# HPCForge/Bubbleformer

Measured on AMD Instinct MI355X. Metric: train samples/sec, FiLMAViT 16x192x192x4ch, bs=8 per GPU, higher is better.
Workload: dtype bf16; 1 GPU; FiLMAViT-small (E=384, 6 heads, 12 blocks, P=16, 9 fluid params) fwd + relative-L2 loss + bwd + AdamW, 4-field 16x192x192 clips, batch 8 per GPU (BASELINE.json configs[1]); global_batch=8, parallelism=dp1

## Files before the change

### bubbleformer_amd/_lib.py

```python
import ctypes as C
import os
import subprocess

_HERE = os.path.dirname(os.path.abspath(__file__))
LIB_PATH = os.path.join(_HERE, "libbubbleformer_hip.so")
CSRC = os.path.join(_HERE, "csrc")

BF_DTYPE_F32, BF_DTYPE_BF16 = 0, 1
BF_LAY_KC, BF_LAY_XC = 0, 1
BF_PRO_NONE, BF_PRO_AFFINE, BF_PRO_AFFINE_GELU, BF_PRO_GELU = 0, 1, 2, 3
BF_AUX_NONE, BF_AUX_ADD, BF_AUX_DGELU = 0, 1, 2
BF_OUT_STORE, BF_OUT_STORE_F32, BF_OUT_ATOMIC_F32 = 0, 1, 2
BF_MAX_STAGES = 5
BF_LOSS_LIMBS = 5

vp, fp, i32, i64, f32 = C.c_void_p, C.c_void_p, C.c_int32, C.c_int64, C.c_float


class Operand(C.Structure):
    _fields_ = [("p", vp), ("ld", i64), ("layout", i32), ("seglen", i32), ("segstride", i64), ("gw", i32), ("gh", i32),
                ("gc", i32), ("pro", i32), ("sc", fp), ("sh", fp), ("rows_per_frame", i32), ("nch", i32)]


class Epilogue(C.Structure):
    _fields_ = [("bias", fp), ("colscale", fp), ("colshift", fp), ("aux_mode", i32), ("aux", vp), ("ld_aux", i64),
                ("out_mode", i32), ("c", vp), ("ldc", i64), ("seglen", i32), ("segstride", i64), ("gw", i32), ("gh", i32),
                ("gc", i32), ("gelu_out", vp), ("colsum", fp), ("rowscale", fp), ("rows_per_group", i32)]


class Dims(C.Structure):
    _fields_ = [(n, i32) for n in ("dtype", "B", "T", "h", "w", "E", "heads", "attn_scale", "feat_scale", "patch", "cin",
                                   "cout", "nfluid")]


TEMPORAL_FIELDS = ("gamma", "attn_scale_factor", "norm1_w", "norm1_b", "norm2_w", "norm2_b", "input_head_w", "input_head_b",
                   "output_head_w", "output_head_b", "qnorm_w", "qnorm_b", "knorm_w", "knorm_b", "rel_pos_emb")
SPATIAL_FIELDS = ("gamma_att", "gamma_mlp", "attn_scale_factor_x", "attn_scale_factor_y", "low_freq_scalar",
                  "high_freq_scalar", "norm1_w", "norm1_b", "norm2_w", "norm2_b", "input_head_w", "input_head_b",
                  "output_head_w", "output_head_b", "qnorm_w", "qnorm_b", "knorm_w", "knorm_b", "rel_pos_emb", "fc1_w", "fc1_b",
                  "fc2_w", "fc2_b", "mlp_norm_w", "mlp_norm_b")


class TemporalParams(C.Structure):
    _fields_ = [(n, fp) for n in TEMPORAL_FIELDS]


class SpatialParams(C.Structure):
    _fields_ = [(n, fp) for n in SPATIAL_FIELDS]


class FrameNorm(C.Structure):
    _fields_ = [("w", fp), ("b", fp), ("g", fp), ("gdiv", i32), ("mean", fp), ("rstd", fp), ("sc", fp), ("sh", fp), ("resid", vp), ("out", vp)]


class EmbedParams(C.Structure):
    _fields_ = [("conv_w", fp * BF_MAX_STAGES), ("in_w", fp * BF_MAX_STAGES), ("in_b", fp * BF_MAX_STAGES), ("film_ln_w", fp),
                ("film_ln_b", fp), ("film_w", fp), ("film_b", fp)]


class DebedParams(C.Structure):
    _fields_ = [("conv_w", fp * BF_MAX_STAGES), ("in_w", fp * BF_MAX_STAGES), ("in_b", fp * BF_MAX_STAGES)]


class ConvSrc(C.Structure):
    _fields_ = [("p", vp), ("C", i32), ("nchw", i32), ("f32", i32)]


class ConvGeo(C.Structure):
    _fields_ = [(n, i32) for n in ("F", "Hi", "Wi", "Ho", "Wo", "kh", "kw", "stride", "pad")]


BF_CONV_PRO_NONE, BF_CONV_PRO_AFFINE_GELU, BF_CONV_PRO_GELU = 0, 1, 2

STAGE_DONE_FN = C.CFUNCTYPE(None, C.c_int, C.c_void_p)
P = C.POINTER
SIGNATURES = {
    "bf_last_error": (C.c_char_p, []),
    "bf_abi_version": (C.c_int, []),
    "bf_prof_enable": (None, [C.c_int]),
    "bf_debug_force_generic_attn": (None, [C.c_int]),
    "bf_debug_tokred_fold": (None, [C.c_int]),
    "bf_side_defer": (None, [C.c_int]),
    "bf_prep_stages": (C.c_int, [C.POINTER(Dims), C.c_int, C.POINTER(C.c_int32), C.POINTER(vp), C.POINTER(vp), C.POINTER(vp), vp]),
    "bf_stage_prepared": (None, [C.c_int]),
    "bf_trunk_train_fwd": (C.c_int, [C.POINTER(Dims), C.c_int, C.POINTER(C.c_int32), C.POINTER(vp), C.POINTER(vp), C.POINTER(vp), C.POINTER(vp), vp,
                                     C.POINTER(vp), vp, vp]),
    "bf_trunk_train_bwd": (C.c_int, [C.POINTER(Dims), C.c_int, C.POINTER(C.c_int32), C.POINTER(vp), C.POINTER(vp), C.POINTER(vp), C.POINTER(vp),
                                     C.POINTER(vp), vp, C.POINTER(vp), vp, C.POINTER(vp), vp, vp, vp, vp, vp]),
    "bf_field_stats_ws_doubles": (i64, [C.c_int]),
    "bf_field_stats": (C.c_int, [fp, vp, vp, C.c_int, vp, vp, vp]),
    "bf_stage_chain_next": (C.c_int, [C.POINTER(Dims), C.c_int, vp, vp]),
    "bf_stage_next_scale": (C.c_int, [fp, C.c_int]),
    "bf_gemm_fwd_frames": (C.c_int, [C.c_int, C.c_int, C.c_int, C.c_int, vp, i64, vp, i64, fp, fp, fp, fp, C.c_int, vp, vp, C.c_int,
                                     C.POINTER(FrameNorm), C.POINTER(FrameNorm), vp]),
    "bf_trunk_eval_weights_bytes": (i64, [C.POINTER(Dims), C.c_int, C.POINTER(C.c_int32)]),
    "bf_trunk_eval_prepare": (C.c_int, [C.POINTER(Dims), C.c_int, C.POINTER(C.c_int32), C.POINTER(vp), vp, vp]),
    "bf_trunk_eval_fwd": (C.c_int, [C.POINTER(Dims), C.c_int, C.POINTER(C.c_int32), C.POINTER(vp), vp, vp, vp, vp, vp]),
    "bf_frame_linear": (C.c_int, [C.c_int, C.c_int, C.c_int, C.c_int, C.c_int, vp, i64, vp, i64, fp, fp, fp, fp, fp, vp, i64, C.c_int, fp, fp, fp,
                                  vp, i64, fp, fp, vp, i64, vp]),
    "bf_side_join": (C.c_int, [vp]),
    "bf_prof_report": (C.c_int, [C.c_char_p, C.c_int]),
    "bf_gemm": (C.c_int, [C.c_int, C.c_int, C.c_int, C.c_int, P(Operand), P(Operand), P(Epilogue), C.c_int, vp]),
    "bf_gemm_tokred": (C.c_int, [C.c_int, C.c_int, C.c_int, i64, vp, i64, vp, i64, fp, C.c_int, fp, fp, i64, vp]),
    "bf_gemm_tokred_ws_floats": (i64, [C.c_int, C.c_int, i64]),
    "bf_gemm_inbwd_frames": (C.c_int, [C.c_int, C.c_int, C.c_int, C.c_int, vp, i64, vp, i64, vp, vp, vp, C.c_int, fp, fp, fp, fp, fp, C.c_int, vp]),
    "bf_gemm_inbwd_frames_chain": (C.c_int, [C.c_int, C.c_int, C.c_int, C.c_int, vp, i64, vp, i64, vp, vp, vp, C.c_int, fp, fp, fp, fp, fp, C.c_int,
                                             vp, vp, fp, fp, fp, fp, C.c_int, fp, vp]),
    "bf_in_stats": (C.c_int, [C.c_int, vp, C.c_int, C.c_int, C.c_int, fp, fp, fp, C.c_int, fp, fp, fp, fp, fp, fp, vp]),
    "bf_in_ws_floats": (i64, [C.c_int, C.c_int, C.c_int, C.c_int]),
    "bf_affine_apply": (C.c_int, [C.c_int, vp, vp, fp, fp, vp, i64, C.c_int, C.c_int, vp]),
    "bf_in_bwd": (C.c_int, [C.c_int, vp, vp, vp, vp, C.c_int, C.c_int, C.c_int, fp, fp, fp, fp, fp, C.c_int, C.c_int, fp, fp,
                            fp, fp, fp, vp]),
    "bf_colsum": (C.c_int, [C.c_int, vp, i64, C.c_int, fp, fp, vp]),
    "bf_attn_axial_fwd": (C.c_int, [C.c_int, vp, vp, i64, C.c_int, C.c_int, C.c_int, C.c_int, fp, fp, fp, fp, fp, fp, fp, vp]),
    "bf_attn_axial_norm_fwd": (C.c_int, [C.c_int, vp, vp, vp, i64, C.c_int, C.c_int, C.c_int, C.c_int, fp, fp, fp, fp, fp, fp, fp, fp, fp, fp, fp, fp,
                                         fp, vp]),
    "bf_attn_fwd": (C.c_int, [C.c_int, vp, vp, i64, C.c_int, i64, i64, i64, i64, C.c_int, C.c_int, fp, fp, fp, fp, fp, fp, f32,
                              C.c_int, vp]),
    "bf_attn_bwd": (C.c_int, [C.c_int, vp, vp, vp, i64, C.c_int, i64, i64, i64, i64, C.c_int, C.c_int, fp, fp, fp, fp, fp, fp,
                              fp, fp, fp, fp, fp, fp, f32, C.c_int, fp, i64, vp]),
    "bf_im2col_nchw": (C.c_int, [C.c_int, fp, vp, C.c_int, C.c_int, C.c_int, C.c_int, C.c_int, vp]),
    "bf_col2im_nchw": (C.c_int, [C.c_int, vp, fp, C.c_int, C.c_int, C.c_int, C.c_int, C.c_int, vp]),
    "bf_pm2nchw": (C.c_int, [fp, fp, fp, fp, C.c_int, C.c_int, C.c_int, C.c_int, C.c_int, vp]),
    "bf_debed_last_bwd": (C.c_int, [C.c_int, fp, fp, fp, fp, fp, vp, vp, vp, C.c_int, C.c_int, C.c_int, C.c_int, C.c_int, C.c_int, vp]),
    "bf_debed_last_bwd_norm": (C.c_int, [C.c_int, fp, fp, fp, fp, fp, vp, vp, vp, fp, fp, fp, fp, vp, fp, fp, C.c_int, C.c_int, C.c_int, C.c_int, C.c_int,
                                         C.c_int, fp, C.c_int64, vp]),
    "bf_gather_gemm": (C.c_int, [C.c_int, vp, vp, C.c_int, fp, fp, vp, C.c_int, C.c_int, C.c_int, C.c_int, C.c_int, vp]),
    "bf_scatter_gemm": (C.c_int, [C.c_int, vp, vp, C.c_int, fp, fp, vp, fp, C.c_int, C.c_int, C.c_int, C.c_int, C.c_int, vp]),
    "bf_gather_wgrad_ws_floats": (C.c_int64, [C.c_int, C.c_int, C.c_int]),
    "bf_gather_wgrad": (C.c_int, [C.c_int, vp, vp, fp, fp, fp, fp, fp, C.c_int, C.c_int, C.c_int, C.c_int, C.c_int, C.c_int, fp, C.c_int64, vp]),
    "bf_gather_gemm_rebuilt": (C.c_int, [C.c_int, vp, vp, vp, C.c_int, fp, fp, vp, C.c_int, C.c_int, C.c_int, C.c_int, C.c_int, vp]),
    "bf_gather_wgrad_rebuilt": (C.c_int, [C.c_int, vp, vp, vp, fp, fp, fp, C.c_int, C.c_int, C.c_int, C.c_int, C.c_int, C.c_int, fp, C.c_int64, vp]),
    "bf_stage_chain_head": (C.c_int, [vp, vp, vp]),
    "bf_stage_chain_tail": (C.c_int, [vp, vp, C.c_int]),
    "bf_embed_tail_ws_floats": (C.c_int64, [C.c_int, C.c_int, C.c_int, C.c_int, C.c_int]),
    "bf_embed_tail_bwd": (C.c_int, [C.c_int, vp, vp, vp, vp, vp, fp, fp, fp, fp, fp, fp, fp, fp, C.c_int, C.c_int, C.c_int, C.c_int, C.c_int, C.c_int,
                                    fp, C.c_int64, vp]),
    "bf_embed_first": (C.c_int, [C.c_int, fp, vp, vp, vp, C.c_int, C.c_int, C.c_int, C.c_int, C.c_int, C.c_int, fp, vp]),
    "bf_in_stats_merge_slices": (C.c_int, [C.c_int, C.c_int, C.c_int, C.c_int, C.c_int, fp, fp, fp, C.c_int, fp, fp, fp, fp, fp, fp, vp]),
    "bf_debed_last": (C.c_int, [C.c_int, vp, fp, fp, vp, fp, fp, fp, C.c_int, C.c_int, C.c_int, C.c_int, C.c_int, C.c_int, vp]),
    "bf_lploss_finalize": (C.c_int, [fp, C.c_int, C.c_int, fp, fp, vp]),
    "bf_nchw2pm": (C.c_int, [C.c_int, fp, fp, fp, fp, fp, vp, C.c_int, C.c_int, C.c_int, C.c_int, C.c_int, vp]),
    "bf_wprep": (C.c_int, [C.c_int, C.c_int, fp, vp, C.c_int, C.c_int, C.c_int, vp]),
    "bf_wgrad_unprep": (C.c_int, [C.c_int, fp, fp, C.c_int, C.c_int, C.c_int, C.c_int, vp]),
    "bf_film_net_fwd": (C.c_int, [fp, fp, fp, fp, fp, fp, fp, fp, C.c_int, C.c_int, C.c_int, vp]),
    "bf_film_net_bwd": (C.c_int, [fp, fp, fp, fp, fp, fp, fp, fp, fp, C.c_int, C.c_int, C.c_int, vp]),
    "bf_adamw": (C.c_int, [fp, fp, fp, fp, i64, C.c_int, f32, f32, f32, f32, f32, f32, vp]),
    "bf_adam": (C.c_int, [fp, fp, fp, fp, i64, C.c_int, f32, f32, f32, f32, f32, f32, vp]),
    "bf_lion": (C.c_int, [fp, fp, fp, i64, f32, f32, f32, f32, f32, vp]),
    "bf_grad_norm_ws_doubles": (i64, [i64]),
    "bf_grad_norm": (C.c_int, [fp, i64, f32, f32, fp, vp, i64, vp]),
    "bf_adamw_dev": (C.c_int, [fp, fp, fp, fp, i64, C.c_int, f32, f32, f32, f32, f32, f32, fp, f32, vp]),
    "bf_adam_dev": (C.c_int, [fp, fp, fp, fp, i64, C.c_int, f32, f32, f32, f32, f32, f32, fp, f32, vp]),
    "bf_lion_dev": (C.c_int, [fp, fp, fp, i64, f32, f32, f32, f32, f32, fp, f32, vp]),
    "bf_eikonal_sum": (C.c_int, [fp, i64, C.c_int, C.c_int, f32, vp, vp]),
    "bf_eikonal_l1_frames": (C.c_int, [fp, i64, C.c_int, C.c_int, f32, fp, vp]),
    "bf_heatflux_rows": (C.c_int, [fp, fp, i64, i64, C.c_int, f32, f32, f32, f32, fp, vp]),
    "bf_clip_gather": (C.c_int, [fp, i64, vp, vp, C.c_int, fp, fp, fp, C.c_int, C.c_int, C.c_int, C.c_int, C.c_int, C.c_int, C.c_int, vp]),
    "bf_clip_gather_batch": (C.c_int, [fp, i64, vp, i64, vp, vp, fp, fp, C.c_int, C.c_int, fp, vp, fp, fp, C.c_int, C.c_int, fp, fp, vp, C.c_int, fp,
                                       C.c_int, C.c_int, C.c_int, C.c_int, C.c_int, vp]),
    "bf_rollout_score_ws_doubles": (i64, [C.c_int, C.c_int, C.c_int, C.c_int, C.c_int]),
    "bf_rollout_score": (C.c_int, [fp, fp, i64, i64, C.c_int, vp, vp, vp, fp, fp, C.c_int, f32, fp, fp, fp, fp, fp, fp, vp, i64, C.c_int, C.c_int,
                                   C.c_int, C.c_int, C.c_int, C.c_int, C.c_int, C.c_int, vp]),
    "bf_rollout_heatflux": (C.c_int, [fp, fp, i64, i64, C.c_int, vp, vp, vp, fp, fp, C.c_int, C.c_int, fp, f32, f32, f32, f32, fp, fp, C.c_int, C.c_int,
# ... 88 lines not shown
```

### bubbleformer_amd/csrc/attn_mfma.hip

```cpp
#include "bf_common.h"
#include "param_reduce.h"
#include <stdlib.h>

namespace {

typedef __attribute__((ext_vector_type(8))) short s16x8;
typedef __attribute__((address_space(3))) s16x4* lds_s16x4;

__device__ __forceinline__ void drain_vm() { __builtin_amdgcn_s_waitcnt(0x0F70); }
__device__ __forceinline__ void wsync() {
    __builtin_amdgcn_fence(__ATOMIC_ACQ_REL, "wavefront");
    __builtin_amdgcn_wave_barrier();
}
__device__ __forceinline__ int t5b(int n) {
    const int a = n < 0 ? -n : n;
    int b;
    if (a < 8) b = a; else if (a < 10) b = 8; else if (a < 12) b = 9; else if (a < 14) b = 10; else if (a < 16) b = 11;
    else if (a < 20) b = 12; else if (a < 23) b = 13; else if (a < 27) b = 14; else b = 15;
    return b + (n < 0 ? 16 : 0);
}
typedef unsigned u32x2 __attribute__((ext_vector_type(2)));
__device__ __forceinline__ float quad_sum(float v) {
    u32x2 r = __builtin_amdgcn_permlane16_swap(__float_as_uint(v), __float_as_uint(v), false, false);
    v = __uint_as_float(r[0]) + __uint_as_float(r[1]);
// ... 812 lines not shown
        const int head = (int)(((long)blockIdx.x * wpb + wave) % heads);
#pragma unroll
        for (int jb = 0; jb < NB; ++jb)
#pragma unroll
            for (int ib = 0; ib < NB; ++ib)
#pragma unroll
                for (int r = 0; r < 4; ++r) {
                    const int i = 16 * ib + i16, j = 16 * jb + 4 * gq + r;
                    if (gr.demb && i < L && j < L) atomicAdd(&s_demb[t5b(i - j) * 16 + head], a_emb[jb][ib][r]);
                }
        if (p.hscale && gr.dhscale) {
            a_dhs = wave_sum(a_dhs);
            if (lane == 0) atomicAdd(&s_dhs[head], a_dhs);
        }
    }
#pragma unroll
    for (int k = 0; k < NACC; ++k) {
        const int v = 16 * k + i16, q = v / (8 * KS), ks = (v >> 3) % KS, j = v & 7;
        relay[q * D + 32 * ks + 8 * gq + j] = a_ln[k];
    }
    __syncthreads();
    const int nvals = 4 * D + 32 * heads + heads;
    for (int i = threadIdx.x; i < nvals; i += blockDim.x) {
        float val;
        float* dst;
        if (i < 4 * D) {
            val = 0.f;
            for (int w = 0; w < wpb; ++w) val += reinterpret_cast<const float*>(smem_bwd + w * PER_WAVE)[i];
            const int q = i / D, e = i % D; dst = (q == 0 ? gr.dqw : q == 1 ? gr.dqb : q == 2 ? gr.dkw : gr.dkb); if (dst) dst += e; }
        else if (i < 4 * D + 32 * heads) { const int t = i - 4 * D; val = s_demb[(t / heads) * 16 + (t % heads)]; dst = gr.demb ? gr.demb + t : nullptr; }
        else { const int t = i - 4 * D - 32 * heads; val = s_dhs[t]; dst = gr.dhscale ? gr.dhscale + t : nullptr; }
        if (ws) ws[(long)blockIdx.x * nvals + i] = val;
        else if (dst && val != 0.f) atomicAdd(dst, val);
    }
}

__global__ void __launch_bounds__(64 * BF_RED_FL) attn_ws_reduce(AttnReduceJob j) {
    __shared__ float red[1][BF_RED_FL][64];
    attn_reduce_block(j, blockIdx.x, blockIdx.y, gridDim.y, red);
}

template <typename K>
int set_lds(K kernel, size_t shm) {
    if (shm > 64 * 1024) {
        hipError_t e = hipFuncSetAttribute(reinterpret_cast<const void*>(kernel), hipFuncAttributeMaxDynamicSharedMemorySize, (int)shm);
        if (e != hipSuccess) return bf_fail(e, __FILE__, __LINE__);
    }
    return 0;
}

template <int NB, int KS>
int go_fwd(const bf16* qkv, bf16* out, Geo g, int heads, Par p, float out_scale, int accumulate, hipStream_t st) {
    constexpr int D = 32 * KS;
    const int wpb = 4;
    const size_t shm = (size_t)wpb * 16 * NB * (D + 16) * sizeof(bf16);
    const long nprob = g.nseq * heads;
    BF_REQUIRE(nprob < (1L << 31) && g.inner < (1L << 31), "attention: problem count must fit 31 bits");
    static const int bpc = bf_knob("BF_ATTN_FWD_BPC", 2);
    const int grid = (int)std::min<long>((nprob + wpb - 1) / wpb, 256L * bpc);
    hipLaunchKernelGGL((attn_fwd_mfma<NB, KS>), dim3(grid), dim3(wpb * 64), shm, st, qkv, out, g, heads, p, out_scale, accumulate);
    BF_CHECK_LAUNCH();
    return 0;
}
template <int NB, int KS, int ACC>
int go_bwd_mode(const bf16* qkv, const bf16* dout, bf16* dqkv, Geo g, int heads, Par p, Grd gr, float out_scale, int accumulate, float* ws,
                long ws_floats, int* rows_out, hipStream_t st) {
    constexpr int D = 32 * KS, R = 16 * NB;
    const int wpb = NB == 1 ? 4 : 2;
    const size_t shm = (size_t)wpb * (3 * R * (D + 16) + 2 * R * 40) * sizeof(bf16);
    if (int rc = set_lds(attn_bwd_mfma<NB, KS, ACC>, shm)) return rc;
    const long nprob = g.nseq * heads;
    BF_REQUIRE(nprob < (1L << 31) && g.inner < (1L << 31), "attention: problem count must fit 31 bits");
    const int nvals = 4 * D + 32 * heads + heads;
    static int resident = 0;
    if (!resident) {
        int dev = 0, cus = 256, per_cu = 1;
        (void)hipGetDevice(&dev);
        (void)hipDeviceGetAttribute(&cus, hipDeviceAttributeMultiprocessorCount, dev);
        if (hipOccupancyMaxActiveBlocksPerMultiprocessor(&per_cu, attn_bwd_mfma<NB, KS, ACC>, wpb * 64, shm) != hipSuccess || per_cu < 1) per_cu = 1;
        static const int bpc = bf_knob("BF_ATTN_BWD_BPC", 0);
        if (bpc > 0) per_cu = bpc;
        resident = cus * per_cu;
    }
    long grid = std::min<long>((nprob + wpb - 1) / wpb, (long)resident);
    {
        long a = wpb, b = heads;
        while (b) { const long t = a % b; a = b; b = t; }
        const long m = heads / a;
        if (grid >= 8 * m) grid -= grid % m;
    }
    if (ws && ws_floats < grid * nvals) { grid = ws_floats / nvals; if (grid < 1) ws = nullptr; }
    hipLaunchKernelGGL((attn_bwd_mfma<NB, KS, ACC>), dim3((int)grid), dim3(wpb * 64), shm, st, qkv, dout, dqkv, g, heads, p, gr, out_scale, accumulate, ws);
    BF_CHECK_LAUNCH();
    if (rows_out) { *rows_out = ws ? (int)grid : 0; return 0; }
    if (ws) {
        const AttnReduceJob j{ws, (int)grid, D, heads, gr.dqw, gr.dqb, gr.dkw, gr.dkb, gr.demb, gr.dhscale};
        hipLaunchKernelGGL(attn_ws_reduce, dim3(bf_cdiv(nvals, 64), 1), dim3(64 * BF_RED_FL), 0, st, j);
        BF_CHECK_LAUNCH();
    }
    return 0;
}
template <int NB, int KS>
int go_bwd(const bf16* qkv, const bf16* dout, bf16* dqkv, Geo g, int heads, Par p, Grd gr, float out_scale, int accumulate, float* ws,
           long ws_floats, int* rows_out, hipStream_t st) {
#define BF_MODE(A) return go_bwd_mode<NB, KS, A>(qkv, dout, dqkv, g, heads, p, gr, out_scale, accumulate, ws, ws_floats, rows_out, st)
    if constexpr (NB == 1 && KS == 2) {
        switch (accumulate) { case 0: BF_MODE(0); case 1: BF_MODE(1); case 2: BF_MODE(2); case 5: BF_MODE(5); default: break; }
    }
    BF_MODE(-1);
#undef BF_MODE
}

}

int bf_attn_fwd_mfma(const void* qkv, void* out, long nseq, int L, long inner, long outer_stride, long inner_stride, long tok_stride, int heads,
                     int d, const float* qw, const float* qb, const float* kw, const float* kb, const float* emb, const float* hscale,
                     float out_scale, int accumulate, hipStream_t st) {
    Geo g{nseq, L, inner, outer_stride, inner_stride, tok_stride};
    Par p{qw, qb, kw, kb, emb, hscale};
    const int nb = L <= 16 ? 1 : 2, ks = d / 32;
#define GO(NB, KS) if (nb == NB && ks == KS) return go_fwd<NB, KS>((const bf16*)qkv, (bf16*)out, g, heads, p, out_scale, accumulate, st)
    GO(1, 1); GO(1, 2); GO(1, 3); GO(1, 4); GO(2, 1); GO(2, 2); GO(2, 3); GO(2, 4);
#undef GO
    return bf_fail_msg("bf_attn_fwd_mfma: unsupported shape", __FILE__, __LINE__);
}
int bf_attn_axial_fwd_mfma(const void* qkv, void* out, int frames, int h, int w, int heads, int d, const float* qw, const float* qb, const float* kw,
                           const float* kb, const float* emb, const float* hscale_x, const float* hscale_y, const float* nw, const float* nb,
                           void* out_n, float* mean, float* rstd, float* sc, float* sh, hipStream_t st) {
    static const bool off = bf_knob("BF_ATTN_AXIAL_FUSED", 1) == 0;
    if (off || h > 16 || w > 16 || h < 1 || w < 1 || d % 32 || d > 128 || heads > 16) return 1;
    Par p{qw, qb, kw, kb, emb, hscale_x};
    const long ntile = (long)frames * heads;
    static const int wpb_env = bf_knob("BF_ATTN_AXIAL_WPB", 0);
    const int ks = d / 32, wpb = (wpb_env == 4 || wpb_env == 12) ? wpb_env : (ntile <= 256 ? 12 : 4);
    const bool norm = nw != nullptr;
    const size_t tile = ((size_t)h * w * (d + 8) + 7) & ~(size_t)7;
    const size_t shm = ((size_t)wpb * 16 * (d + 16) + tile) * sizeof(bf16) + (norm ? ((size_t)(256 / (d / 8)) + 2) * d * sizeof(float) : 0);
    const int grid = (int)std::min<long>(ntile, 256L * 3);
    const AxNorm nrm{nw, nb, (bf16*)out_n, mean, rstd, sc, sh};
#define GO2(KS, NRM, W) { if (int rc = set_lds(attn_fwd_axial_mfma<KS, NRM, W>, shm)) return rc; \
        hipLaunchKernelGGL((attn_fwd_axial_mfma<KS, NRM, W>), dim3(grid), dim3(W * 64), shm, st, (const bf16*)qkv, (bf16*)out, frames, h, w, heads, p, hscale_y, nrm); }
#define GO(KS) if (ks == KS) { \
        if (norm) { if (wpb == 12) GO2(KS, true, 12) else GO2(KS, true, 4) } \
        else { if (wpb == 12) GO2(KS, false, 12) else GO2(KS, false, 4) } }
    GO(1) GO(2) GO(3) GO(4)
#undef GO
#undef GO2
    BF_CHECK_LAUNCH();
    return 0;
}
int bf_attn_bwd_mfma(const void* qkv, const void* dout, void* dqkv, long nseq, int L, long inner, long outer_stride, long inner_stride,
                     long tok_stride, int heads, int d, const float* qw, const float* qb, const float* kw, const float* kb, const float* emb,
                     const float* hscale, float* dqw, float* dqb, float* dkw, float* dkb, float* demb, float* dhscale, float out_scale,
                     int accumulate, float* ws, long ws_floats, int* rows_out, hipStream_t st) {
    Geo g{nseq, L, inner, outer_stride, inner_stride, tok_stride};
    Par p{qw, qb, kw, kb, emb, hscale};
    Grd gr{dqw, dqb, dkw, dkb, demb, dhscale};
    const int nb = L <= 16 ? 1 : 2, ks = d / 32;
#define GO(NB, KS) if (nb == NB && ks == KS) return go_bwd<NB, KS>((const bf16*)qkv, (const bf16*)dout, (bf16*)dqkv, g, heads, p, gr, out_scale, accumulate, ws, ws_floats, rows_out, st)
    GO(1, 1); GO(1, 2); GO(1, 3); GO(1, 4); GO(2, 1); GO(2, 2); GO(2, 3); GO(2, 4);
#undef GO
    return bf_fail_msg("bf_attn_bwd_mfma: unsupported shape", __FILE__, __LINE__);
}
```

### bubbleformer_amd/csrc/bf_common.h

```cpp
#pragma once
#include <hip/hip_runtime.h>
#include <stdint.h>
#include <math.h>

#include "../../include/bubbleformer_hip.h"

typedef __bf16 bf16;
typedef __attribute__((ext_vector_type(8))) __bf16 bf16x8;
typedef __attribute__((ext_vector_type(4))) __bf16 bf16x4;
typedef __attribute__((ext_vector_type(4))) short s16x4;
typedef __attribute__((ext_vector_type(4))) float f32x4;

#define BF_WAVE 64
#define BF_IN_EPS 1e-5f

#define BF_CHECK_LAUNCH()                                   \
    do {                                                    \
        hipError_t e__ = hipGetLastError();                 \
        if (e__ != hipSuccess) return bf_fail(e__, __FILE__, __LINE__); \
    } while (0)
#define BF_REQUIRE(cond, msg)                                \
    do {                                                     \
        if (!(cond)) return bf_fail_msg(msg, __FILE__, __LINE__); \
    } while (0)

int bf_prof_begin(hipStream_t st);
bool bf_prof_is_on();
void bf_prof_end(int idx, hipStream_t st, const char* name, double flops, double bytes);
struct BfProfScope {
    int idx; hipStream_t st; const char* name; double flops, bytes;
    BfProfScope(hipStream_t s, const char* n, double f, double b) : idx(bf_prof_begin(s)), st(s), name(n), flops(f), bytes(b) {}
    ~BfProfScope() { if (idx >= 0) bf_prof_end(idx, st, name, flops, bytes); }
};

int bf_in_bwd_partials(int dtype, const void* dy, const void* x, const void* add, void* dx, int frames, int S, int C, const float* mean,
                       const float* rstd, const float* w, const float* b, const float* g, int gdiv, int gelu, float* ws, hipStream_t stream);
int bf_attn_bwd_partials(int dtype, const void* qkv, const void* dout, void* dqkv, int64_t nseq, int L, int64_t inner, int64_t outer_stride,
                         int64_t inner_stride, int64_t tok_stride, int heads, int d, const float* qw, const float* qb, const float* kw,
                         const float* kb, const float* emb, const float* hscale, float* dqw, float* dqb, float* dkw, float* dkb, float* demb,
                         float* dhscale, float out_scale, int accumulate, float* ws, int64_t ws_floats, int* rows, hipStream_t stream);
int bf_in_stats_apply(int dtype, const void* x, int frames, int S, int C, const float* w, const float* b, const float* g, int gdiv, const float* gb,
                      float* mean, float* rstd, float* sc, float* sh, float* ws, const void* resid, void* out, hipStream_t stream);
int bf_in_stats_apply_chain(int dtype, const void* x, int frames, int S, int C, const float* w, const float* b, const float* g, int gdiv, const float* gb,
                            float* mean, float* rstd, float* sc, float* sh, float* ws, const void* resid, void* out, const float* nw, const float* nb,
                            float* nmean, float* nrstd, float* nsc, float* nsh, void* nxn, bool* chained, hipStream_t stream);
int bf_wprep_multi(int dtype, int n, const int* mode, const float* const* src, void* const* dst, const int* R, const int* K, const int* Kp, hipStream_t st);
int bf_frame_scale(int dtype, const void* z, const float* m, int fdiv, void* out, long nrows, int S, int C, hipStream_t st);

int bf_gemm_slabs(int dtype, int M, int N, int K, const bf_operand* A, const bf_operand* B, float* out, long ldc, int accumulate, int splitk,
                  float* ws, long ws_floats, hipStream_t st);
int bf_tokred_narrow(int dtype, int C, int64_t P, const void* wide, const void* narrow, float* out, int ldo, int accumulate, int transposed,
                     const float* sc, const float* sh, int64_t rows_per_frame, float* ws, int64_t ws_floats, hipStream_t st);
int bf_gemm_pair_scaled(int M, int N, int K, const bf_operand* A, const bf_operand* B, const bf_epilogue* E, void* out2, const float* rowfac,
                        int rows_per_group, hipStream_t st);

#ifdef BF_EXPERIMENTS
#include <stdlib.h>
inline int bf_knob(const char* name, int dflt) { const char* v = getenv(name); return v ? atoi(v) : dflt; }
#else
constexpr int bf_knob(const char*, int dflt) { return dflt; }
#endif

struct BfPerDeviceOnce {
    bool done[64] = {};
    bool& flag() { int dev = 0; (void)hipGetDevice(&dev); return done[(dev >= 0 && dev < 64) ? dev : 0]; }
};
template <class T> struct BfPerDevice {
    T tab[64] = {};
    T& get() { int dev = 0; (void)hipGetDevice(&dev); return tab[(dev >= 0 && dev < 64) ? dev : 0]; }
};
int bf_fail(hipError_t e, const char* file, int line);
int bf_fail_msg(const char* msg, const char* file, int line);
int bf_decline(const char* msg);

__device__ __forceinline__ float to_f(float x) { return x; }
__device__ __forceinline__ float to_f(bf16 x) { return (float)x; }
template <typename T> __device__ __forceinline__ T from_f(float x);
template <> __device__ __forceinline__ float from_f<float>(float x) { return x; }
template <> __device__ __forceinline__ bf16 from_f<bf16>(float x) { return (bf16)x; }

template <typename T> struct Chunk;
template <> struct Chunk<float> {
    static constexpr int N = 4;
    float4 raw;
    __device__ __forceinline__ void load(const float* p) { raw = *reinterpret_cast<const float4*>(p); }
    __device__ __forceinline__ void store(float* p) const { *reinterpret_cast<float4*>(p) = raw; }
    __device__ __forceinline__ void zero() { raw = make_float4(0.f, 0.f, 0.f, 0.f); }
    __device__ __forceinline__ float get(int i) const { return i == 0 ? raw.x : i == 1 ? raw.y : i == 2 ? raw.z : raw.w; }
    __device__ __forceinline__ void set(int i, float v) { if (i == 0) raw.x = v; else if (i == 1) raw.y = v; else if (i == 2) raw.z = v; else raw.w = v; }
};
template <> struct Chunk<bf16> {
    static constexpr int N = 8;
    bf16x8 raw;
    __device__ __forceinline__ void load(const bf16* p) { raw = *reinterpret_cast<const bf16x8*>(p); }
    __device__ __forceinline__ void store(bf16* p) const { *reinterpret_cast<bf16x8*>(p) = raw; }
    __device__ __forceinline__ void zero() { for (int i = 0; i < 8; ++i) raw[i] = (bf16)0.f; }
    __device__ __forceinline__ float get(int i) const { return (float)raw[i]; }
    __device__ __forceinline__ void set(int i, float v) { raw[i] = (bf16)v; }
};

__device__ __forceinline__ float erf_fast(float x) {
    const float ax = fabsf(x);
    const float t = __builtin_amdgcn_rcpf(1.0f + 0.3275911f * ax);
    const float poly = t * (0.254829592f + t * (-0.284496736f + t * (1.421413741f + t * (-1.453152027f + t * 1.061405429f))));
    const float r = 1.0f - poly * __expf(-ax * ax);
    return copysignf(r, x);
}
__device__ __forceinline__ float gelu_f(float x) { return 0.5f * x * (1.0f + erf_fast(x * 0.70710678118654752440f)); }
__device__ __forceinline__ float dgelu_f(float x) {
    const float ax = fabsf(x) * 0.70710678118654752440f;
    const float t = __builtin_amdgcn_rcpf(1.0f + 0.3275911f * ax);
    const float poly = t * (0.254829592f + t * (-0.284496736f + t * (1.421413741f + t * (-1.453152027f + t * 1.061405429f))));
    const float e = __expf(-0.5f * x * x);
    const float cdf = 0.5f * (1.0f + copysignf(1.0f - poly * e, x));
    return cdf + x * (0.39894228040143267794f * e);
}

__device__ __forceinline__ float phi_fast(float x) {
    const float xc = fminf(fmaxf(x, -4.0f), 4.0f), u = xc * xc;
    float r = -1.520480094e-09f;
    r = r * u + 1.180964698e-07f; r = r * u - 4.014221545e-06f; r = r * u + 7.960997465e-05f; r = r * u - 1.041295800e-03f;
    r = r * u + 9.641715296e-03f; r = r * u - 6.614117438e-02f; r = r * u + 3.988329119e-01f;
    return 0.5f + xc * r;
}
__device__ __forceinline__ float gelu_fast(float x) { return x * phi_fast(x); }
__device__ __forceinline__ float dgelu_fast(float x) {
    const float xc = fminf(fmaxf(x, -4.0f), 4.0f), u = xc * xc;
    float r = 9.387459194e-10f;
    r = r * u - 7.941240515e-08f; r = r * u + 2.950722870e-06f; r = r * u - 6.380590451e-05f; r = r * u + 8.975979855e-04f;
    r = r * u - 8.669717964e-03f; r = r * u + 5.833777581e-02f; r = r * u - 2.646917422e-01f; r = r * u + 7.975648121e-01f;
    return 0.5f + xc * r;
}

// ... 17 lines not shown
```

### bubbleformer_amd/csrc/gemm_stream.hip

```cpp
#include "gemm_common.h"
#include <stdio.h>
#include <stdlib.h>
#include <algorithm>

namespace {
using namespace bfgemm;

constexpr int BM = 256, BNB = 128, BK = 64;
constexpr int CHUNK = BNB * BK;
constexpr int ACHUNK = BM * BK;
constexpr int NSLOT = 2;

struct StreamArgs {
    const bf16* A; long lda; const bf16* W; long ldw; bf16* C; long ldc;
    const float* bias; const float* colscale; const float* colshift; const float* rowscale; int rpg;
    int aux_mode; const bf16* aux; long ld_aux; bf16* gelu_out;
    int KS, mt, nb, ng;
    int mh, hunit;
    int stagger;
    int dbg;
};

__device__ __forceinline__ void wait_vm_n(int n) {
    if (n >= 16) { wait_vm<16>(); return; }
// ... 409 lines not shown
            if constexpr (CS) {
#pragma unroll
                for (int i = 0; i < 4; ++i) asm volatile("" : "+v"(rsr[i]));
            }
            __builtin_amdgcn_sched_barrier(0);
        }
#pragma unroll
        for (int i = 0; i < 4; ++i) {
            const int m = m0 + wm * 64 + i * 16 + li;
#pragma unroll
            for (int pp = 0; pp < 2; ++pp) {
                float v[8];
#pragma unroll
                for (int r = 0; r < 4; ++r) {
                    typedef __attribute__((ext_vector_type(2))) unsigned u32x2;
                    const u32x2 sw = __builtin_amdgcn_permlane16_swap(__float_as_uint(acc[i][2 * pp][r]), __float_as_uint(acc[i][2 * pp + 1][r]), false, false);
                    v[r] = __uint_as_float(sw[0]); v[4 + r] = __uint_as_float(sw[1]);
                }
                if constexpr (AUX == BF_AUX_ADD) {
                    const bf16x8 ax = __builtin_bit_cast(bf16x8, auxr[i][pp]);
#pragma unroll
                    for (int q = 0; q < 8; ++q) {
                        float cs_ = 1.f, ch_ = 0.f;
                        if constexpr (CS) { cs_ = e_cs[pp][q]; ch_ = e_ch[pp][q]; }
                        v[q] = epi_lin_add(v[q], e_bias[pp][q], cs_, ch_, has_rs ? rsr[i] : 1.f, CS, (float)ax[q]);
                    }
                } else {
#pragma unroll
                    for (int q = 0; q < 8; ++q) {
                        float cs_ = 1.f, ch_ = 0.f;
                        if constexpr (CS) { cs_ = e_cs[pp][q]; ch_ = e_ch[pp][q]; }
                        v[q] = epi_lin(v[q], e_bias[pp][q], cs_, ch_, has_rs ? rsr[i] : 1.f, CS);
                    }
                    if constexpr (AUX == BF_AUX_DGELU) {
                        const bf16x8 ax = __builtin_bit_cast(bf16x8, auxr[i][pp]);
#pragma unroll
                        for (int q = 0; q < 8; ++q) v[q] = v[q] * dgelu_fast((float)ax[q]);
                    }
                }
                bf16x8 o;
#pragma unroll
                for (int q = 0; q < 8; ++q) o[q] = (bf16)v[q];
                const long off = (long)m * a.ldc + c_nb * BNB + c8 + 32 * pp;
                *reinterpret_cast<bf16x8*>(a.C + off) = o;
                if constexpr (GELU2) {
                    bf16x8 g8;
#pragma unroll
                    for (int q = 0; q < 8; ++q) g8[q] = (bf16)gelu_fast(v[q]);
                    *reinterpret_cast<bf16x8*>(a.gelu_out + off) = g8;
                }
            }
        }
        issued += GELU2 ? 16 : 8;
    }
}


int num_cus() {
    static const int n = []() {
        int dev = 0; hipDeviceProp_t p;
        if (hipGetDevice(&dev) != hipSuccess || hipGetDeviceProperties(&p, dev) != hipSuccess || p.multiProcessorCount < 8) return 256;
        return p.multiProcessorCount;
    }();
    return n;
}

bool team_split(int NB, int mt, int wpx, int* nb, int* ng) {
    static const int force = bf_knob("BF_STREAM_GROUPS", 0);
    int best = 0, best_cost = 0;
    for (int g = 1; g <= NB; ++g) {
        if (NB % g || NB / g > wpx || (force > 0 && g != force)) continue;
        const int nteams = 8 * (wpx / (NB / g));
        if (nteams < g) continue;
        const int fewest = nteams / g;
        const int cost = (mt + fewest - 1) / fewest;
        if (!best || cost < best_cost) { best = g; best_cost = cost; }
    }
    if (!best) return false;
    *ng = best; *nb = NB / best;
    return true;
}

}

int bf_gemm_stream_try(int M, int N, int K, const bf_operand* A, const bf_operand* B, const bf_epilogue* E, hipStream_t st) {
    static const int enabled = bf_knob("BF_GEMM_STREAM", 1);
    if (!enabled) return 1;
    if (A->layout != BF_LAY_KC || B->layout != BF_LAY_KC || A->pro != BF_PRO_NONE || B->pro != BF_PRO_NONE) return 1;
    if (A->gw > 0 || A->seglen > 0 || B->gw > 0 || B->seglen > 0 || E->gw > 0 || E->seglen > 0) return 1;
    if (E->out_mode != BF_OUT_STORE || E->colsum) return 1;
    static const int pp_env = bf_knob("BF_STREAM_PP", -1);
    if (M % BM || N % BNB || K % BK || K < 2 * BK) return 1;
    const bool ws_ok = K >= 4 * BK && K <= 6 * BK;
    const bool use_pp = pp_env == 1 || !ws_ok;
    if (pp_env == 0 && !ws_ok) return 1;
    if (A->ld % 8 || B->ld % 8 || E->ldc % 8 || (E->aux_mode != BF_AUX_NONE && E->ld_aux % 8)) return 1;
    if (((uintptr_t)A->p | (uintptr_t)B->p | (uintptr_t)E->c | (uintptr_t)E->aux | (uintptr_t)E->gelu_out) & 15) return 1;
    if (E->gelu_out && E->aux_mode != BF_AUX_NONE) return 1;
    if (E->colscale && !E->colshift) return 1;
    StreamArgs a;
    a.A = (const bf16*)A->p; a.lda = A->ld; a.W = (const bf16*)B->p; a.ldw = B->ld; a.C = (bf16*)E->c; a.ldc = E->ldc;
    a.bias = E->bias; a.colscale = E->colscale; a.colshift = E->colshift; a.rowscale = E->rowscale; a.rpg = E->rows_per_group > 0 ? E->rows_per_group : 1;
    a.aux_mode = E->aux_mode; a.aux = (const bf16*)E->aux; a.ld_aux = E->ld_aux; a.gelu_out = (bf16*)E->gelu_out;
    a.KS = K / BK; a.mt = M / BM; a.mh = M / (BM / 2);
    static const int half_on = bf_knob("BF_STREAM_HALF", 1);
    a.hunit = half_on ? 1 : 2;
    const int grid = (num_cus() / 8) * 8;
    if (!team_split(N / BNB, (use_pp || !half_on) ? a.mt : a.mh, grid / 8, &a.nb, &a.ng)) return 1;
    static const int dbg = bf_knob("BF_STREAM_DEBUG", 0);
    a.dbg = dbg;
    static const int stagger = bf_knob("BF_STREAM_STAGGER", 1);
    a.stagger = stagger;
    const int lds_bytes = a.KS * CHUNK * 2 + NSLOT * ACHUNK * 2;
    static thread_local char pname[64];
    snprintf(pname, sizeof(pname), use_pp ? "stream_pp<%s>" : "stream_gemm<%s>", E->gelu_out ? "gelu2" : E->aux_mode == BF_AUX_ADD ? "add" : E->aux_mode == BF_AUX_DGELU ? "dgelu" : "plain");
    BfProfScope prof(st, pname, 2.0 * M * N * K, ((double)M * K + (double)N * K + (double)M * N * (E->gelu_out ? 2 : 1) + (E->aux_mode != BF_AUX_NONE ? (double)M * N : 0.0)) * 2.0);
#define BF_STREAM_GO(AUXM, G2, CSF)                                                                                                       \
    do {                                                                                                                                \
        static BfPerDeviceOnce attr_once, attr_pp_once; bool& attr_done = attr_once.flag(); bool& attr_pp_done = attr_pp_once.flag();                                                                            \
        if (use_pp) {                                                                                                                   \
            if (!attr_pp_done) {                                                                                                        \
                hipError_t e_ = hipFuncSetAttribute((const void*)stream_pp_kernel<AUXM, G2, CSF>, hipFuncAttributeMaxDynamicSharedMemorySize, PNSLOT * PSLOT); \
                if (e_ != hipSuccess) return bf_fail(e_, __FILE__, __LINE__);                                                           \
                attr_pp_done = true;                                                                                                    \
            }                                                                                                                           \
            hipLaunchKernelGGL((stream_pp_kernel<AUXM, G2, CSF>), dim3(grid), dim3(512), PNSLOT * PSLOT, st, a);                        \
            break;                                                                                                                      \
        }                                                                                                                               \
        if (!attr_done) {                                                                                                               \
            hipError_t e_ = hipFuncSetAttribute((const void*)stream_gemm_kernel<AUXM, G2, CSF>, hipFuncAttributeMaxDynamicSharedMemorySize, 6 * CHUNK * 2 + NSLOT * ACHUNK * 2); \
            if (e_ != hipSuccess) return bf_fail(e_, __FILE__, __LINE__);                                                               \
            attr_done = true;                                                                                                           \
        }                                                                                                                               \
        hipLaunchKernelGGL((stream_gemm_kernel<AUXM, G2, CSF>), dim3(grid), dim3(512), lds_bytes, st, a);                                    \
    } while (0)
    const bool cs = E->colscale != nullptr || E->rowscale != nullptr;
    if (E->gelu_out && !cs) BF_STREAM_GO(BF_AUX_NONE, true, false);
    else if (E->gelu_out) return 1;
    else if (E->aux_mode == BF_AUX_ADD && cs) BF_STREAM_GO(BF_AUX_ADD, false, true);
    else if (E->aux_mode == BF_AUX_ADD) BF_STREAM_GO(BF_AUX_ADD, false, false);
    else if (E->aux_mode == BF_AUX_DGELU && !cs) BF_STREAM_GO(BF_AUX_DGELU, false, false);
    else if (E->aux_mode == BF_AUX_DGELU) return 1;
    else if (cs) return 1;
    else BF_STREAM_GO(BF_AUX_NONE, false, false);
#undef BF_STREAM_GO
    BF_CHECK_LAUNCH();
    return 0;
}
```

### bubbleformer_amd/csrc/gemm_tokred.hip

```cpp
#include "gemm_common.h"
#include <stdio.h>
#include <stdlib.h>
#include <algorithm>

namespace {
using namespace bfgemm;

constexpr int PTN = 192;
constexpr int HR = 32;
constexpr int NSB = PTN / 64;
constexpr int SUBB = HR * 64 * 2;
constexpr int NBUF = 4;
template <int NI> struct PPGeom {
    static constexpr int TM = 64 * NI, HALFB = (NI + NSB) * SUBB, TILES = NI * 6, TILE_FLOATS = TM * PTN;
};

template <int OFF>
__device__ __forceinline__ void glds16_off(const void* gsrc, unsigned lds_dst) {
    unsigned keep;
    asm volatile("s_mov_b32 %0, m0\n\ts_mov_b32 m0, %2\n\ts_nop 0\n\tglobal_load_lds_dwordx4 %1, off offset:%3\n\ts_mov_b32 m0, %0"
                 : "=&s"(keep) : "v"(gsrc), "s"(lds_dst - (unsigned)OFF), "n"(OFF) : "memory");
}

typedef __attribute__((address_space(3))) s16x4* lds_s16x4_ptr;
__device__ __forceinline__ bf16x8 tr_frag(unsigned addr) {
    const s16x4 lo = __builtin_amdgcn_ds_read_tr16_b64_v4i16((lds_s16x4_ptr)(uintptr_t)addr);
    const s16x4 hi = __builtin_amdgcn_ds_read_tr16_b64_v4i16((lds_s16x4_ptr)(uintptr_t)(addr + 512u));
    typedef __attribute__((ext_vector_type(8))) short s16x8;
    const s16x8 r = {lo[0], lo[1], lo[2], lo[3], hi[0], hi[1], hi[2], hi[3]};
    return __builtin_bit_cast(bf16x8, r);
}

template <int NI, int GRP>
__device__ __forceinline__ void tokred_pp_body(const bf16* __restrict__ A, long lda, const bf16* __restrict__ B, long ldb,
                                               float* __restrict__ slab_tile, float* __restrict__ cslab_row, int nh, bool do_cs,
                                               unsigned ring_lds, int lane, int w4) {
    using Gm = PPGeom<NI>;
    constexpr int HALFB = Gm::HALFB;
    constexpr int PG = NI == 6 ? (GRP == 0 ? 5 : 4) : 3;
    constexpr int NCS = 3;
    const int wm = w4, wn = GRP;
    const int dr = 8 * w4 + (lane >> 3);
    const int dkey = ((dr >> 1) & 1) | (((dr >> 3) & 1) << 1);
    const int dch = (lane & 7) ^ (dkey << 1);
    const bf16* pA = A + (long)dr * lda + 8 * dch;
    const bf16* pB = B + (long)dr * ldb + 8 * dch;
    const long stepA = (long)HR * lda, stepB = (long)HR * ldb;
    auto issue = [&](int buf) {
        const unsigned base = __builtin_amdgcn_readfirstlane(ring_lds + (unsigned)buf * (unsigned)HALFB + (unsigned)w4 * 1024u);
        if constexpr (NI == 6 && GRP == 0) {
            glds16_off<0>(pA, base + 0 * SUBB); glds16_off<128>(pA, base + 1 * SUBB); glds16_off<256>(pA, base + 2 * SUBB);
            glds16_off<384>(pA, base + 3 * SUBB); glds16_off<512>(pA, base + 4 * SUBB);
            pA += stepA;
        } else if constexpr (NI == 6) {
            glds16_off<640>(pA, base + 5 * SUBB);
            glds16_off<0>(pB, base + 6 * SUBB); glds16_off<128>(pB, base + 7 * SUBB); glds16_off<256>(pB, base + 8 * SUBB);
            pA += stepA; pB += stepB;
        } else if constexpr (GRP == 0) {
            glds16_off<0>(pA, base + 0 * SUBB); glds16_off<128>(pA, base + 1 * SUBB); glds16_off<256>(pA, base + 2 * SUBB);
            pA += stepA;
        } else {
            glds16_off<0>(pB, base + 3 * SUBB); glds16_off<128>(pB, base + 4 * SUBB); glds16_off<256>(pB, base + 5 * SUBB);
            pB += stepB;
        }
    };
    const int g = lane >> 4, q = (lane >> 2) & 3, p = lane & 3;
    const int fkey = ((q >> 1) & 1) | ((g & 1) << 1);
    const unsigned rowb = (unsigned)(8 * g + q) * 128u + (unsigned)(p & 1) * 8u;
    const unsigned offA = rowb + (unsigned)(((2 * wm + (p >> 1)) ^ (fkey << 1)) * 16);
    const unsigned offB0 = rowb + (unsigned)(((2 * wn + (p >> 1)) ^ (fkey << 1)) * 16) + (unsigned)(NI * SUBB);
    const unsigned offB1 = rowb + (unsigned)(((2 * wn + 4 + (p >> 1)) ^ (fkey << 1)) * 16) + (unsigned)(NI * SUBB);

    f32x4 acc[NI][6];
#pragma unroll
    for (int i = 0; i < NI; ++i)
#pragma unroll
        for (int j = 0; j < 6; ++j) acc[i][j] = f32x4{0.f, 0.f, 0.f, 0.f};
    f32x4 cs[NCS];
#pragma unroll
    for (int c = 0; c < NCS; ++c) cs[c] = f32x4{0.f, 0.f, 0.f, 0.f};
    bf16x8 ones;
#pragma unroll
    for (int c = 0; c < 8; ++c) ones[c] = (bf16)1.0f;

    issue(0);
    if (nh > 1) issue(1);
    if (nh > 2) issue(2);
    if (nh > 2) wait_vm<2 * PG>(); else if (nh > 1) wait_vm<PG>(); else wait_vm<0>();
    __builtin_amdgcn_s_barrier();
    if constexpr (GRP == 1) __builtin_amdgcn_s_barrier();

    int buf = 0;
    for (int h = 0; h < nh; ++h) {
        const unsigned hb = ring_lds + (unsigned)buf * (unsigned)HALFB;
        bf16x8 fa[NI], fb[6];
#pragma unroll
        for (int i = 0; i < NI; ++i) fa[i] = tr_frag(hb + offA + (unsigned)(i * SUBB));
#pragma unroll
        for (int j = 0; j < 6; ++j) fb[j] = tr_frag(hb + ((j & 1) ? offB1 : offB0) + (unsigned)((j >> 1) * SUBB));
        if (h + 3 < nh) issue((buf + 3) & 3);
        const int younger = min(h + 3, nh - 1) - (h + 1);
        if (younger >= 2) wait_vm<2 * PG>(); else if (younger == 1) wait_vm<PG>(); else wait_vm<0>();
        asm volatile("s_waitcnt lgkmcnt(0)" ::: "memory");
        __builtin_amdgcn_sched_barrier(0);
        __builtin_amdgcn_s_barrier();
#pragma unroll
        for (int i = 0; i < NI; ++i)
#pragma unroll
            for (int j = 0; j < 6; ++j) acc[i][j] = __builtin_amdgcn_mfma_f32_16x16x32_bf16(fb[j], fa[i], acc[i][j], 0, 0, 0);
        if (do_cs) {
#pragma unroll
            for (int c = 0; c < NCS; ++c) {
                if constexpr (NI == 6) cs[c] = __builtin_amdgcn_mfma_f32_16x16x32_bf16(ones, fa[NCS * GRP + c], cs[c], 0, 0, 0);
                else if constexpr (GRP == 0) cs[c] = __builtin_amdgcn_mfma_f32_16x16x32_bf16(ones, fa[c], cs[c], 0, 0, 0);
            }
        }
        __builtin_amdgcn_sched_barrier(0);
        __builtin_amdgcn_s_barrier();
        buf = (buf + 1) & 3;
    }
    if constexpr (GRP == 0) __builtin_amdgcn_s_barrier();

    const int wave = GRP * 4 + w4;
    float* so = slab_tile + ((size_t)wave * Gm::TILES * 64 + lane) * 4;
#pragma unroll
    for (int i = 0; i < NI; ++i)
#pragma unroll
        for (int j = 0; j < 6; ++j)
            *reinterpret_cast<float4*>(so + (size_t)(i * 6 + j) * 256) = make_float4(acc[i][j][0], acc[i][j][1], acc[i][j][2], acc[i][j][3]);
    if (do_cs && lane < 16) {
        if constexpr (NI == 6) {
#pragma unroll
            for (int c = 0; c < NCS; ++c) cslab_row[16 * (wm + 4 * (NCS * GRP + c)) + lane] = cs[c][0];
        } else if constexpr (GRP == 0) {
#pragma unroll
            for (int c = 0; c < NCS; ++c) cslab_row[16 * (wm + 4 * c) + lane] = cs[c][0];
        }
    }
}

struct FoldRed { const float* slab; const float* cslab; int nslice, ntiles, tiles_k, Nout, Kin; float* out; float* colsum; int accumulate; int nwg; };
template <int NI>
__device__ __forceinline__ void fold_reduce(const FoldRed& r, int b) {
    using Gm = PPGeom<NI>;
    constexpr int T4 = Gm::TILE_FLOATS / 4;
    const long total = (long)r.ntiles * T4;
    const size_t sstride = (size_t)r.ntiles * Gm::TILE_FLOATS;
    for (long e = (long)b * 512 + threadIdx.x; e < total; e += (long)r.nwg * 512) {
        const int tile = (int)(e / T4), q = (int)(e - (long)tile * T4);
        const int lane = q & 63, t = q >> 6, wave = t / Gm::TILES, ij = t - wave * Gm::TILES, i = ij / 6, j = ij - i * 6;
        const int wm = wave & 3, wn = wave >> 2;
        const int nout = (tile / r.tiles_k) * Gm::TM + 16 * (wm + 4 * i) + (lane & 15);
        const int kin = (tile % r.tiles_k) * PTN + 16 * (wn + 2 * j) + 4 * (lane >> 4);
        const float* src = r.slab + (size_t)tile * Gm::TILE_FLOATS + (size_t)q * 4;
        float4* dst = reinterpret_cast<float4*>(r.out + (size_t)nout * r.Kin + kin);
        float4 a = r.accumulate ? *dst : make_float4(0.f, 0.f, 0.f, 0.f);
        for (int s0 = 0; s0 < r.nslice; s0 += 8) {
            float4 v[8];
#pragma unroll
            for (int u = 0; u < 8; ++u) v[u] = s0 + u < r.nslice ? *reinterpret_cast<const float4*>(src + (size_t)(s0 + u) * sstride) : make_float4(0.f, 0.f, 0.f, 0.f);
#pragma unroll
            for (int u = 0; u < 8; ++u)
                if (s0 + u < r.nslice) { a.x += v[u].x; a.y += v[u].y; a.z += v[u].z; a.w += v[u].w; }
        }
        *dst = a;
    }
    if (r.colsum)
        for (long m = (long)b * 512 + threadIdx.x; m < r.Nout; m += (long)r.nwg * 512) {
            float a = r.accumulate ? r.colsum[m] : 0.f;
            for (int s2 = 0; s2 < r.nslice; ++s2) a += r.cslab[(size_t)s2 * r.Nout + m];
            r.colsum[m] = a;
        }
}

template <int NI>
__global__ void __launch_bounds__(512) tokred_pp_kernel(const bf16* __restrict__ A, long lda, const bf16* __restrict__ B, long ldb,
                                                      float* __restrict__ slab, float* __restrict__ cslab, int Nout, int halves_total,
                                                      int halves_per, int tiles_k, int ntiles, int main_wgs, FoldRed red) {
    using Gm = PPGeom<NI>;
    extern __shared__ __attribute__((aligned(16))) char smem[];
    if ((int)blockIdx.x >= main_wgs) { fold_reduce<NI>(red, (int)blockIdx.x - main_wgs); return; }
    const int tid = threadIdx.x, lane = tid & 63, wave = __builtin_amdgcn_readfirstlane(tid >> 6);
    const int seq = xcd_remap(blockIdx.x, main_wgs);
    const int slice = seq / ntiles, tile = seq - slice * ntiles;
    const int n0 = (tile / tiles_k) * Gm::TM, c0 = (tile % tiles_k) * PTN;
    const int h_beg = slice * halves_per;
    const int nh = min(halves_per, halves_total - h_beg);
    const bf16* a0 = A + (long)h_beg * HR * lda + n0;
    const bf16* b0 = B + (long)h_beg * HR * ldb + c0;
    float* slab_tile = slab + ((size_t)slice * ntiles + tile) * Gm::TILE_FLOATS;
    const bool do_cs = cslab != nullptr && c0 == 0;
    float* cslab_row = do_cs ? cslab + (size_t)slice * Nout + n0 : nullptr;
    const unsigned ring_lds = lds_addr(smem);
    if (wave < 4) tokred_pp_body<NI, 0>(a0, lda, b0, ldb, slab_tile, cslab_row, nh, do_cs, ring_lds, lane, wave);
    else tokred_pp_body<NI, 1>(a0, lda, b0, ldb, slab_tile, cslab_row, nh, do_cs, ring_lds, lane, wave - 4);
}

template <int NI, int MAXS>
__global__ void __launch_bounds__(256) tokred_pp_reduce_kernel(const float* __restrict__ slab, const float* __restrict__ cslab, int nslice,
                                                               int ntiles, int tiles_k, int Nout, int Kin, float* __restrict__ out,
                                                               float* __restrict__ colsum, int accumulate) {
    using Gm = PPGeom<NI>;
    constexpr int T4 = Gm::TILE_FLOATS / 4;
    const long e = (long)blockIdx.x * 256 + threadIdx.x;
    if (e < (long)ntiles * T4) {
        const int tile = (int)(e / T4), r = (int)(e - (long)tile * T4);
        const int lane = r & 63, t = r >> 6, wave = t / Gm::TILES, ij = t - wave * Gm::TILES, i = ij / 6, j = ij - i * 6;
        const int wm = wave & 3, wn = wave >> 2;
        const int nout = (tile / tiles_k) * Gm::TM + 16 * (wm + 4 * i) + (lane & 15);
        const int kin = (tile % tiles_k) * PTN + 16 * (wn + 2 * j) + 4 * (lane >> 4);
        const size_t sstride = (size_t)ntiles * Gm::TILE_FLOATS;
        const float* src = slab + (size_t)tile * Gm::TILE_FLOATS + (size_t)r * 4;
        float4 v[MAXS];
#pragma unroll
        for (int s = 0; s < MAXS; ++s) v[s] = s < nslice ? *reinterpret_cast<const float4*>(src + s * sstride) : make_float4(0.f, 0.f, 0.f, 0.f);
        float4* dst = reinterpret_cast<float4*>(out + (size_t)nout * Kin + kin);
        float4 a = accumulate ? *dst : make_float4(0.f, 0.f, 0.f, 0.f);
#pragma unroll
        for (int s = 0; s < MAXS; ++s)
            if (s < nslice) { a.x += v[s].x; a.y += v[s].y; a.z += v[s].z; a.w += v[s].w; }
        *dst = a;
    }
    if (colsum && e < Nout) {
        float v[MAXS];
#pragma unroll
        for (int s = 0; s < MAXS; ++s) v[s] = s < nslice ? cslab[(size_t)s * Nout + e] : 0.f;
        float a = accumulate ? colsum[e] : 0.f;
#pragma unroll
        for (int s = 0; s < MAXS; ++s)
            if (s < nslice) a += v[s];
        colsum[e] = a;
    }
}

constexpr int NW_TILE = 32;
template <int CT, bool PRO>
__global__ void __launch_bounds__(256) tokred_narrow_kernel(const bf16* __restrict__ dy, const bf16* __restrict__ x, long tiles_total, float* __restrict__ slab,
                                                          const float* __restrict__ psc, const float* __restrict__ psh, int tiles_per_frame) {
    constexpr int C = 16 * CT, DYB = NW_TILE * C * 2, XB = NW_TILE * 16 * 2, TB_ = DYB + XB;
    extern __shared__ __attribute__((aligned(16))) char smem[];
    const int tid = threadIdx.x, lane = tid & 63, wave = __builtin_amdgcn_readfirstlane(tid >> 6);
    const long nwaves = (long)gridDim.x * 4, w = (long)blockIdx.x * 4 + wave;
    const long t_beg = tiles_total * w / nwaves, t_end = tiles_total * (w + 1) / nwaves;
    char* mine = smem + (size_t)wave * 2 * TB_;
    const unsigned lds0 = lds_addr(mine);
    auto issue = [&](long t, int slot) {
        const char* gd = reinterpret_cast<const char*>(dy) + t * DYB + lane * 16;
        const unsigned dst = __builtin_amdgcn_readfirstlane(lds0 + (unsigned)slot * (unsigned)TB_);
#pragma unroll
        for (int pce = 0; pce < DYB / 1024; ++pce) glds16(gd + pce * 1024, dst + (unsigned)pce * 1024u);
        glds16(reinterpret_cast<const char*>(x) + t * XB + lane * 16, dst + (unsigned)DYB);
    };
    constexpr int PCS = DYB / 1024 + 1;
    f32x4 acc[CT];
#pragma unroll
    for (int i = 0; i < CT; ++i) acc[i] = f32x4{0.f, 0.f, 0.f, 0.f};
    const int g = lane >> 4, q = (lane >> 2) & 3, pp = lane & 3;
    const unsigned offD = (unsigned)((8 * g + q) * (C * 2) + 8 * pp), offX = (unsigned)(DYB + (8 * g + q) * 32 + 8 * pp);
    auto trf = [&](unsigned addr, unsigned hi_off) {
        const s16x4 lo = __builtin_amdgcn_ds_read_tr16_b64_v4i16((lds_s16x4_ptr)(uintptr_t)addr);
        const s16x4 hi = __builtin_amdgcn_ds_read_tr16_b64_v4i16((lds_s16x4_ptr)(uintptr_t)(addr + hi_off));
        typedef __attribute__((ext_vector_type(8))) short s16x8;
        const s16x8 r = {lo[0], lo[1], lo[2], lo[3], hi[0], hi[1], hi[2], hi[3]};
        return __builtin_bit_cast(bf16x8, r);
    };
    float scv[CT], shv[CT];
    for (long s_beg = t_beg; s_beg < t_end;) {
        long s_end = t_end;
        if constexpr (PRO) {
            const long f = s_beg / tiles_per_frame;
            s_end = min(t_end, (f + 1) * (long)tiles_per_frame);
            wait_vm<0>();
#pragma unroll
            for (int i = 0; i < CT; ++i) { scv[i] = psc[f * C + 16 * i + (lane & 15)]; shv[i] = psh ? psh[f * C + 16 * i + (lane & 15)] : 0.f; }
#pragma unroll
            for (int i = 0; i < CT; ++i) asm volatile("s_waitcnt vmcnt(0)" : "+v"(scv[i]), "+v"(shv[i]) :: "memory");
        }
        issue(s_beg, 0);
        int slot = 0;
        for (long t = s_beg; t < s_end; ++t) {
// ... 145 lines not shown
#pragma unroll
    for (int i = 0; i < TMI; ++i)
#pragma unroll
        for (int j = 0; j < TNI; ++j)
            *reinterpret_cast<float4*>(so + (size_t)(i * 16) * Kin + j * 16) = make_float4(acc[i][j][0], acc[i][j][1], acc[i][j][2], acc[i][j][3]);
    if (do_cs && lg == 0) cslab[(size_t)slice * Nout + n0 + wm * (16 * TMI) + wn * 16 + li] = cs[0];
}

__global__ void __launch_bounds__(256) tokred_reduce_kernel(const float* __restrict__ slab, const float* __restrict__ cslab, int nslice, long n,
                                                            int Nout, float* __restrict__ out, float* __restrict__ colsum, int accumulate) {
    const long n4 = n / 4;
    for (long i = (long)blockIdx.x * 256 + threadIdx.x; i < n4; i += (long)gridDim.x * 256) {
        float4 a = accumulate ? reinterpret_cast<const float4*>(out)[i] : make_float4(0.f, 0.f, 0.f, 0.f);
        for (int s0 = 0; s0 < nslice; s0 += 8) {
            float4 v[8];
#pragma unroll
            for (int q = 0; q < 8; ++q) v[q] = s0 + q < nslice ? reinterpret_cast<const float4*>(slab + (size_t)(s0 + q) * n)[i] : make_float4(0.f, 0.f, 0.f, 0.f);
#pragma unroll
            for (int q = 0; q < 8; ++q)
                if (s0 + q < nslice) { a.x += v[q].x; a.y += v[q].y; a.z += v[q].z; a.w += v[q].w; }
        }
        reinterpret_cast<float4*>(out)[i] = a;
    }
    if (colsum) {
        for (long m = (long)blockIdx.x * 256 + threadIdx.x; m < Nout; m += (long)gridDim.x * 256) {
            float a = accumulate ? colsum[m] : 0.f;
            for (int s = 0; s < nslice; ++s) a += cslab[(size_t)s * Nout + m];
            colsum[m] = a;
        }
    }
}

constexpr int MAX_SLICES = 16;

}

extern "C" int64_t bf_gemm_tokred_ws_floats(int Nout, int Kin, int64_t M) {
    if (Nout <= 0 || Kin <= 0 || M <= 0) return 0;
    return (int64_t)MAX_SLICES * ((int64_t)Nout * Kin + Nout);
}

namespace {
struct PendingRed { bool on = false; FoldRed r{}; int NI = 0; hipStream_t st = nullptr; bool half = false; hipEvent_t handoff = nullptr; };
PendingRed g_pending[64];
PendingRed& pending_slot() { int dev = 0; (void)hipGetDevice(&dev); return g_pending[(dev >= 0 && dev < 64) ? dev : 0]; }
constexpr int FOLD_WGS = 40;
}
static int tokred_impl(int dtype, int Nout, int Kin, int64_t M, const void* dy, int64_t ldy, const void* x, int64_t ldx, float* out,
                       int accumulate, float* colsum, float* ws, int64_t ws_floats, bool defer, bf_stream_t stream);
static int flush_pending(PendingRed& p, hipStream_t caller) {
    if (!p.on) return 0;
    p.on = false;
    hipStream_t st = p.st;
    const FoldRed& r = p.r;
    const long n = (long)r.Nout * r.Kin;
    const unsigned rblocks = (unsigned)bf_cdiv(std::max<long>(n / 4, r.Nout), 256);
    BfProfScope prof(st, "tokred_reduce_kernel", 0.0, (double)(r.nslice + 1 + (r.accumulate ? 1 : 0)) * n * 4.0);
    if (p.NI == 6) {
        if (r.nslice <= 8) hipLaunchKernelGGL((tokred_pp_reduce_kernel<6, 8>), dim3(rblocks), dim3(256), 0, st, r.slab, r.cslab, r.nslice, r.ntiles, r.tiles_k, r.Nout, r.Kin, r.out, r.colsum, r.accumulate);
        else hipLaunchKernelGGL((tokred_pp_reduce_kernel<6, MAX_SLICES>), dim3(rblocks), dim3(256), 0, st, r.slab, r.cslab, r.nslice, r.ntiles, r.tiles_k, r.Nout, r.Kin, r.out, r.colsum, r.accumulate);
    } else {
        if (r.nslice <= 8) hipLaunchKernelGGL((tokred_pp_reduce_kernel<3, 8>), dim3(rblocks), dim3(256), 0, st, r.slab, r.cslab, r.nslice, r.ntiles, r.tiles_k, r.Nout, r.Kin, r.out, r.colsum, r.accumulate);
        else hipLaunchKernelGGL((tokred_pp_reduce_kernel<3, MAX_SLICES>), dim3(rblocks), dim3(256), 0, st, r.slab, r.cslab, r.nslice, r.ntiles, r.tiles_k, r.Nout, r.Kin, r.out, r.colsum, r.accumulate);
    }
    BF_CHECK_LAUNCH();
    if (caller == st) return 0;
    hipError_t e = p.handoff ? hipSuccess : hipEventCreateWithFlags(&p.handoff, hipEventDisableTiming);
    if (e == hipSuccess) e = hipEventRecord(p.handoff, st);
    if (e == hipSuccess) e = hipStreamWaitEvent(caller, p.handoff, 0);
    return e == hipSuccess ? 0 : bf_fail(e, __FILE__, __LINE__);
}
int bf_gemm_tokred_flush(hipStream_t st) { return flush_pending(pending_slot(), st); }
namespace { bool g_fold_off = false; }
extern "C" void bf_debug_tokred_fold(int on) { g_fold_off = on == 0; }
bool bf_gemm_tokred_pending() { return pending_slot().on; }
const float* bf_gemm_tokred_pending_out() { const PendingRed& p = pending_slot(); return p.on ? p.r.out : nullptr; }
int bf_gemm_tokred_deferred(int dtype, int Nout, int Kin, int64_t M, const void* dy, int64_t ldy, const void* x, int64_t ldx, float* out,
                            int accumulate, float* colsum, float* ws, int64_t ws_floats, hipStream_t stream) {
    return tokred_impl(dtype, Nout, Kin, M, dy, ldy, x, ldx, out, accumulate, colsum, ws, ws_floats, true, (bf_stream_t)stream);
}
extern "C" int bf_gemm_tokred(int dtype, int Nout, int Kin, int64_t M, const void* dy, int64_t ldy, const void* x, int64_t ldx, float* out,
                              int accumulate, float* colsum, float* ws, int64_t ws_floats, bf_stream_t stream) {
    return tokred_impl(dtype, Nout, Kin, M, dy, ldy, x, ldx, out, accumulate, colsum, ws, ws_floats, false, stream);
}
static int tokred_impl(int dtype, int Nout, int Kin, int64_t M, const void* dy, int64_t ldy, const void* x, int64_t ldx, float* out,
                       int accumulate, float* colsum, float* ws, int64_t ws_floats, bool defer, bf_stream_t stream) {
    if (dtype != BF_DTYPE_BF16) return 1;
    static const int skip_env = bf_knob("BF_TOKRED_SKIP", 0);
    if (skip_env) return 0;
    const bool pp = Nout % 192 == 0 && Kin % PTN == 0 && M % HR == 0 && M >= 4 * HR;
    if (!pp && (Nout % TB || Kin % TB || M % BK || M < BK)) return 1;
    if (ldy % 8 || ldx % 8) return 1;
    BF_REQUIRE(dy && x && out && ws, "bf_gemm_tokred: null pointer");
    BF_REQUIRE(((uintptr_t)dy & 15) == 0 && ((uintptr_t)x & 15) == 0 && ((uintptr_t)out & 15) == 0 && ((uintptr_t)ws & 15) == 0,
               "bf_gemm_tokred: operands must be 16-byte aligned");
    BF_REQUIRE(ldy >= Nout && ldx >= Kin, "bf_gemm_tokred: leading dimensions smaller than the row length");
    hipStream_t st = (hipStream_t)stream;
    const long n = (long)Nout * Kin;
    static const int slices_env = bf_knob("BF_TOKRED_SLICES", 0);
    static const int tile_env = bf_knob("BF_TOKRED_TILE", 0);
    static const int wgs_env = bf_knob("BF_TOKRED_WGS", 128);
    if (pp) {
        const long halves = M / HR;
        const int tiles_k0 = Kin / PTN;
        const bool big = Nout % 384 == 0 && tile_env == 384;
        const int tm = big ? 384 : 192;
        int nslice = slices_env > 0 ? slices_env : std::max(1, wgs_env / ((Nout / tm) * tiles_k0));
        nslice = (int)std::max<long>(1, std::min<long>({(long)nslice, (long)MAX_SLICES, halves / 4}));
        const int halves_per = bf_cdiv(halves, nslice);
        const int ns = bf_cdiv(halves, halves_per);
        BF_REQUIRE(ws_floats >= (int64_t)ns * (n + Nout), "bf_gemm_tokred: workspace too small (bf_gemm_tokred_ws_floats)");
        const int tiles_k = Kin / PTN, ntiles = (Nout / tm) * tiles_k;
        static const bool fold_on = bf_knob("BF_TOKRED_FOLD", 1) != 0;
        const int64_t half_floats = (ws_floats / 2) & ~(int64_t)3;
        const bool fold = defer && fold_on && !g_fold_off && (int64_t)ns * (n + Nout) <= half_floats;
        PendingRed& pend = pending_slot();
        if (pend.on && (!fold || pend.NI != (big ? 6 : 3) || pend.st != st)) { const int frc = flush_pending(pend, st); if (frc) return frc; }
        float* region = ws;
        if (fold) { region = ws + (pend.half ? half_floats : 0); pend.half = !pend.half; }
        float* slab = region;
        float* cslab = colsum ? region + (size_t)ns * n : nullptr;
        const unsigned rblocks = (unsigned)bf_cdiv(std::max<long>(n / 4, Nout), 256);
        FoldRed red{};
        static const int fold_wgs = bf_knob("BF_TOKRED_FOLD_WGS", FOLD_WGS);
        if (fold && pend.on) { red = pend.r; red.nwg = fold_wgs; }
        const unsigned extra = red.nwg > 0 ? (unsigned)red.nwg : 0u;
#define BF_PP_GO(NIV)                                                                                                                     \
        do {                                                                                                                              \
            {                                                                                                                             \
                BfProfScope prof(st, NIV == 6 ? "tokred_pp_kernel<384x192,h32,ring4>" : "tokred_pp_kernel<192x192,h32,ring4>",           \
                                 2.0 * Nout * Kin * (double)M, (double)M * (Nout + Kin) * 2.0 + (double)n * 4.0);                         \
                static BfPerDeviceOnce attr_once; bool& attr_done = attr_once.flag();                                                                                            \
                constexpr int lds_bytes = NBUF * PPGeom<NIV>::HALFB;                                                                      \
                if (!attr_done) {                                                                                                         \
                    hipError_t e_ = hipFuncSetAttribute((const void*)tokred_pp_kernel<NIV>, hipFuncAttributeMaxDynamicSharedMemorySize, lds_bytes); \
                    if (e_ != hipSuccess) return bf_fail(e_, __FILE__, __LINE__);                                                         \
                    attr_done = true;                                                                                                     \
                }                                                                                                                         \
                hipLaunchKernelGGL(tokred_pp_kernel<NIV>, dim3((unsigned)(ns * ntiles) + extra), dim3(512), lds_bytes, st, (const bf16*)dy, (long)ldy, \
                                   (const bf16*)x, (long)ldx, slab, cslab, Nout, (int)halves, halves_per, tiles_k, ntiles, ns * ntiles, red); \
                BF_CHECK_LAUNCH();                                                                                                        \
            }                                                                                                                             \
            if (fold) {                                                                                                                   \
                pend.on = true; pend.NI = NIV; pend.st = st;                                                                              \
                pend.r = FoldRed{slab, cslab, ns, ntiles, tiles_k, Nout, Kin, out, colsum, accumulate, 0};                                \
                break;                                                                                                                    \
            }                                                                                                                             \
            BfProfScope prof(st, "tokred_reduce_kernel", 0.0, (double)(ns + 1 + (accumulate ? 1 : 0)) * n * 4.0);                         \
            if (ns <= 8) hipLaunchKernelGGL((tokred_pp_reduce_kernel<NIV, 8>), dim3(rblocks), dim3(256), 0, st, slab, cslab, ns, ntiles, tiles_k, Nout, Kin, out, colsum, accumulate); \
            else hipLaunchKernelGGL((tokred_pp_reduce_kernel<NIV, MAX_SLICES>), dim3(rblocks), dim3(256), 0, st, slab, cslab, ns, ntiles, tiles_k, Nout, Kin, out, colsum, accumulate); \
            BF_CHECK_LAUNCH();                                                                                                            \
        } while (0)
        if (big) BF_PP_GO(6); else BF_PP_GO(3);
#undef BF_PP_GO
        return 0;
    }
    { const int frc = flush_pending(pending_slot(), st); if (frc) return frc; }
    const long steps = M / BK;
    int nslice = slices_env > 0 ? slices_env : 8;
    nslice = (int)std::max<long>(1, std::min<long>({(long)nslice, (long)MAX_SLICES, steps}));
    BF_REQUIRE(ws_floats >= (int64_t)nslice * (n + Nout), "bf_gemm_tokred: workspace too small (bf_gemm_tokred_ws_floats)");
    const int steps_per = bf_cdiv(steps, nslice);
    const int ns = bf_cdiv(steps, steps_per);
    const int tiles_k = Kin / TB, ntiles = (Nout / TB) * tiles_k;
    float* slab = ws;
    float* cslab = colsum ? ws + (size_t)ns * n : nullptr;
    {
        BfProfScope prof(st, "tokred_kernel<128x128,bk64,slots3>", 2.0 * Nout * Kin * (double)M, (double)M * (Nout + Kin) * 2.0 + (double)n * 4.0);
        static BfPerDeviceOnce attr_once; bool& attr_done = attr_once.flag();
        constexpr int lds_bytes = NSLOT * 2 * BK * TB * 2;
        if (!attr_done) {
            hipError_t e_ = hipFuncSetAttribute((const void*)tokred_kernel, hipFuncAttributeMaxDynamicSharedMemorySize, lds_bytes);
            if (e_ != hipSuccess) return bf_fail(e_, __FILE__, __LINE__);
            attr_done = true;
        }
        hipLaunchKernelGGL(tokred_kernel, dim3((unsigned)(ns * ntiles)), dim3(512), lds_bytes, st, (const bf16*)dy, (long)ldy, (const bf16*)x,
                           (long)ldx, slab, cslab, Nout, Kin, (int)steps, steps_per, tiles_k, ntiles);
        BF_CHECK_LAUNCH();
    }
    {
        BfProfScope prof(st, "tokred_reduce_kernel", 0.0, (double)(ns + 1 + (accumulate ? 1 : 0)) * n * 4.0);
        const int blocks = (int)std::min<long>(512, (n / 4 + 255) / 256);
        hipLaunchKernelGGL(tokred_reduce_kernel, dim3(blocks), dim3(256), 0, st, slab, cslab, ns, n, Nout, out, colsum, accumulate);
        BF_CHECK_LAUNCH();
    }
    return 0;
}

int bf_tokred_narrow(int dtype, int C, int64_t P, const void* wide, const void* narrow, float* out, int ldo, int accumulate, int transposed,
                     const float* sc, const float* sh, int64_t rows_per_frame, float* ws, int64_t ws_floats, hipStream_t st) {
    static const bool off = bf_knob("BF_TOKRED_NARROW", 1) == 0;
    if (off || dtype != BF_DTYPE_BF16 || (C != 96 && C != 64 && C != 32) || P <= 0 || P % NW_TILE || ldo < (transposed ? C : 16)) return 1;
    if (((uintptr_t)wide | (uintptr_t)narrow | (uintptr_t)ws) & 15) return 1;
    if (sc && (rows_per_frame <= 0 || rows_per_frame % NW_TILE)) return 1;
    const int wgs = sc ? 512 : 256;
    if (ws_floats < (int64_t)wgs * C * 16) return 1;
    const long tiles = P / NW_TILE;
    const int tpf = sc ? (int)(rows_per_frame / NW_TILE) : 1;
    BfProfScope prof(st, sc ? "tokred_narrow_kernel<gelu>" : "tokred_narrow_kernel", 2.0 * C * 16 * (double)P, (double)P * (C + 16) * 2.0);
#define BF_NARROW_GO(CTV)                                                                                                               \
    do {                                                                                                                                \
        constexpr int lds_bytes = 4 * 2 * (NW_TILE * 16 * CTV * 2 + NW_TILE * 16 * 2);                                                  \
        static_assert(lds_bytes >= 4 * 16 * CTV * 16 * 4, "the reduction buffer aliases the tile rings");                               \
        if (sc) hipLaunchKernelGGL((tokred_narrow_kernel<CTV, true>), dim3(wgs), dim3(256), lds_bytes, st, (const bf16*)wide, (const bf16*)narrow, tiles, ws, sc, sh, tpf); \
        else hipLaunchKernelGGL((tokred_narrow_kernel<CTV, false>), dim3(wgs), dim3(256), lds_bytes, st, (const bf16*)wide, (const bf16*)narrow, tiles, ws, sc, sh, tpf); \
    } while (0)
    if (C == 96) BF_NARROW_GO(6); else if (C == 64) BF_NARROW_GO(4); else BF_NARROW_GO(2);
#undef BF_NARROW_GO
    BF_CHECK_LAUNCH();
    hipLaunchKernelGGL(tokred_narrow_reduce_kernel, dim3(bf_cdiv(C * 16, 256)), dim3(256), 0, st, ws, wgs, C, out, ldo, accumulate, transposed);
    BF_CHECK_LAUNCH();
    return 0;
}
```

### bubbleformer_amd/csrc/model.hip

```cpp
#include <functional>
#include <vector>
#include "bf_common.h"
#include "param_reduce.h"
#include <stdlib.h>
#include <string.h>

bool bf_attn_raw_modes(int dtype, int d);
int bf_gemm_tokred_deferred(int dtype, int Nout, int Kin, int64_t M, const void* dy, int64_t ldy, const void* x, int64_t ldx, float* out,
                            int accumulate, float* colsum, float* ws, int64_t ws_floats, hipStream_t stream);
int bf_gemm_tokred_flush(hipStream_t st);
bool bf_gemm_tokred_pending();
const float* bf_gemm_tokred_pending_out();
int bf_gemm_inbwd_frames_scaled(int dtype, int M, int N, int K, const void* A, int64_t lda, const void* B, int64_t ldb, const void* x,
                                const void* add, void* out, int S, const float* mean, const float* rstd, const float* w, float* ws,
                                const float* fscale, int fdiv, void* out_s, const float* f_s, int fdiv_s, hipStream_t stream);

namespace {

struct D {
    int dtype, B, T, h, w, E, heads, attn_scale, feat_scale, patch, cin, cout, nfluid;
    long N, F, S;
    int d, nst;
    size_t es;
};
int get_dims(const bf_dims* s, D* o) {
    if (!s) return bf_fail_msg("dims: null", __FILE__, __LINE__);
    o->dtype = s->dtype; o->B = s->B; o->T = s->T; o->h = s->h; o->w = s->w; o->E = s->E; o->heads = s->heads;
    o->attn_scale = s->attn_scale; o->feat_scale = s->feat_scale; o->patch = s->patch; o->cin = s->cin; o->cout = s->cout;
    o->nfluid = s->nfluid;
    if (o->B < 1 || o->T < 1 || o->h < 1 || o->w < 1 || o->E < 8 || o->E > 1024 || o->heads < 1 || o->E % o->heads)
        return bf_fail_msg("dims: bad sizes", __FILE__, __LINE__);
    if (o->dtype != BF_DTYPE_F32 && o->dtype != BF_DTYPE_BF16) return bf_fail_msg("dims: bad dtype", __FILE__, __LINE__);
    o->F = (long)o->B * o->T; o->S = (long)o->h * o->w; o->N = o->F * o->S; o->d = o->E / o->heads;
    o->es = bf_esize(o->dtype);
    const int ch = o->dtype == BF_DTYPE_BF16 ? 8 : 4;
    if (o->E % ch || o->d % ch) return bf_fail_msg("dims: E and head dim must be multiples of the 16-byte chunk", __FILE__, __LINE__);
    if (o->T > 128 || o->h > 128 || o->w > 128) return bf_fail_msg("dims: attention axes are limited to 128 tokens", __FILE__, __LINE__);
    o->nst = 0;
    if (o->patch > 0) {
        int p = o->patch;
        while (p > 1) { if (p & 1) return bf_fail_msg("dims: patch must be a power of two", __FILE__, __LINE__); p >>= 1; o->nst++; }
        if (o->nst < 1 || o->nst > BF_MAX_STAGES) return bf_fail_msg("dims: patch size out of range", __FILE__, __LINE__);
        if (o->nst > 1 && (o->E / 4) % ch) return bf_fail_msg("dims: E/4 must be a multiple of the 16-byte chunk", __FILE__, __LINE__);
    }
    return 0;
}

struct Arena {
    char* base; size_t off;
    explicit Arena(void* p) : base((char*)p), off(0) {}
    void* take(size_t bytes) { void* r = base ? base + off : nullptr; off += (bytes + 255) & ~(size_t)255; return r; }
    float* f32(size_t n) { return (float*)take(n * 4); }
};

bf_operand op_plain(const void* p, long ld, int layout) {
    bf_operand o; memset(&o, 0, sizeof(o)); o.p = p; o.ld = ld; o.layout = layout; return o;
}
void op_affine(bf_operand& o, int pro, const float* sc, const float* sh, long rpf, int nch) {
    o.pro = pro; o.sc = sc; o.sh = sh; o.rows_per_frame = (int)rpf; o.nch = nch;
}
void op_gather(bf_operand& o, int gw, int gh, int C) { o.gw = gw; o.gh = gh; o.gc = C; o.seglen = 2 * C; o.segstride = 2L * gw * C; }
bf_epilogue epi_store(void* c, long ldc) { bf_epilogue e; memset(&e, 0, sizeof(e)); e.c = c; e.ldc = ldc; e.out_mode = BF_OUT_STORE; return e; }
bf_epilogue epi_atomic(float* c, long ldc) { bf_epilogue e = epi_store(c, ldc); e.out_mode = BF_OUT_ATOMIC_F32; return e; }
void epi_scatter(bf_epilogue& e, int gw, int gh, int C) { e.gw = gw; e.gh = gh; e.gc = C; e.seglen = 2 * C; e.segstride = 2L * gw * C; }

int splitk_for(int M, int N, long K) {
    const long tiles = (long)bf_cdiv(M, 128) * bf_cdiv(N, 128);
    static const long target = bf_knob("BF_SPLITK_TARGET", 256);
    long s = (target + tiles / 2) / tiles;
    const long kt = (K + 63) / 64;
    if (s > kt / 4) s = kt / 4;
    if (s < 1) s = 1;
    return (int)s;
}

#define TRY(x) do { int rc__ = (x); if (rc__) return rc__; } while (0)
#define ZERO(ptr, bytes) do { hipError_t e__ = hipMemsetAsync((ptr), 0, (bytes), st); if (e__ != hipSuccess) return bf_fail(e__, __FILE__, __LINE__); } while (0)
#define ZERO_ON(stream, ptr, bytes) do { hipError_t e__ = hipMemsetAsync((ptr), 0, (bytes), (stream)); if (e__ != hipSuccess) return bf_fail(e__, __FILE__, __LINE__); } while (0)
#define HIP_TRY(x) do { hipError_t e__ = (x); if (e__ != hipSuccess) return bf_fail(e__, __FILE__, __LINE__); } while (0)

struct SideStream { hipStream_t st = nullptr; hipEvent_t fork = nullptr, join = nullptr, tail[2] = {nullptr, nullptr}; bool failed = false; bool pending[2] = {false, false}; };
bool g_side_defer = false;

struct NextHead { bool armed = false; const float *w = nullptr, *b = nullptr; float *mean = nullptr, *rstd = nullptr, *sc = nullptr, *sh = nullptr; void* xn = nullptr; const void* saved = nullptr; };
struct NextTail { bool armed = false; const bf_spatial_params* p = nullptr; const void* saved = nullptr; bool drop = false; };
struct NextScale { const float* f = nullptr; int fdiv = 1; };
struct StageHints { bool prepared = false; NextHead head; NextTail tail; NextScale scale; };

struct ReduceJobs {
    static constexpr int IN_CAP = 6, ATTN_CAP = 4;
    int n_in = 0, n_attn = 0; InReduceJob in[IN_CAP]; AttnReduceJob at[ATTN_CAP];
    bool at_follows[ATTN_CAP] = {};
    bool fits(const ReduceJobs& o) const { return n_in + o.n_in <= IN_CAP && n_attn + o.n_attn <= ATTN_CAP; }
    int push(const InReduceJob& j) { BF_REQUIRE(n_in < IN_CAP, "ReduceJobs: more InstanceNorm reductions than one launch holds"); in[n_in++] = j; return 0; }
    int push(const AttnReduceJob& j) { BF_REQUIRE(n_attn < ATTN_CAP, "ReduceJobs: more attention reductions than one launch holds"); at[n_attn++] = j; return 0; }
};

struct TrunkLinks {
    StageHints hints;
    StageHints take_hints() { const StageHints h = hints; hints = StageHints{}; return h; }
    struct HeadDone { const void* saved = nullptr; hipStream_t st = nullptr; } head_done;
    struct TailDone { const void* saved = nullptr; const void* dx = nullptr; float* ws = nullptr; hipStream_t st = nullptr; } tail_done;
    struct DbrReady { const void* dx = nullptr; const float* f = nullptr; void* buf = nullptr; hipStream_t st = nullptr; } dbr_ready;
    int scratch_parity = 0; bool tail_ws_flip = false, dbr_flip = false;
    bool take_head_done(const void* saved, hipStream_t st) { const bool hit = head_done.saved == saved && head_done.st == st; head_done = HeadDone{}; return hit; }
    struct { ReduceJobs jobs; bool on = false; hipStream_t st = nullptr; } reduce;
    hipEvent_t handoff = nullptr;
    SideStream side;
    std::vector<const void*> embed_lean;

    SideStream* side_stream() {
        static const bool enabled = bf_knob("BF_SIDE_STREAM", 1) != 0;
        if (!enabled) return nullptr;
        SideStream& s = side;
        if (!s.st && !s.failed) {
            int lo = 0, hi = 0;
            (void)hipDeviceGetStreamPriorityRange(&lo, &hi);
            const unsigned ef = hipEventDisableTiming | hipEventDisableSystemFence;
            if (hipStreamCreateWithPriority(&s.st, hipStreamNonBlocking, lo) != hipSuccess || hipEventCreateWithFlags(&s.fork, ef) != hipSuccess ||
                hipEventCreateWithFlags(&s.join, ef) != hipSuccess || hipEventCreateWithFlags(&s.tail[0], ef) != hipSuccess ||
                hipEventCreateWithFlags(&s.tail[1], ef) != hipSuccess) { s.failed = true; s.st = nullptr; }
        }
        return s.st ? &s : nullptr;
    }
    int hand_over(hipStream_t from, hipStream_t to) {
        if (from == to) return 0;
        if (!handoff) HIP_TRY(hipEventCreateWithFlags(&handoff, hipEventDisableTiming));
        HIP_TRY(hipEventRecord(handoff, from));
        HIP_TRY(hipStreamWaitEvent(to, handoff, 0));
        return 0;
    }
    void clear(bool forward_side) {
        if (forward_side) { hints.prepared = false; hints.head = NextHead{}; head_done = HeadDone{}; }
        hints.tail = NextTail{}; hints.scale = NextScale{}; tail_done = TailDone{}; dbr_ready = DbrReady{};
    }
    bool embed_lean_get(const void* saved) const { return std::find(embed_lean.begin(), embed_lean.end(), saved) != embed_lean.end(); }
    void embed_lean_set(const void* saved, bool lean) {
        const auto it = std::find(embed_lean.begin(), embed_lean.end(), saved);
        if (it == embed_lean.end()) { if (lean) embed_lean.push_back(saved); }
        else if (!lean) { *it = embed_lean.back(); embed_lean.pop_back(); }
    }
};
BfPerDevice<TrunkLinks> g_links;

int launch_reduce_jobs(ReduceJobs& J, hipStream_t st);
int flush_pending_reduce(TrunkLinks& L, hipStream_t st) {
    if (!L.reduce.on) return 0;
    L.reduce.on = false;
    TRY(launch_reduce_jobs(L.reduce.jobs, L.reduce.st));
    return L.hand_over(L.reduce.st, st);
}
int launch_with_pending(TrunkLinks& L, ReduceJobs& J, hipStream_t st) {
    if (L.reduce.on && L.reduce.st == st && J.fits(L.reduce.jobs)) {
        L.reduce.on = false;
        const ReduceJobs& P = L.reduce.jobs;
        for (int i = 0; i < P.n_in; ++i) TRY(J.push(P.in[i]));
        for (int i = 0; i < P.n_attn; ++i) TRY(J.push(P.at[i]));
    }
    TRY(flush_pending_reduce(L, st));
    return launch_reduce_jobs(J, st);
}
int side_join_pending(TrunkLinks& L, hipStream_t main, int set = -1) {
    if (set < 0) TRY(flush_pending_reduce(L, main));
    SideStream* s = L.side_stream();
    if (set < 0 && bf_gemm_tokred_pending()) {
        hipStream_t ws_st = s ? s->st : main;
        TRY(bf_gemm_tokred_flush(ws_st));
        if (s) { HIP_TRY(hipEventRecord(s->join, s->st)); HIP_TRY(hipStreamWaitEvent(main, s->join, 0)); }
    }
    if (!s) return 0;
    for (int i = 0; i < 2; ++i)
        if ((set < 0 || set == i) && s->pending[i]) {
            HIP_TRY(hipStreamWaitEvent(main, s->tail[i], 0));
            s->pending[i] = false;
        }
    return 0;
}
struct Fork {
    hipStream_t main; SideStream* s; bool used = false; bool deferred; int set;
    std::vector<std::function<int(hipStream_t)>> jobs;
    std::vector<std::function<int(hipStream_t)>> late;
    hipStream_t last_side = nullptr;
    explicit Fork(TrunkLinks& L, hipStream_t m, bool may_defer = false, int scratch_set = 0) : main(m), s(L.side_stream()), set(scratch_set) {
        deferred = may_defer && g_side_defer && s != nullptr;
    }
    int begin(hipStream_t* out) {
        *out = main;
        if (!s) return 0;
        HIP_TRY(hipEventRecord(s->fork, main));
        HIP_TRY(hipStreamWaitEvent(s->st, s->fork, 0));
        used = true;
        *out = s->st;
        return 0;
    }
    template <class F> int run(F&& job) {
        hipStream_t ss;
        const int rc = begin(&ss);
        last_side = ss;
        return rc ? rc : job(ss);
    }
    template <class F> void run_late(F&& job) { late.push_back(job); }
    int drain_late() {
        if (late.empty()) return 0;
        hipStream_t ss = last_side ? last_side : main;
        for (auto& j : late) TRY(j(ss));
        late.clear();
        return 0;
    }
    int flush() {
        if (!deferred || jobs.empty()) return 0;
        hipStream_t ss;
        TRY(begin(&ss));
        for (auto& j : jobs) TRY(j(ss));
        jobs.clear();
        return 0;
    }
    int join() {
        if (deferred) {
            TRY(flush());
            TRY(drain_late());
            if (used) { HIP_TRY(hipEventRecord(s->tail[set], s->st)); s->pending[set] = true; used = false; }
            return 0;
        }
        TRY(drain_late());
        if (bf_gemm_tokred_pending()) TRY(bf_gemm_tokred_flush(last_side ? last_side : main));
        if (!s || !used) return 0;
        HIP_TRY(hipEventRecord(s->join, s->st));
        HIP_TRY(hipStreamWaitEvent(main, s->join, 0));
        used = false;
        return 0;
    }
};

struct PrepArgs { const float *W, *bias, *nb, *gamma, *lo, *hi; float *alpha, *beta, *mc; int E; void* wscaled; int dtype;
                  const float *tab_m, *tab_v; float* tab_out; int tab_F;
                  const float* tr_src; void* tr_dst; int tr_R, tr_C; };
__device__ __forceinline__ void outproj_prep_row(const float* __restrict__ W, const float* __restrict__ bias, const float* __restrict__ nb,
                                                 const float* __restrict__ gamma, const float* __restrict__ lo, const float* __restrict__ hi,
                                                 float* __restrict__ alpha, float* __restrict__ beta, float* __restrict__ mc, int E, int n,
                                                 void* __restrict__ wscaled, int dtype) {
    __shared__ float red[4];
    __shared__ float s_alpha;
    float acc = 0.f;
    if (lo) for (int k = threadIdx.x; k < E; k += blockDim.x) acc += W[(long)n * E + k] * nb[k];
    acc = wave_sum(acc);
    if ((threadIdx.x & 63) == 0) red[threadIdx.x >> 6] = acc;
    __syncthreads();
    if (threadIdx.x == 0) {
        float m = bias[n];
        for (int i = 0; i < (int)(blockDim.x >> 6); ++i) m += red[i];
        const float l = lo ? lo[n] : 0.f, h = hi ? hi[n] : 0.f, g = gamma[n];
        alpha[n] = g * (1.f + h);
        beta[n] = g * (bias[n] * (1.f + h) + (lo ? m * (l - h) : 0.f));
        mc[n] = m;
        s_alpha = g * (1.f + h);
    }
    if (wscaled) {
        __syncthreads();
        const float al = s_alpha;
        for (int k = threadIdx.x; k < E; k += blockDim.x) {
            const float v = al * W[(long)n * E + k];
            if (dtype == BF_DTYPE_BF16) reinterpret_cast<bf16*>(wscaled)[(long)n * E + k] = (bf16)v;
            else reinterpret_cast<float*>(wscaled)[(long)n * E + k] = v;
        }
    }
}
__global__ void __launch_bounds__(256) outproj_prep_kernel(PrepArgs a) {
    outproj_prep_row(a.W, a.bias, a.nb, a.gamma, a.lo, a.hi, a.alpha, a.beta, a.mc, a.E, blockIdx.x, a.wscaled, a.dtype);
}
__global__ void outproj_finalize_kernel(const float* __restrict__ G, const float* __restrict__ csum, const float* __restrict__ W,
                                        const float* __restrict__ bias, const float* __restrict__ nb, const float* __restrict__ gamma,
                                        const float* __restrict__ lo, const float* __restrict__ hi, const float* __restrict__ mc,
                                        float* __restrict__ dW, float* __restrict__ dbias, float* __restrict__ dnb, float* __restrict__ dgamma,
                                        float* __restrict__ dlo, float* __restrict__ dhi, int E) {
    __shared__ float red[4];
    __shared__ float s_dmc, s_alpha;
    if ((int)blockIdx.x >= E) {
        __shared__ float part[16][16];
        __shared__ float coef[1024];
        for (int n = threadIdx.x; n < E; n += blockDim.x) coef[n] = csum[n] * gamma[n] * (lo[n] - hi[n]);
        __syncthreads();
        const int c = threadIdx.x & 15, k = ((int)blockIdx.x - E) * 16 + c, q = threadIdx.x >> 4;
        float a = 0.f;
        if (k < E) {
            int n = q;
            for (; n + 112 < E; n += 128) {
                float wv[8];
#pragma unroll
                for (int u = 0; u < 8; ++u) wv[u] = W[(long)(n + 16 * u) * E + k];
#pragma unroll
                for (int u = 0; u < 8; ++u) a = fmaf(coef[n + 16 * u], wv[u], a);
            }
            for (; n < E; n += 16) a = fmaf(coef[n], W[(long)n * E + k], a);
        }
        part[q][c] = a;
        __syncthreads();
        if (q == 0 && k < E) {
            float t = 0.f;
#pragma unroll
            for (int i = 0; i < 16; ++i) t += part[i][c];
            atomicAdd(dnb + k, t);
        }
        return;
    }
// ... 214 lines not shown
        ones = a.f32((size_t)4 * d.E);
        wg = a.f32(wgn);
        tokred_floats = bf_gemm_tokred_ws_floats(4 * d.E, d.E, d.N);
        tokred_ws = a.f32((size_t)tokred_floats);
        attn_ws = a.f32(ATTN_WS_FLOATS);
        attn_ws2 = a.f32(ATTN_WS_FLOATS);
        {
            int64_t n = bf_in_ws_floats(d.dtype, (int)d.F, (int)d.S, d.E);
            long Si = d.S;
            for (int i = 1; i < d.nst; ++i) { Si *= 4; n = std::max(n, bf_in_ws_floats(d.dtype, (int)d.F, (int)Si, cm)); }
            in_ws = a.f32((size_t)n);
            const size_t nt = (size_t)bf_in_ws_floats(d.dtype, (int)d.F, (int)d.S, d.E);
            in_ws2 = a.f32(nt); in_ws3 = a.f32(nt); in_ws4 = a.f32(nt); in_ws5 = a.f32(nt);
        }
        size_t tok = (size_t)d.N * d.E;
        size_t big = tok * 4;
        if (d.patch > 1) {
            const size_t P0 = (size_t)d.N * (d.patch / 2) * (d.patch / 2);
            const int kp = ((4 * std::max(d.cin, d.cout) + 7) / 8) * 8;
            big = std::max(big, P0 * (size_t)std::max(cm, kp) * 2);
        }
        t4 = a.take(big * d.es);
        t3 = a.take(std::max(tok * 3, big / 2) * d.es);
        t1 = a.take(std::max(tok, big / 2) * d.es);
        t1b = a.take(std::max(tok, big / 2) * d.es);
        t1b_floats = (int64_t)(std::max(tok, big / 2) * d.es / 4);
        s1 = a.take(tok * d.es); e5 = a.take(tok * d.es); e6 = a.take(tok * d.es); e7 = a.take(tok * d.es);
        bytes = a.off;
    }
};

__global__ void __launch_bounds__(64 * BF_RED_FL) stage_param_reduce_kernel(ReduceJobs J) {
    __shared__ float red[5][BF_RED_FL][64];
    const int z = blockIdx.z;
    if (z < J.n_in) {
        const InReduceJob& j = J.in[z];
        if ((int)blockIdx.x < (j.C + 63) / 64 && (int)blockIdx.y < (j.frames + j.rdiv() - 1) / j.rdiv()) in_reduce_block(j, blockIdx.x, blockIdx.y, red);
    } else {
        int a = z - J.n_in;
        if (J.at_follows[a]) return;
        for (;; ++a) {
            const AttnReduceJob& j = J.at[a];
            const int nvals = 4 * j.D + 32 * j.heads + j.heads;
            if ((int)blockIdx.x < (nvals + 63) / 64 && blockIdx.y == 0) attn_reduce_block(j, blockIdx.x, 0, 1, red);
            if (a + 1 >= J.n_attn || !J.at_follows[a + 1]) break;
            __syncthreads();
        }
    }
}
int launch_reduce_jobs(ReduceJobs& J, hipStream_t st) {
    int k = 0;
    for (int i = 0; i < J.n_attn; ++i) if (J.at[i].rows > 0) J.at[k++] = J.at[i];
    J.n_attn = k;
    for (int i = 0; i < J.n_attn; ++i)
        J.at_follows[i] = i > 0 && J.at[i].D == J.at[i - 1].D && J.at[i].heads == J.at[i - 1].heads &&
                          ((J.at[i].dqw && J.at[i].dqw == J.at[i - 1].dqw) || (J.at[i].demb && J.at[i].demb == J.at[i - 1].demb));
    if (J.n_in + J.n_attn == 0) return 0;
    int gx = 1, gy = 1;
    for (int i = 0; i < J.n_in; ++i) { gx = std::max(gx, bf_cdiv(J.in[i].C, 64)); gy = std::max(gy, bf_cdiv(J.in[i].frames, J.in[i].rdiv())); }
    for (int i = 0; i < J.n_attn; ++i) { gx = std::max(gx, bf_cdiv(4 * J.at[i].D + 33 * J.at[i].heads, 64)); }
    hipLaunchKernelGGL(stage_param_reduce_kernel, dim3(gx, gy, J.n_in + J.n_attn), dim3(64 * BF_RED_FL), 0, st, J);
    BF_CHECK_LAUNCH();
    return 0;
}

int qkv_gemm(const D& d, const void* xn, const void* w_c, const float* bias, void* qkv, hipStream_t st) {
    bf_operand A = op_plain(xn, d.E, BF_LAY_KC);
    bf_operand Bo = op_plain(w_c, d.E, BF_LAY_KC);
    bf_epilogue e = epi_store(qkv, 3L * d.E);
    e.bias = bias;
    return bf_gemm(d.dtype, (int)d.N, 3 * d.E, d.E, &A, &Bo, &e, 1, st);
}
int outproj_gemm(const D& d, const void* on, const void* w_c, const float* alpha, const float* beta,
                 const void* resid, void* out, const float* drop, long rows_per_group, hipStream_t st) {
    bf_operand A = op_plain(on, d.E, BF_LAY_KC);
    bf_operand Bo = op_plain(w_c, d.E, BF_LAY_KC);
    bf_epilogue e = epi_store(out, d.E);
    e.colscale = alpha; e.colshift = beta; e.aux_mode = BF_AUX_ADD; e.aux = resid; e.ld_aux = d.E;
    e.rowscale = drop; e.rows_per_group = (int)rows_per_group;
    return bf_gemm(d.dtype, (int)d.N, d.E, d.E, &A, &Bo, &e, 1, st);
}
void* bwd_scratch(TrunkLinks& L, const D& d, void* scratch) {
    if (!g_side_defer || !L.side_stream()) return scratch;
    L.scratch_parity ^= 1;
    return (char*)scratch + (size_t)L.scratch_parity * Scratch(d, nullptr).bytes;
}
struct TailNorm { const void* z; void* dz; const float *mean, *rstd, *w, *g; int gdiv; float* ws; bool* done; };
struct InFuse { const void* x; const void* add; void* dx; const float* mean; const float* rstd; const float* w; const float* b; float* ws;
                const float* fscale = nullptr; int fdiv = 1;
                const TailNorm* tail = nullptr;
                void* scaled_out = nullptr; const float* scaled_f = nullptr; int scaled_fdiv = 1; bool* scaled_done = nullptr; };
int dgrad_inbwd(const D& d, const void* dy, int Kdim, const void* w_xc, int Nout, void* tmp, const InFuse& f, hipStream_t st) {
    if (f.tail) {
        const TailNorm& t = *f.tail;
        const int crc = bf_gemm_inbwd_frames_chain(d.dtype, (int)d.N, Nout, Kdim, dy, Kdim, w_xc, Nout, f.x, f.add, f.dx, (int)d.S, f.mean, f.rstd, f.w, f.ws,
                                                   f.fscale, f.fdiv, t.z, t.dz, t.mean, t.rstd, t.w, t.g, t.gdiv, t.ws, st);
        if (crc < 0) return crc;
        if (crc == 0) { *t.done = true; return 0; }
    }
    if (f.scaled_out) {
        const int src = bf_gemm_inbwd_frames_scaled(d.dtype, (int)d.N, Nout, Kdim, dy, Kdim, w_xc, Nout, f.x, f.add, f.dx, (int)d.S, f.mean, f.rstd, f.w, f.ws,
                                                    f.fscale, f.fdiv, f.scaled_out, f.scaled_f, f.scaled_fdiv, st);
        if (src < 0) return src;
        if (src == 0) { *f.scaled_done = true; return 0; }
    }
    const int rc = bf_gemm_inbwd_frames(d.dtype, (int)d.N, Nout, Kdim, dy, Kdim, w_xc, Nout, f.x, f.add, f.dx, (int)d.S, f.mean, f.rstd, f.w, f.ws,
                                        f.fscale, f.fdiv, st);
    if (rc <= 0) return rc;
    bf_operand A = op_plain(dy, Kdim, BF_LAY_KC);
    bf_operand Bo = op_plain(w_xc, Nout, BF_LAY_XC);
    bf_epilogue e = epi_store(tmp, Nout);
    if (f.fscale) { e.rowscale = f.fscale; e.rows_per_group = (int)(d.S * f.fdiv); }
    TRY(bf_gemm(d.dtype, (int)d.N, Nout, Kdim, &A, &Bo, &e, 1, st));
    return bf_in_bwd_partials(d.dtype, tmp, f.x, f.add, f.dx, (int)d.F, (int)d.S, Nout, f.mean, f.rstd, f.w, f.b, nullptr, 1, 0, f.ws, st);
}
int outproj_bwd(const D& d, const Scratch& sc, const void* dout, const void* on, const void* w_s,
                const float* W, const float* bias, const float* nb, const float* gamma, const float* lo, const float* hi,
                const float* alpha, const float* mc, float* dW, float* dbias, float* dnb, float* dgamma, float* dlo, float* dhi,
                void* don, hipStream_t st, Fork& fk, const InFuse* fu = nullptr) {
    TRY(fk.run([=](hipStream_t ss) -> int {
        const void* dsrc = dout;
        const int trc = bf_gemm_tokred_deferred(d.dtype, d.E, d.E, d.N, dsrc, d.E, on, d.E, sc.G, 0, sc.csum, sc.tokred_ws, sc.tokred_floats, ss);
        if (trc < 0) return trc;
        if (trc == 1) {
            ZERO_ON(ss, sc.G, (size_t)((char*)sc.csum - (char*)sc.G) + (size_t)d.E * 4);
            bf_operand A = op_plain(dsrc, d.E, BF_LAY_XC);
            bf_operand Bo = op_plain(on, d.E, BF_LAY_XC);
            bf_epilogue e = epi_atomic(sc.G, d.E);
            e.colsum = sc.csum;
            TRY(bf_gemm(d.dtype, d.E, d.E, (int)d.N, &A, &Bo, &e, splitk_for(d.E, d.E, d.N), ss));
        }
        return 0;
    }));
    fk.run_late([=](hipStream_t ss) -> int {
        if (bf_gemm_tokred_pending_out() == sc.G) TRY(bf_gemm_tokred_flush(ss));
        hipLaunchKernelGGL(outproj_finalize_kernel, dim3(d.E + (lo ? bf_cdiv(d.E, 16) : 0)), dim3(256), 0, ss, sc.G, sc.csum, W, bias, nb, gamma, lo, hi, mc,
                           dW, dbias, dnb, dgamma, dlo, dhi, d.E);
        BF_CHECK_LAUNCH();
        return 0;
    });
    if (fu) return dgrad_inbwd(d, dout, d.E, w_s, d.E, don, *fu, st);
    {
        bf_operand A = op_plain(dout, d.E, BF_LAY_KC);
        bf_operand Bo = op_plain(w_s, d.E, BF_LAY_XC);
        bf_epilogue e = epi_store(don, d.E);
        TRY(bf_gemm(d.dtype, (int)d.N, d.E, d.E, &A, &Bo, &e, 1, st));
    }
    return 0;
}
int linear_bwd(const D& d, const Scratch& sc, const void* dy, int Nout, const void* x, int Kin, int xpro, const float* xsc, const float* xsh,
               const void* w_c, float* dW, float* db, void* dxn, const bf_epilogue* dx_epi, hipStream_t st, Fork& fk, const InFuse* fu = nullptr,
               bool last = false, const void* w_t = nullptr, void* scaled_out = nullptr, const float* rowfac = nullptr, int rpg = 1,
               bool* scaled_done = nullptr) {
    TRY(fk.run([=](hipStream_t ss) -> int {
        const void* xo = x;
        int pro = xpro;
        bf_operand A = op_plain(dy, Nout, BF_LAY_XC);
        if (pro == BF_PRO_AFFINE) {
            TRY(bf_affine_apply(d.dtype, x, nullptr, xsc, xsh, sc.s1, d.N, (int)d.S, Kin, ss));
            xo = sc.s1;
            pro = BF_PRO_NONE;
        }
        bf_operand Bo = op_plain(xo, Kin, BF_LAY_XC);
        if (pro == BF_PRO_NONE) {
            const int trc = bf_gemm_tokred_deferred(d.dtype, Nout, Kin, d.N, dy, Nout, xo, Kin, dW, 1, db, sc.tokred_ws, sc.tokred_floats, ss);
            if (trc <= 0) return trc;
        }
        if (pro != BF_PRO_NONE) op_affine(Bo, pro, xsc, xsh, d.S, Kin);
        bf_epilogue e = epi_atomic(dW, Kin);
        e.colsum = db;
        return bf_gemm(d.dtype, Nout, Kin, (int)d.N, &A, &Bo, &e, splitk_for(Nout, Kin, d.N), ss);
    }));
    if (last) TRY(fk.flush());
    if (fu) return dgrad_inbwd(d, dy, Nout, w_c, Kin, dxn, *fu, st);
    {
        bf_operand A = op_plain(dy, Nout, BF_LAY_KC);
        bf_operand Bo = w_t ? op_plain(w_t, Nout, BF_LAY_KC) : op_plain(w_c, Kin, BF_LAY_XC);
        bf_epilogue e = dx_epi ? *dx_epi : epi_store(dxn, Kin);
        e.c = dxn; e.ldc = Kin;
        if (scaled_out && rowfac && d.dtype == BF_DTYPE_BF16) {
            const int rc = bf_gemm_pair_scaled((int)d.N, Kin, Nout, &A, &Bo, &e, scaled_out, rowfac, rpg, st);
            if (rc < 0) return rc;
            if (rc == 0) { if (scaled_done) *scaled_done = true; return 0; }
        }
        TRY(bf_gemm(d.dtype, (int)d.N, Kin, Nout, &A, &Bo, &e, 1, st));
    }
    return 0;
}

}

extern "C" int64_t bf_temporal_saved_bytes(const bf_dims* s) { D d; if (get_dims(s, &d)) return -1; return (int64_t)TemporalSaved(d, nullptr).bytes; }
extern "C" int64_t bf_spatial_saved_bytes(const bf_dims* s) { D d; if (get_dims(s, &d)) return -1; return (int64_t)SpatialSaved(d, nullptr).bytes; }
size_t dbr_bytes(const D& d) { return (((size_t)d.N * d.E * d.es) + 255) & ~(size_t)255; }
extern "C" int64_t bf_scratch_bytes(const bf_dims* s) { D d; if (get_dims(s, &d)) return -1; return 2 * (int64_t)Scratch(d, nullptr).bytes + 2 * (int64_t)dbr_bytes(d); }

extern "C" void bf_side_defer(int on) { g_side_defer = on != 0; }
extern "C" int bf_side_join(bf_stream_t s) { return side_join_pending(g_links.get(), (hipStream_t)s); }

extern "C" void bf_stage_prepared(int on) { g_links.get().hints.prepared = on != 0; }
extern "C" int bf_stage_chain_tail(const bf_spatial_params* prev_p, const void* prev_saved, int has_drop_mlp) {
    g_links.get().hints.tail = NextTail{prev_p && prev_saved, prev_p, prev_saved, has_drop_mlp != 0};
    return 0;
}
extern "C" int bf_stage_next_scale(const float* factors, int fdiv) { g_links.get().hints.scale = NextScale{factors, fdiv > 0 ? fdiv : 1}; return 0; }
static NextHead next_head(const D& d, int kind, const void* params, void* saved) {
    auto of = [&](auto* np, const auto& sv) { return NextHead{true, np->norm1_w, np->norm1_b, sv.mean1, sv.rstd1, sv.sc1, sv.sh1, sv.xn, saved}; };
    return kind == 0 ? of((const bf_temporal_params*)params, TemporalSaved(d, saved)) : of((const bf_spatial_params*)params, SpatialSaved(d, saved));
}
extern "C" int bf_stage_chain_next(const bf_dims* dims, int next_kind, const void* next_params, void* next_saved) {
    NextHead& h = g_links.get().hints.head;
    h = NextHead{};
    if (!dims || !next_params || !next_saved) return 0;
    BF_REQUIRE(next_kind == 0 || next_kind == 1, "bf_stage_chain_next: kind must be 0 (temporal) or 1 (spatial)");
    D d; TRY(get_dims(dims, &d));
    h = next_head(d, next_kind, next_params, next_saved);
    return 0;
}
extern "C" int bf_stage_chain_head(const bf_dims* dims, const bf_temporal_params* next_p, void* next_saved) {
    return bf_stage_chain_next(dims, 0, next_p, next_saved);
}

static int temporal_fwd(TrunkLinks& L, const StageHints& H, const bf_dims* dims, const bf_temporal_params* p, const void* x, void* out, void* saved,
                        void* scratch, const float* drop, bf_stream_t s) {
    D d; TRY(get_dims(dims, &d));
    BF_REQUIRE(p && x && out && saved && scratch, "bf_temporal_fwd: null pointer");
    hipStream_t st = (hipStream_t)s;
    const bool head_done = L.take_head_done(saved, st);
    TRY(side_join_pending(L, st));
    TemporalSaved sv(d, saved);
    Scratch sc(d, scratch);
    const void *win_c, *wout_c;
    {
        const float* src[2] = {p->input_head_w, p->output_head_w};
        void* dst[2] = {sv.win_c, sv.wout_c};
        const long n[2] = {3L * d.E * d.E, (long)d.E * d.E};
        const void* out[4];
        const bool b16 = d.dtype == BF_DTYPE_BF16;
        const PrepArgs prep{p->output_head_w, p->output_head_b, p->norm2_b, p->gamma, nullptr, nullptr, sv.alpha, sv.beta, sv.mc, d.E, sv.wout_s, d.dtype,
                            nullptr, nullptr, nullptr, 0, b16 ? p->output_head_w : nullptr, b16 ? sv.wout_t : nullptr, d.E, d.E};
        const bool ready = H.prepared && d.dtype == BF_DTYPE_BF16;
        if (ready) { out[0] = sv.win_c; out[1] = sv.wout_c; }
        else TRY(wviews(d, 2, src, dst, n, out, st, &prep));
        win_c = out[0]; wout_c = out[1];
    }
    if (!head_done)
        TRY(bf_in_stats_apply(d.dtype, x, (int)d.F, (int)d.S, d.E, p->norm1_w, p->norm1_b, nullptr, 1, nullptr, sv.mean1, sv.rstd1, sv.sc1, sv.sh1, sc.in_ws,
                              nullptr, sv.xn, st));
    TRY(qkv_gemm(d, sv.xn, win_c, p->input_head_b, sv.qkv, st));
    TRY(bf_attn_fwd(d.dtype, sv.qkv, sv.o, (long)d.B * d.S, d.T, d.S, (long)d.T * d.S, 1, d.S, d.heads, d.d, p->qnorm_w, p->qnorm_b,
                    p->knorm_w, p->knorm_b, p->rel_pos_emb, d.attn_scale ? p->attn_scale_factor : nullptr, 1.f, 0, st));
    TRY(bf_in_stats_apply(d.dtype, sv.o, (int)d.F, (int)d.S, d.E, p->norm2_w, p->norm2_b, nullptr, 1, nullptr, sv.mean2, sv.rstd2, sv.sc2, sv.sh2, sc.in_ws,
                          nullptr, sv.on, st));
    if (H.head.armed) {
        const NextHead& h = H.head;
        const bf_frame_norm n2{h.w, h.b, nullptr, 1, h.mean, h.rstd, h.sc, h.sh, nullptr, h.xn};
        const int rc = bf_gemm_fwd_frames(d.dtype, (int)d.N, d.E, d.E, sv.on, d.E, sv.wout_t, d.E, nullptr, sv.alpha, sv.beta, drop, d.T, x, out, (int)d.S,
                                          nullptr, &n2, s);
        if (rc < 0) return rc;
        if (rc == 0) { L.head_done = {h.saved, st}; return 0; }
    }
    TRY(outproj_gemm(d, sv.on, wout_c, sv.alpha, sv.beta, x, out, drop, (long)d.T * d.S, st));
    return 0;
}

static int temporal_bwd(TrunkLinks& L, const StageHints& H, const bf_dims* dims, const bf_temporal_params* p, const bf_temporal_params* g, const void* x,
                        const void* dout, void* dx, void* saved, void* scratch, const float* drop, bf_stream_t s) {
    D d; TRY(get_dims(dims, &d));
    BF_REQUIRE(p && g && x && dout && dx && saved && scratch, "bf_temporal_bwd: null pointer");
    hipStream_t st = (hipStream_t)s;
    TemporalSaved sv(d, saved);
    Scratch sc(d, bwd_scratch(L, d, scratch));
    const void* win_c = d.dtype == BF_DTYPE_F32 ? (const void*)p->input_head_w : sv.win_c;
    Fork fk(L, st, true, L.scratch_parity);
    if (fk.deferred) TRY(side_join_pending(L, st, fk.set));
    void* don = sc.t1;
    void* dO = sc.t1b;
    void* dqkv = sc.t3;
    const void* dbr = dout;
    if (drop) {
        const TrunkLinks::DbrReady& r = L.dbr_ready;
        if (r.dx == dout && r.f == drop && r.buf && r.st == st) dbr = r.buf;
        else {
            TRY(bf_frame_scale(d.dtype, dout, drop, d.T, sc.t4, d.N, (int)d.S, d.E, st));
            dbr = sc.t4;
        }
    }
    L.dbr_ready = TrunkLinks::DbrReady{};
    const InFuse fu2{sv.o, nullptr, dO, sv.mean2, sv.rstd2, p->norm2_w, p->norm2_b, sc.in_ws2};
    TRY(outproj_bwd(d, sc, dbr, sv.on, sv.wout_s, p->output_head_w, p->output_head_b, p->norm2_b, p->gamma, nullptr, nullptr,
                    sv.alpha, sv.mc, g->output_head_w, g->output_head_b, nullptr, g->gamma, nullptr, nullptr, don, st, fk, &fu2));
    ReduceJobs jobs;
    TRY(jobs.push(InReduceJob{sc.in_ws2, (int)d.F, d.E, p->norm2_w, p->norm2_b, nullptr, 1, g->norm2_w, g->norm2_b, nullptr, nullptr, nullptr, nullptr}));
    {
        int rows = 0;
        TRY(bf_attn_bwd_partials(d.dtype, sv.qkv, dO, dqkv, (long)d.B * d.S, d.T, d.S, (long)d.T * d.S, 1, d.S, d.heads, d.d, p->qnorm_w, p->qnorm_b,
                                 p->knorm_w, p->knorm_b, p->rel_pos_emb, d.attn_scale ? p->attn_scale_factor : nullptr, g->qnorm_w, g->qnorm_b,
                                 g->knorm_w, g->knorm_b, g->rel_pos_emb, d.attn_scale ? g->attn_scale_factor : nullptr, 1.f, 0, sc.attn_ws,
                                 Scratch::ATTN_WS_FLOATS, &rows, st));
        TRY(jobs.push(AttnReduceJob{sc.attn_ws, rows, d.d, d.heads, g->qnorm_w, g->qnorm_b, g->knorm_w, g->knorm_b, g->rel_pos_emb,
                                    d.attn_scale ? g->attn_scale_factor : nullptr}));
    }
    void* dxn = sc.t1;
    InFuse fu1{x, dout, dx, sv.mean1, sv.rstd1, p->norm1_w, p->norm1_b, sc.in_ws};
    TailNorm tn;
    bool tail_done = false;
    static const bool chain_on = bf_knob("BF_BWD_CHAIN", 1) != 0;
    if (H.tail.armed && chain_on && fk.deferred && d.dtype == BF_DTYPE_BF16 && d.S == 144 && d.F % 2 == 0) {
        const NextTail& h = H.tail;
        const int oset = L.scratch_parity ^ 1;
        TRY(side_join_pending(L, st, oset));
        Scratch so(d, (char*)scratch + (size_t)oset * Scratch(d, nullptr).bytes);
        SpatialSaved ps(d, const_cast<void*>(h.saved));
        tn = TailNorm{ps.z, so.t1, ps.mean3, ps.rstd3, h.p->mlp_norm_w, h.drop ? ps.gtab : h.p->gamma_mlp, h.drop ? 1 : (int)d.F, L.tail_ws_flip ? so.in_ws5 : so.in_ws4, &tail_done};
        L.tail_ws_flip = !L.tail_ws_flip;
        fu1.tail = &tn;
    }
    if (H.tail.armed) L.tail_done = TrunkLinks::TailDone{};
    TRY(linear_bwd(d, sc, dqkv, 3 * d.E, sv.xn, d.E, BF_PRO_NONE, nullptr, nullptr, win_c, g->input_head_w, g->input_head_b, dxn, nullptr, st, fk, &fu1, true));
    if (tail_done) L.tail_done = {H.tail.saved, dx, tn.ws, st};
    TRY(jobs.push(InReduceJob{sc.in_ws, (int)d.F, d.E, p->norm1_w, p->norm1_b, nullptr, 1, g->norm1_w, g->norm1_b, nullptr, nullptr, nullptr, nullptr}));
    TRY(launch_with_pending(L, jobs, st));
    return fk.join();
}
extern "C" int bf_temporal_fwd(const bf_dims* dims, const bf_temporal_params* p, const void* x, void* out, void* saved, void* scratch,
                               const float* drop, bf_stream_t s) {
    TrunkLinks& L = g_links.get();
    return temporal_fwd(L, L.take_hints(), dims, p, x, out, saved, scratch, drop, s);
}
extern "C" int bf_temporal_bwd(const bf_dims* dims, const bf_temporal_params* p, const bf_temporal_params* g, const void* x, const void* dout,
                               void* dx, void* saved, void* scratch, const float* drop, bf_stream_t s) {
    TrunkLinks& L = g_links.get();
    return temporal_bwd(L, L.take_hints(), dims, p, g, x, dout, dx, saved, scratch, drop, s);
}

static int prep_stages(TrunkLinks& L, const bf_dims* dims, int n, const int32_t* kinds, const void* const* params, void* const* saved,
                       const float* const* drop_mlp, bf_stream_t s) {
    D d; TRY(get_dims(dims, &d));
    BF_REQUIRE(n >= 1 && kinds && params && saved, "bf_prep_stages: bad arguments");
    if (d.dtype != BF_DTYPE_BF16) return 1;
    hipStream_t st = (hipStream_t)s;
    TRY(side_join_pending(L, st));
    for (int i0 = 0; i0 < n; i0 += PREP_BATCH) {
        PrepBatch b;
        memset(&b, 0, sizeof(b));
        const int m = std::min(PREP_BATCH, n - i0);
        for (int i = 0; i < m; ++i) {
            BF_REQUIRE(params[i0 + i] && saved[i0 + i] && (kinds[i0 + i] == 0 || kinds[i0 + i] == 1), "bf_prep_stages: bad stage entry");
            Cast4& j = b.j[i];
            if (kinds[i0 + i] == 0) {
                const bf_temporal_params* p = (const bf_temporal_params*)params[i0 + i];
                TemporalSaved sv(d, saved[i0 + i]);
                const float* src[2] = {p->input_head_w, p->output_head_w};
                void* dst[2] = {sv.win_c, sv.wout_c};
                const long cn[2] = {3L * d.E * d.E, (long)d.E * d.E};
                for (int q = 0; q < 4; ++q) { j.src[q] = src[q < 2 ? q : 0]; j.dst[q] = (bf16*)dst[q < 2 ? q : 0]; j.n[q] = q < 2 ? cn[q] : 0; }
                b.cnt[i] = 2;
                b.a[i] = PrepArgs{p->output_head_w, p->output_head_b, p->norm2_b, p->gamma, nullptr, nullptr, sv.alpha, sv.beta, sv.mc, d.E, sv.wout_s, d.dtype,
                                  nullptr, nullptr, nullptr, 0, p->output_head_w, sv.wout_t, d.E, d.E};
            } else {
                const bf_spatial_params* p = (const bf_spatial_params*)params[i0 + i];
                SpatialSaved sv(d, saved[i0 + i]);
                const float* src[4] = {p->input_head_w, p->output_head_w, p->fc1_w, p->fc2_w};
                void* dst[4] = {sv.win_c, sv.wout_c, sv.w1_c, sv.w2_c};
                const long cn[4] = {3L * d.E * d.E, (long)d.E * d.E, 4L * d.E * d.E, 4L * d.E * d.E};
                for (int q = 0; q < 4; ++q) { j.src[q] = src[q]; j.dst[q] = (bf16*)dst[q]; j.n[q] = cn[q]; }
                b.cnt[i] = 4;
                const float* dm = drop_mlp ? drop_mlp[i0 + i] : nullptr;
                b.a[i] = PrepArgs{p->output_head_w, p->output_head_b, p->norm2_b, p->gamma_att, d.feat_scale ? p->low_freq_scalar : nullptr,
                                  d.feat_scale ? p->high_freq_scalar : nullptr, sv.alpha, sv.beta, sv.mc, d.E, sv.wout_s, d.dtype,
                                  dm, dm ? p->gamma_mlp : nullptr, dm ? sv.gtab : nullptr, (int)d.F,
                                  p->fc2_w, sv.w2t_c, d.E, 4 * d.E};
            }
        }
        hipLaunchKernelGGL(stage_prep_multi_kernel, dim3(std::max(64, d.E), 7, m), dim3(256), 0, st, b);
        BF_CHECK_LAUNCH();
    }
    return 0;
}
extern "C" int bf_prep_stages(const bf_dims* dims, int n, const int32_t* kinds, const void* const* params, void* const* saved,
                              const float* const* drop_mlp, bf_stream_t s) {
    return prep_stages(g_links.get(), dims, n, kinds, params, saved, drop_mlp, s);
}

static int spatial_fwd(TrunkLinks& L, const StageHints& H, const bf_dims* dims, const bf_spatial_params* p, const void* x, void* out, void* saved,
                       void* scratch, const float* drop_att, const float* drop_mlp, bf_stream_t s) {
    D d; TRY(get_dims(dims, &d));
    BF_REQUIRE(p && x && out && saved && scratch, "bf_spatial_fwd: null pointer");
    hipStream_t st = (hipStream_t)s;
    const bool head_done = L.take_head_done(saved, st);
    TRY(side_join_pending(L, st));
    SpatialSaved sv(d, saved);
    Scratch sc(d, scratch);
// ... 12 lines not shown
        if (ready) { out[0] = sv.win_c; out[1] = sv.wout_c; out[2] = sv.w1_c; out[3] = sv.w2_c; }
        else TRY(wviews(d, 4, src, dst, n, out, st, &prep));
        win_c = out[0]; wout_c = out[1]; w1_c = out[2]; w2_c = out[3];
    }
    if (!head_done)
        TRY(bf_in_stats_apply(d.dtype, x, (int)d.F, (int)d.S, d.E, p->norm1_w, p->norm1_b, nullptr, 1, nullptr, sv.mean1, sv.rstd1, sv.sc1, sv.sh1, sc.in_ws,
                              nullptr, sv.xn, st));
    TRY(qkv_gemm(d, sv.xn, win_c, p->input_head_b, sv.qkv, st));
    {
        const int rc = bf_attn_axial_norm_fwd(d.dtype, sv.qkv, sv.o, sv.on, d.F, (int)d.h, (int)d.w, d.heads, d.d, p->qnorm_w, p->qnorm_b, p->knorm_w,
                                              p->knorm_b, p->rel_pos_emb, d.attn_scale ? p->attn_scale_factor_x : nullptr,
                                              d.attn_scale ? p->attn_scale_factor_y : nullptr, p->norm2_w, p->norm2_b, sv.mean2, sv.rstd2, sv.sc2,
                                              sv.sh2, st);
        if (rc < 0) return rc;
        if (rc == 1) {
            TRY(bf_attn_axial_fwd(d.dtype, sv.qkv, sv.o, d.F, (int)d.h, (int)d.w, d.heads, d.d, p->qnorm_w, p->qnorm_b, p->knorm_w, p->knorm_b,
                                  p->rel_pos_emb, d.attn_scale ? p->attn_scale_factor_x : nullptr, d.attn_scale ? p->attn_scale_factor_y : nullptr, st));
            TRY(bf_in_stats_apply(d.dtype, sv.o, (int)d.F, (int)d.S, d.E, p->norm2_w, p->norm2_b, nullptr, 1, nullptr, sv.mean2, sv.rstd2, sv.sc2, sv.sh2,
                                  sc.in_ws, nullptr, sv.on, st));
        }
    }
    TRY(outproj_gemm(d, sv.on, wout_c, sv.alpha, sv.beta, x, sv.x1, drop_att, d.S, st));
    {
        bf_operand A = op_plain(sv.x1, d.E, BF_LAY_KC);
        bf_operand Bo = op_plain(w1_c, d.E, BF_LAY_KC);
        bf_epilogue e = epi_store(sv.pre, 4L * d.E);
        e.bias = p->fc1_b;
        e.gelu_out = sv.hid;
        TRY(bf_gemm(d.dtype, (int)d.N, 4 * d.E, d.E, &A, &Bo, &e, 1, st));
    }
    const float* g3 = p->gamma_mlp;
    int g3div = (int)d.F;
    if (drop_mlp) {
        if (d.dtype == BF_DTYPE_F32) {
            hipLaunchKernelGGL(frame_table_kernel, dim3(bf_cdiv(d.F * d.E, 256)), dim3(256), 0, st, drop_mlp, 1, (const float*)p->gamma_mlp, sv.gtab, (int)d.F, d.E);
            BF_CHECK_LAUNCH();
        }
        g3 = sv.gtab; g3div = 1;
    }
    if (d.dtype == BF_DTYPE_BF16) {
        const bf_frame_norm n1{p->mlp_norm_w, p->mlp_norm_b, g3, g3div, sv.mean3, sv.rstd3, sv.sc3, sv.sh3, sv.x1, out};
        const NextHead& h = H.head;
        const bf_frame_norm n2{h.w, h.b, nullptr, 1, h.mean, h.rstd, h.sc, h.sh, nullptr, h.xn};
        const int rc = bf_gemm_fwd_frames(d.dtype, (int)d.N, d.E, 4 * d.E, sv.hid, 4L * d.E, sv.w2t_c, d.E, p->fc2_b, nullptr, nullptr, nullptr, 1, nullptr, sv.z,
                                          (int)d.S, &n1, h.armed ? &n2 : nullptr, s);
        if (rc < 0) return rc;
        if (rc == 0) {
            if (h.armed) L.head_done = {h.saved, st};
            return 0;
        }
    }
    {
        bf_operand A = op_plain(sv.hid, 4L * d.E, BF_LAY_KC);
        bf_operand Bo = op_plain(w2_c, 4L * d.E, BF_LAY_KC);
        bf_epilogue e = epi_store(sv.z, d.E);
        e.bias = p->fc2_b;
        TRY(bf_gemm(d.dtype, (int)d.N, d.E, 4 * d.E, &A, &Bo, &e, 1, st));
    }
    if (H.head.armed) {
        const NextHead& h = H.head;
        bool chained = false;
        TRY(bf_in_stats_apply_chain(d.dtype, sv.z, (int)d.F, (int)d.S, d.E, p->mlp_norm_w, p->mlp_norm_b, g3, g3div, nullptr, sv.mean3, sv.rstd3, sv.sc3, sv.sh3,
                                    sc.in_ws, sv.x1, out, h.w, h.b, h.mean, h.rstd, h.sc, h.sh, h.xn, &chained, st));
        if (chained) L.head_done = {h.saved, st};
        return 0;
    }
    TRY(bf_in_stats_apply(d.dtype, sv.z, (int)d.F, (int)d.S, d.E, p->mlp_norm_w, p->mlp_norm_b, g3, g3div, nullptr, sv.mean3, sv.rstd3,
                          sv.sc3, sv.sh3, sc.in_ws, sv.x1, out, st));
    return 0;
}

static int spatial_bwd(TrunkLinks& L, const StageHints& H, const bf_dims* dims, const bf_spatial_params* p, const bf_spatial_params* g, const void* x,
                       const void* dout, void* dx, void* saved, void* scratch, const float* drop_att, const float* drop_mlp, bf_stream_t s) {
    D d; TRY(get_dims(dims, &d));
    BF_REQUIRE(p && g && x && dout && dx && saved && scratch, "bf_spatial_bwd: null pointer");
    hipStream_t st = (hipStream_t)s;
    SpatialSaved sv(d, saved);
    Scratch sc(d, bwd_scratch(L, d, scratch));
    const bool f32 = d.dtype == BF_DTYPE_F32;
    const void* win_c = f32 ? (const void*)p->input_head_w : sv.win_c;
    const void* w1_c = f32 ? (const void*)p->fc1_w : sv.w1_c;
    const void* w2_c = f32 ? (const void*)p->fc2_w : sv.w2_c;
    TRY(flush_pending_reduce(L, st));
    Fork fk(L, st, true, L.scratch_parity);
    if (fk.deferred) TRY(side_join_pending(L, st, fk.set));
    void* dz = sc.t1;
    ReduceJobs jobs;
    const TrunkLinks::TailDone td = L.tail_done;
    L.tail_done = TrunkLinks::TailDone{};
    const bool tail_done = td.saved == saved && td.dx == dout && td.st == st;
    {
        const float* gsc = drop_mlp ? sv.gtab : p->gamma_mlp;
        const int gdiv = drop_mlp ? 1 : (int)d.F;
        if (!tail_done)
            TRY(bf_in_bwd_partials(d.dtype, dout, sv.z, nullptr, dz, (int)d.F, (int)d.S, d.E, sv.mean3, sv.rstd3, p->mlp_norm_w, p->mlp_norm_b, gsc, gdiv, 0, sc.in_ws3, st));
        TRY(jobs.push(InReduceJob{tail_done ? td.ws : sc.in_ws3, (int)d.F, d.E, p->mlp_norm_w, p->mlp_norm_b, gsc, gdiv, g->mlp_norm_w, g->mlp_norm_b,
                                  drop_mlp ? nullptr : g->gamma_mlp, nullptr, drop_mlp, drop_mlp ? g->gamma_mlp : nullptr}));
    }
    void* dpre = sc.t4;
    {
        bf_epilogue e; memset(&e, 0, sizeof(e));
        e.aux_mode = BF_AUX_DGELU; e.aux = sv.pre; e.ld_aux = 4L * d.E; e.out_mode = BF_OUT_STORE;
        static const bool use_t = bf_knob("BF_FC2_DGRAD_T", 1) != 0;
        TRY(linear_bwd(d, sc, dz, d.E, sv.hid, 4 * d.E, BF_PRO_NONE, nullptr, nullptr, w2_c, g->fc2_w, g->fc2_b, dpre, &e, st, fk, nullptr, false,
                       (!f32 && use_t) ? sv.w2t_c : nullptr));
    }
    void* dx1 = sc.t1b;
    bool dbr_done = false;
    {
        bf_epilogue e; memset(&e, 0, sizeof(e));
        e.aux_mode = BF_AUX_ADD; e.aux = dout; e.ld_aux = d.E; e.out_mode = BF_OUT_STORE;
        TRY(linear_bwd(d, sc, dpre, 4 * d.E, sv.x1, d.E, BF_PRO_NONE, nullptr, nullptr, w1_c, g->fc1_w, g->fc1_b, dx1, &e, st, fk, nullptr, false, nullptr,
                       drop_att ? sc.e5 : nullptr, drop_att, (int)d.S, &dbr_done));
    }
    void* don = sc.e6;
    const void* dbr = dx1;
    if (dbr_done) dbr = sc.e5;
    else if (drop_att) {
        TRY(bf_frame_scale(d.dtype, dx1, drop_att, 1, sc.e5, d.N, (int)d.S, d.E, st));
        dbr = sc.e5;
    }
    void* dO = sc.e7;
    const InFuse fu2{sv.o, nullptr, dO, sv.mean2, sv.rstd2, p->norm2_w, p->norm2_b, sc.in_ws2};
    TRY(outproj_bwd(d, sc, dbr, sv.on, sv.wout_s, p->output_head_w, p->output_head_b, p->norm2_b, p->gamma_att,
                    d.feat_scale ? p->low_freq_scalar : nullptr, d.feat_scale ? p->high_freq_scalar : nullptr, sv.alpha, sv.mc,
                    g->output_head_w, g->output_head_b, g->norm2_b, g->gamma_att, d.feat_scale ? g->low_freq_scalar : nullptr,
                    d.feat_scale ? g->high_freq_scalar : nullptr, don, st, fk, &fu2));
    TRY(jobs.push(InReduceJob{sc.in_ws2, (int)d.F, d.E, p->norm2_w, p->norm2_b, nullptr, 1, g->norm2_w, g->norm2_b, nullptr, nullptr, nullptr, nullptr}));
    void* dqkv = sc.t3;
    {
        int rows = 0;
        static const bool raw_on = bf_knob("BF_ATTN_RAW", 1) != 0;
        const bool rawm = raw_on && bf_attn_raw_modes(d.dtype, d.d);
        TRY(bf_attn_bwd_partials(d.dtype, sv.qkv, dO, dqkv, d.F * d.h, d.w, 1, d.w, 0, 1, d.heads, d.d, p->qnorm_w, p->qnorm_b, p->knorm_w, p->knorm_b,
                                 p->rel_pos_emb, d.attn_scale ? p->attn_scale_factor_x : nullptr, g->qnorm_w, g->qnorm_b, g->knorm_w, g->knorm_b,
                                 g->rel_pos_emb, d.attn_scale ? g->attn_scale_factor_x : nullptr, 0.5f, rawm ? 2 : 0, sc.attn_ws, Scratch::ATTN_WS_FLOATS, &rows, st));
        TRY(jobs.push(AttnReduceJob{sc.attn_ws, rows, d.d, d.heads, g->qnorm_w, g->qnorm_b, g->knorm_w, g->knorm_b, g->rel_pos_emb,
                                    d.attn_scale ? g->attn_scale_factor_x : nullptr}));
        TRY(bf_attn_bwd_partials(d.dtype, sv.qkv, dO, dqkv, d.F * d.w, d.h, d.w, d.S, 1, d.w, d.heads, d.d, p->qnorm_w, p->qnorm_b, p->knorm_w, p->knorm_b,
                                 p->rel_pos_emb, d.attn_scale ? p->attn_scale_factor_y : nullptr, g->qnorm_w, g->qnorm_b, g->knorm_w, g->knorm_b,
                                 g->rel_pos_emb, d.attn_scale ? g->attn_scale_factor_y : nullptr, 0.5f, rawm ? 5 : 1, sc.attn_ws2, Scratch::ATTN_WS_FLOATS, &rows, st));
        TRY(jobs.push(AttnReduceJob{sc.attn_ws2, rows, d.d, d.heads, g->qnorm_w, g->qnorm_b, g->knorm_w, g->knorm_b, g->rel_pos_emb,
                                    d.attn_scale ? g->attn_scale_factor_y : nullptr}));
    }
    void* dxn = sc.e6;
    InFuse fu1{x, dx1, dx, sv.mean1, sv.rstd1, p->norm1_w, p->norm1_b, sc.in_ws};
    bool scaled_done = false;
    const NextScale& ns = H.scale;
    L.dbr_ready = TrunkLinks::DbrReady{};
    static const bool scaled_on = bf_knob("BF_BWD_SCALED_COPY", 1) != 0;
    if (ns.f && scaled_on && fk.deferred && d.dtype == BF_DTYPE_BF16) {
        fu1.scaled_out = (char*)scratch + 2 * Scratch(d, nullptr).bytes + (L.dbr_flip ? dbr_bytes(d) : 0);
        fu1.scaled_f = ns.f; fu1.scaled_fdiv = ns.fdiv; fu1.scaled_done = &scaled_done;
    }
    TRY(linear_bwd(d, sc, dqkv, 3 * d.E, sv.xn, d.E, BF_PRO_NONE, nullptr, nullptr, win_c, g->input_head_w, g->input_head_b, dxn, nullptr, st, fk, &fu1, true));
    if (scaled_done) { L.dbr_ready = {dx, ns.f, fu1.scaled_out, st}; L.dbr_flip = !L.dbr_flip; }
    TRY(jobs.push(InReduceJob{sc.in_ws, (int)d.F, d.E, p->norm1_w, p->norm1_b, nullptr, 1, g->norm1_w, g->norm1_b, nullptr, nullptr, nullptr, nullptr}));
    static const bool merge_on = bf_knob("BF_REDUCE_MERGE", 1) != 0;
    if (fk.deferred && merge_on) { L.reduce.jobs = jobs; L.reduce.on = true; L.reduce.st = st; }
    else TRY(launch_reduce_jobs(jobs, st));
    return fk.join();
}
extern "C" int bf_spatial_fwd(const bf_dims* dims, const bf_spatial_params* p, const void* x, void* out, void* saved, void* scratch,
                              const float* drop_att, const float* drop_mlp, bf_stream_t s) {
    TrunkLinks& L = g_links.get();
    return spatial_fwd(L, L.take_hints(), dims, p, x, out, saved, scratch, drop_att, drop_mlp, s);
}
extern "C" int bf_spatial_bwd(const bf_dims* dims, const bf_spatial_params* p, const bf_spatial_params* g, const void* x, const void* dout,
                              void* dx, void* saved, void* scratch, const float* drop_att, const float* drop_mlp, bf_stream_t s) {
    TrunkLinks& L = g_links.get();
    return spatial_bwd(L, L.take_hints(), dims, p, g, x, dout, dx, saved, scratch, drop_att, drop_mlp, s);
}

extern "C" int bf_trunk_train_fwd(const bf_dims* dims, int n, const int32_t* kinds, const void* const* params, void* const* saved,
                                  const float* const* drop_a, const float* const* drop_b, const void* x, void* const* acts, void* scratch,
                                  bf_stream_t s) {
    D d; TRY(get_dims(dims, &d));
    BF_REQUIRE(n >= 1 && kinds && params && saved && x && acts && scratch, "bf_trunk_train_fwd: bad arguments");
    for (int i = 0; i < n; ++i)
        BF_REQUIRE(params[i] && saved[i] && acts[i] && (kinds[i] == 0 || kinds[i] == 1), "bf_trunk_train_fwd: bad stage entry");
    TrunkLinks& L = g_links.get();
    (void)L.take_hints();
    const bool b16 = d.dtype == BF_DTYPE_BF16;
    if (b16) {
        const int rc = prep_stages(L, dims, n, kinds, params, saved, drop_b, s);
        if (rc < 0) return rc;
    }
    for (int i = 0; i < n; ++i) {
        const void* in = i ? acts[i - 1] : x;
        StageHints H;
        H.prepared = b16;
        if (b16 && i + 1 < n && kinds[i + 1] != kinds[i]) H.head = next_head(d, kinds[i + 1], params[i + 1], saved[i + 1]);
        TRY(kinds[i] == 0
            ? temporal_fwd(L, H, dims, (const bf_temporal_params*)params[i], in, acts[i], saved[i], scratch, drop_a ? drop_a[i] : nullptr, s)
            : spatial_fwd(L, H, dims, (const bf_spatial_params*)params[i], in, acts[i], saved[i], scratch, drop_a ? drop_a[i] : nullptr,
                          drop_b ? drop_b[i] : nullptr, s));
    }
    return 0;
}

extern "C" int bf_trunk_train_bwd(const bf_dims* dims, int n, const int32_t* kinds, const void* const* params, const void* const* grads,
                                  void* const* saved, const float* const* drop_a, const float* const* drop_b, const void* x, void* const* acts,
                                  const void* dout, void* const* gbuf3, void* dx, void* scratch, bf_stage_done_fn stage_done, void* user,
                                  bf_stream_t s) {
    D d; TRY(get_dims(dims, &d));
    BF_REQUIRE(n >= 1 && kinds && params && grads && saved && x && acts && dout && gbuf3 && dx && scratch, "bf_trunk_train_bwd: bad arguments");
    BF_REQUIRE(gbuf3[0] && gbuf3[1] && gbuf3[2], "bf_trunk_train_bwd: three gradient buffers are needed");
    TrunkLinks& L = g_links.get();
    (void)L.take_hints();
    const void* cur = dout;
    int rot = 0;
    for (int i = n - 1; i >= 0; --i) {
        BF_REQUIRE(params[i] && grads[i] && saved[i] && (kinds[i] == 0 || kinds[i] == 1), "bf_trunk_train_bwd: bad stage entry");
        const void* in = i ? acts[i - 1] : x;
        void* gout = i ? gbuf3[rot] : dx;
        rot = (rot + 1) % 3;
        StageHints H;
        if (kinds[i] == 0) {
            if (i > 0 && kinds[i - 1] == 1) H.tail = NextTail{true, (const bf_spatial_params*)params[i - 1], saved[i - 1], drop_b && drop_b[i - 1]};
            TRY(temporal_bwd(L, H, dims, (const bf_temporal_params*)params[i], (const bf_temporal_params*)grads[i], in, cur, gout, saved[i], scratch,
                             drop_a ? drop_a[i] : nullptr, s));
        } else {
            if (i > 0 && kinds[i - 1] == 0 && drop_a && drop_a[i - 1]) H.scale = NextScale{drop_a[i - 1], d.T};
            TRY(spatial_bwd(L, H, dims, (const bf_spatial_params*)params[i], (const bf_spatial_params*)grads[i], in, cur, gout, saved[i], scratch,
                            drop_a ? drop_a[i] : nullptr, drop_b ? drop_b[i] : nullptr, s));
        }
        if (stage_done) stage_done(i, user);
        cur = gout;
    }
    return 0;
}

namespace {
struct EvalStage {
    void *win_c, *wout_c, *w1_c, *w2_c; float *alpha, *beta, *mc;
    size_t bytes;
    EvalStage(const D& d, int kind, void* base) {
        Arena a(base);
        alpha = a.f32(d.E); beta = a.f32(d.E); mc = a.f32(d.E);
        win_c = a.take((size_t)3 * d.E * d.E * 2);
        wout_c = a.take((size_t)d.E * d.E * 2);
        w1_c = kind == 1 ? a.take((size_t)4 * d.E * d.E * 2) : nullptr;
        w2_c = kind == 1 ? a.take((size_t)4 * d.E * d.E * 2) : nullptr;
        bytes = a.off;
    }
};
bool trunk_eval_covers(const D& d) { return d.dtype == BF_DTYPE_BF16 && d.S == 144 && d.E == 384 && d.h <= 16 && d.w <= 16 && d.T <= 32; }
}

extern "C" int64_t bf_trunk_eval_weights_bytes(const bf_dims* dims, int n, const int32_t* kinds) {
    D d; if (get_dims(dims, &d) || n < 1 || !kinds) return -1;
    int64_t t = 0;
    for (int i = 0; i < n; ++i) t += (int64_t)EvalStage(d, kinds[i], nullptr).bytes;
    return t;
}

extern "C" int bf_trunk_eval_prepare(const bf_dims* dims, int n, const int32_t* kinds, const void* const* params, void* weights, bf_stream_t s) {
    D d; TRY(get_dims(dims, &d));
    BF_REQUIRE(n >= 1 && kinds && params && weights, "bf_trunk_eval_prepare: bad arguments");
    if (!trunk_eval_covers(d)) return 1;
    hipStream_t st = (hipStream_t)s;
    char* base = (char*)weights;
    for (int i0 = 0; i0 < n; i0 += PREP_BATCH) {
        PrepBatch b;
        memset(&b, 0, sizeof(b));
        const int m = std::min(PREP_BATCH, n - i0);
        for (int i = 0; i < m; ++i) {
            BF_REQUIRE(params[i0 + i] && (kinds[i0 + i] == 0 || kinds[i0 + i] == 1), "bf_trunk_eval_prepare: bad stage entry");
            EvalStage ev(d, kinds[i0 + i], base);
            base += ev.bytes;
            Cast4& j = b.j[i];
            if (kinds[i0 + i] == 0) {
                const bf_temporal_params* p = (const bf_temporal_params*)params[i0 + i];
                const float* src[2] = {p->input_head_w, p->output_head_w};
                void* dst[2] = {ev.win_c, ev.wout_c};
                const long cn[2] = {3L * d.E * d.E, (long)d.E * d.E};
                for (int q = 0; q < 4; ++q) { j.src[q] = src[q < 2 ? q : 0]; j.dst[q] = (bf16*)dst[q < 2 ? q : 0]; j.n[q] = q < 2 ? cn[q] : 0; }
                b.cnt[i] = 2;
                b.a[i] = PrepArgs{p->output_head_w, p->output_head_b, p->norm2_b, p->gamma, nullptr, nullptr, ev.alpha, ev.beta, ev.mc, d.E, nullptr, d.dtype,
                                  nullptr, nullptr, nullptr, 0, nullptr, nullptr, 0, 0};
            } else {
                const bf_spatial_params* p = (const bf_spatial_params*)params[i0 + i];
                const float* src[4] = {p->input_head_w, p->output_head_w, p->fc1_w, p->fc2_w};
                void* dst[4] = {ev.win_c, ev.wout_c, ev.w1_c, ev.w2_c};
                const long cn[4] = {3L * d.E * d.E, (long)d.E * d.E, 4L * d.E * d.E, 4L * d.E * d.E};
                for (int q = 0; q < 4; ++q) { j.src[q] = src[q]; j.dst[q] = (bf16*)dst[q]; j.n[q] = cn[q]; }
                b.cnt[i] = 4;
                b.a[i] = PrepArgs{p->output_head_w, p->output_head_b, p->norm2_b, p->gamma_att, d.feat_scale ? p->low_freq_scalar : nullptr,
                                  d.feat_scale ? p->high_freq_scalar : nullptr, ev.alpha, ev.beta, ev.mc, d.E, nullptr, d.dtype,
                                  nullptr, nullptr, nullptr, 0, nullptr, nullptr, 0, 0};
            }
        }
        hipLaunchKernelGGL(stage_prep_multi_kernel, dim3(std::max(64, d.E), 5, m), dim3(256), 0, st, b);
        BF_CHECK_LAUNCH();
    }
    return 0;
}

extern "C" int bf_trunk_eval_fwd(const bf_dims* dims, int n, const int32_t* kinds, const void* const* params, const void* weights,
                                 const void* x, void* out, void* scratch, bf_stream_t s) {
    D d; TRY(get_dims(dims, &d));
    BF_REQUIRE(n >= 1 && kinds && params && weights && x && out && scratch, "bf_trunk_eval_fwd: bad arguments");
    if (!trunk_eval_covers(d)) return 1;
    hipStream_t st = (hipStream_t)s;
    TrunkLinks& L = g_links.get();
    TRY(side_join_pending(L, st));
    Scratch sc(d, scratch);
    const int F = (int)d.F, E = d.E;
    void *qkv = sc.t3, *o = sc.t1, *on = sc.t1b, *x1 = sc.e5, *hid = sc.t4;
    float* stat = sc.tokred_ws;
    BF_REQUIRE(sc.tokred_floats >= (int64_t)4 * F * E, "bf_trunk_eval_fwd: scratch too small");
// ... 497 lines not shown
```

### bubbleformer_amd/kernels.py

```python
import ctypes as C

import torch

from . import _lib as L
from .ops import _dt, _p, _stream


def operand(t=None, ld=0, layout=L.BF_LAY_KC, seglen=0, segstride=0, gw=0, gh=0, gc=0, pro=L.BF_PRO_NONE, sc=None, sh=None,
            rows_per_frame=0, nch=0) -> L.Operand:
    return L.Operand(_p(t), ld, layout, seglen, segstride, gw, gh, gc, pro, _p(sc), _p(sh), rows_per_frame, nch)


def epilogue(c, ldc, bias=None, colscale=None, colshift=None, aux_mode=L.BF_AUX_NONE, aux=None, ld_aux=0, out_mode=L.BF_OUT_STORE,
             seglen=0, segstride=0, gw=0, gh=0, gc=0, gelu_out=None, colsum=None, rowscale=None, rows_per_group=0) -> L.Epilogue:
    return L.Epilogue(_p(bias), _p(colscale), _p(colshift), aux_mode, _p(aux), ld_aux, out_mode, _p(c), ldc, seglen, segstride, gw, gh, gc, _p(gelu_out), _p(colsum), _p(rowscale), rows_per_group)


def gemm(dtype, M, N, K, A: L.Operand, B: L.Operand, E: L.Epilogue, splitk=1):
    L.check(L.lib().bf_gemm(_dt(dtype), M, N, K, C.byref(A), C.byref(B), C.byref(E), splitk, _stream()), "bf_gemm")


def gemm_tokred(dy, x, out, accumulate=False, colsum=None):
    M, Nout = dy.shape
    Kin = x.shape[1]
    n = L.lib().bf_gemm_tokred_ws_floats(Nout, Kin, M)
    ws = torch.empty(n, dtype=torch.float32, device=x.device)
    rc = L.lib().bf_gemm_tokred(_dt(x.dtype), Nout, Kin, M, _p(dy), dy.stride(0), _p(x), x.stride(0), _p(out), int(accumulate), _p(colsum),
                                _p(ws), n, _stream())
    if rc == 1:
        return False
    L.check(rc, "bf_gemm_tokred")
    return True


def in_stats(x, frames, S, Cc, w, b, g=None, gdiv=1, gb=None):
    dev = x.device
    mean, rstd, sc, sh = (torch.empty(frames, Cc, dtype=torch.float32, device=dev) for _ in range(4))
    ws = torch.empty(L.lib().bf_in_ws_floats(_dt(x.dtype), frames, S, Cc), dtype=torch.float32, device=dev)
    L.check(L.lib().bf_in_stats(_dt(x.dtype), _p(x), frames, S, Cc, _p(w), _p(b), _p(g), gdiv, _p(gb), _p(mean), _p(rstd), _p(sc),
                                _p(sh), _p(ws), _stream()), "bf_in_stats")
    return mean, rstd, sc, sh


def in_bwd(dy, x, frames, S, Cc, mean, rstd, w, b, add=None, g=None, gdiv=1, gelu=False, use_ws=True):
    dev = x.device
    dx = torch.empty_like(x)
    dw = torch.zeros(Cc, dtype=torch.float32, device=dev)
    db = torch.zeros(Cc, dtype=torch.float32, device=dev)
    ws = torch.empty(L.lib().bf_in_ws_floats(_dt(x.dtype), frames, S, Cc), dtype=torch.float32, device=dev) if use_ws else None
    L.check(L.lib().bf_in_bwd(_dt(x.dtype), _p(dy), _p(x), _p(add), _p(dx), frames, S, Cc, _p(mean), _p(rstd), _p(w), _p(b), _p(g), gdiv,
                              int(gelu), _p(dw), _p(db), None, None, _p(ws), _stream()), "bf_in_bwd")
    return dx, dw, db


def gemm_inbwd_frames(A, B, x, S, mean, rstd, w, add=None, fscale=None, fdiv=1):
    M, K = A.shape
    N = B.shape[1]
    out = torch.empty(M, N, dtype=x.dtype, device=x.device)
    ws = torch.zeros((M // S) * N * 2, dtype=torch.float32, device=x.device)
    rc = L.lib().bf_gemm_inbwd_frames(_dt(x.dtype), M, N, K, _p(A), A.stride(0), _p(B), B.stride(0), _p(x), _p(add), _p(out), S, _p(mean),
                                      _p(rstd), _p(w), _p(ws), _p(fscale), fdiv, _stream())
    if rc == 1:
        return None
    L.check(rc, "bf_gemm_inbwd_frames")
    return out, ws


def attn_fwd(qkv, out, nseq, Lq, inner, outer_stride, inner_stride, tok_stride, heads, d, qw, qb, kw, kb, emb, hscale, out_scale=1.0,
             accumulate=False):
    L.check(L.lib().bf_attn_fwd(_dt(qkv.dtype), _p(qkv), _p(out), nseq, Lq, inner, outer_stride, inner_stride, tok_stride, heads, d,
                                _p(qw), _p(qb), _p(kw), _p(kb), _p(emb), _p(hscale), out_scale, int(accumulate), _stream()), "bf_attn_fwd")


def check_frame_linear(A, W, frames, S, nw=None, nb=None, bias=None, colscale=None, colshift=None, resid=None, ew=None, eb=None, eg=None,
                       xw=None, xb=None) -> None:
    E = L.BubbleformerHipError
    if A.dim() != 2 or W.dim() != 2:
        raise E("frame_linear: A must be [tokens][K], W [N][K]")
    M, K = A.shape
    N = W.shape[0]
    if frames < 1 or S < 1 or frames * S != M:
        raise E(f"frame_linear: frames * tokens_per_frame = {frames} * {S} != {M} rows of A")
    if W.shape[1] != K:
        raise E(f"frame_linear: W has K = {W.shape[1]}, A has K = {K}")
    if A.dtype != torch.bfloat16 or W.dtype != torch.bfloat16:
        raise E(f"frame_linear: A and W must be bfloat16 (got {A.dtype}, {W.dtype})")
    if not A.is_cuda or W.device != A.device:
        raise E("frame_linear: A and W must be on the same ROCm device")
    if A.stride(1) != 1 or W.stride(1) != 1:
        raise E("frame_linear: A and W need unit inner strides")
    if resid is not None and (resid.shape != (M, N) or resid.dtype != torch.bfloat16 or resid.stride(1) != 1 or resid.device != A.device):
        raise E(f"frame_linear: resid must be a bfloat16 [{M}][{N}] tensor with a unit inner stride on {A.device}")
    for name, t, n in (("norm weight", nw, K), ("norm bias", nb, K), ("bias", bias, N), ("colscale", colscale, N), ("colshift", colshift, N),
                       ("out_norm weight", ew, N), ("out_norm bias", eb, N), ("out_norm scale", eg, N), ("next_norm weight", xw, N),
                       ("next_norm bias", xb, N)):
        if t is None:
            continue
        if t.dtype != torch.float32 or not t.is_contiguous() or t.numel() < n or t.device != A.device:
            raise E(f"frame_linear: {name} must be a contiguous fp32 tensor of at least {n} elements on {A.device}")
    if (nw is None) != (nb is None) or (colscale is None) != (colshift is None) or (xw is None) != (xb is None):
        raise E("frame_linear: norm / colscale+colshift / next_norm tables come in pairs")
    if ew is not None and (eb is None or eg is None):
        raise E("frame_linear: out_norm needs (weight, bias, scale)")


def frame_linear(A, W, frames, S, norm=None, bias=None, colscale=None, colshift=None, resid=None, gelu=False, out_norm=None, next_norm=None):
    nw, nb = norm if norm is not None else (None, None)
    ew, eb, eg = out_norm if out_norm is not None else (None, None, None)
    xw, xb = next_norm if next_norm is not None else (None, None)
    check_frame_linear(A, W, frames, S, nw, nb, bias, colscale, colshift, resid, ew, eb, eg, xw, xb)
    M, K = A.shape
    N = W.shape[0]
    out = torch.empty(M, N, dtype=A.dtype, device=A.device)
    out_n = torch.empty_like(out) if next_norm is not None else None
# ... 8 lines not shown
```

### include/bubbleformer_hip.h

```cpp
#ifndef BUBBLEFORMER_HIP_H
#define BUBBLEFORMER_HIP_H

#include <stdint.h>

#ifdef __cplusplus
extern "C" {
#endif

typedef void* bf_stream_t;

enum { BF_DTYPE_F32 = 0, BF_DTYPE_BF16 = 1 };

enum { BF_LAY_KC = 0,
       BF_LAY_XC = 1   };
enum { BF_PRO_NONE = 0, BF_PRO_AFFINE = 1, BF_PRO_AFFINE_GELU = 2, BF_PRO_GELU = 3 };
enum { BF_AUX_NONE = 0, BF_AUX_ADD = 1 , BF_AUX_DGELU = 2  };
enum { BF_OUT_STORE = 0 , BF_OUT_ATOMIC_F32 = 2 ,
       BF_OUT_STORE_F32 = 1  };

typedef struct bf_operand {
    const void* p;
    int64_t ld;
    int32_t layout;
    int32_t seglen;
// ... 14 lines not shown
    const void* aux;
    int64_t ld_aux;
    int32_t out_mode;
    void* c;
    int64_t ldc;
    int32_t seglen;
    int64_t segstride;
    int32_t gw, gh, gc;
    void* gelu_out;
    float* colsum;
    const float* rowscale;
    int32_t rows_per_group;
} bf_epilogue;

int bf_gemm(int dtype, int M, int N, int K, const bf_operand* A, const bf_operand* B, const bf_epilogue* E,
            int splitk, bf_stream_t stream);

int bf_gemm_inbwd_frames(int dtype, int M, int N, int K, const void* A, int64_t lda, const void* B, int64_t ldb, const void* x,
                         const void* add, void* out, int S, const float* mean, const float* rstd, const float* w, float* ws,
                         const float* fscale , int fdiv,
                         bf_stream_t stream);
int bf_gemm_inbwd_frames_chain(int dtype, int M, int N, int K, const void* A, int64_t lda, const void* B, int64_t ldb, const void* x,
                               const void* add, void* out, int S, const float* mean, const float* rstd, const float* w, float* ws,
                               const float* fscale, int fdiv, const void* cz, void* cdz, const float* cmean, const float* crstd,
                               const float* cw, const float* cg, int cgdiv, float* cws, bf_stream_t stream);

typedef struct bf_frame_norm {
    const float *w, *b;
    const float* g; int32_t gdiv;
    float *mean, *rstd, *sc, *sh;
    const void* resid;
    void* out;
} bf_frame_norm;
int bf_gemm_fwd_frames(int dtype, int M, int N, int K, const void* A, int64_t lda, const void* Bt, int64_t ldb, const float* bias,
                       const float* colscale, const float* colshift, const float* fscale, int fdiv, const void* add, void* out, int S,
                       const bf_frame_norm* n1, const bf_frame_norm* n2, bf_stream_t stream);

int bf_gemm_tokred(int dtype, int Nout, int Kin, int64_t M, const void* dy, int64_t ldy, const void* x, int64_t ldx, float* out,
                   int accumulate, float* colsum, float* ws, int64_t ws_floats, bf_stream_t stream);
int64_t bf_gemm_tokred_ws_floats(int Nout, int Kin, int64_t M);

int bf_frame_linear(int dtype, int frames, int S, int K, int N, const void* A, int64_t lda, const void* W, int64_t ldw,
                    const float* norm_w, const float* norm_b, const float* bias, const float* colscale, const float* colshift,
                    const void* resid, int64_t ldr, int gelu, const float* en_w, const float* en_b, const float* en_g,
                    void* out, int64_t ldo,
                    const float* next_w, const float* next_b, void* out_n, int64_t ldn,
                    bf_stream_t stream);


int bf_in_stats(int dtype, const void* x, int frames, int S, int C, const float* w, const float* b, const float* g, int gdiv,
                const float* gb, float* mean, float* rstd, float* sc, float* sh,
                float* ws ,
                bf_stream_t stream);
int64_t bf_in_ws_floats(int dtype, int frames, int S, int C);
int bf_affine_apply(int dtype, const void* z, const void* resid, const float* sc, const float* sh, void* out, int64_t nrows,
                    int S, int C, bf_stream_t stream);
int bf_in_bwd(int dtype, const void* dy, const void* x, const void* add, void* dx, int frames, int S, int C, const float* mean,
              const float* rstd, const float* w, const float* b, const float* g, int gdiv, int gelu, float* dw, float* db,
              float* dg, float* dgb, float* ws ,
              bf_stream_t stream);
int bf_colsum(int dtype, const void* x, int64_t nrows, int C, const float* scale, float* out, bf_stream_t stream);

int bf_attn_fwd(int dtype, const void* qkv, void* out, int64_t nseq, int L, int64_t inner, int64_t outer_stride,
                int64_t inner_stride, int64_t tok_stride, int heads, int d, const float* qw, const float* qb, const float* kw,
                const float* kb, const float* emb, const float* hscale, float out_scale, int accumulate, bf_stream_t stream);
int bf_attn_axial_fwd(int dtype, const void* qkv, void* out, int64_t frames, int h, int w, int heads, int d, const float* qw,
                      const float* qb, const float* kw, const float* kb, const float* emb, const float* hscale_x,
                      const float* hscale_y, bf_stream_t stream);
int bf_attn_axial_norm_fwd(int dtype, const void* qkv, void* out, void* out_n, int64_t frames, int h, int w, int heads, int d,
                           const float* qw, const float* qb, const float* kw, const float* kb, const float* emb, const float* hscale_x,
                           const float* hscale_y, const float* norm_w, const float* norm_b, float* mean, float* rstd, float* sc,
                           float* sh, bf_stream_t stream);
int bf_attn_bwd(int dtype, const void* qkv, const void* dout, void* dqkv, int64_t nseq, int L, int64_t inner,
                int64_t outer_stride, int64_t inner_stride, int64_t tok_stride, int heads, int d, const float* qw,
                const float* qb, const float* kw, const float* kb, const float* emb, const float* hscale, float* dqw,
                float* dqb, float* dkw, float* dkb, float* demb, float* dhscale, float out_scale, int accumulate,
                float* ws, int64_t ws_floats,
                bf_stream_t stream);

void bf_side_defer(int on);
int bf_side_join(bf_stream_t stream);
void bf_debug_force_generic_attn(int on);
void bf_debug_tokred_fold(int on);

int bf_im2col_nchw(int dtype, const float* x, void* out, int frames, int C, int H, int W, int Kp, bf_stream_t stream);
int bf_col2im_nchw(int dtype, const void* g, float* dx, int frames, int C, int H, int W, int Kp, bf_stream_t stream);
#define BF_LOSS_LIMBS 5
int bf_pm2nchw(const float* pm, float* pred, const float* y, float* lossbuf, int frames, int Co, int h, int w, int Np,
               bf_stream_t stream);
int bf_debed_last(int dtype, const void* act, const float* sc, const float* sh, const void* wc, float* pred, const float* y,
                  float* lossbuf, int frames, int Ci, int Co, int h, int w, int Np, bf_stream_t stream);
int bf_debed_last_bwd(int dtype, const float* dpred, const float* pred, const float* y, const float* coef, const float* gscale,
                      const void* wc, void* dpm, void* dact, int frames, int Ci, int Co, int h, int w, int Np, bf_stream_t stream);
int bf_debed_last_bwd_norm(int dtype, const float* dpred, const float* pred, const float* y, const float* coef, const float* gscale,
                           const void* wc, void* dpm, const void* ymap, const float* mean, const float* rstd, const float* in_w,
                           const float* in_b, void* dx, float* d_in_w, float* d_in_b, int frames, int Ci, int Co, int h, int w, int Np,
                           float* ws, int64_t ws_floats, bf_stream_t stream);
int bf_embed_first(int dtype, const float* x, const void* wc, void* patches, void* y0, int frames, int C0, int cin, int h2, int w2,
                   int Kp, float* stat_part, bf_stream_t stream);
int bf_in_stats_merge_slices(int dtype, int frames, int S, int C, int rows, const float* w, const float* b, const float* g, int gdiv,
                             const float* gb, float* mean, float* rstd, float* sc, float* sh, float* ws, bf_stream_t stream);
int bf_gather_gemm(int dtype, const void* map, const void* w, int w_kn, const float* sc, const float* sh, void* out, int frames, int gh,
                   int gw, int C0, int N, bf_stream_t stream);
int bf_scatter_gemm(int dtype, const void* a, const void* w, int w_kn, const float* sc, const float* sh, void* map, float* stat_part, int frames,
                    int gh, int gw, int K, int C0, bf_stream_t stream);
int64_t bf_gather_wgrad_ws_floats(int frames, int gh, int gw);
int bf_gather_wgrad(int dtype, const void* fine, const void* coarse, const float* fsc, const float* fsh, const float* csc, const float* csh,
                    float* out, int transposed, int frames, int gh, int gw, int C0, int Kc, float* ws, int64_t ws_floats, bf_stream_t stream);
int bf_gather_gemm_rebuilt(int dtype, const void* patches, const void* w0c, const void* w, int w_kn, const float* sc, const float* sh, void* out,
                           int frames, int gh, int gw, int C0, int N, bf_stream_t stream);
int bf_gather_wgrad_rebuilt(int dtype, const void* patches, const void* w0c, const void* coarse, const float* fsc, const float* fsh, float* out,
                            int transposed, int frames, int gh, int gw, int C0, int Kc, float* ws, int64_t ws_floats, bf_stream_t stream);
int64_t bf_embed_tail_ws_floats(int frames, int gh1, int gw1, int C0, int Kp);
int bf_embed_tail_bwd(int dtype, const void* dy1, const void* w1c, const void* y0, const void* patches, const void* w0c, const float* sc,
                      const float* sh, const float* mean, const float* rstd, const float* in_w, float* dwprep, float* d_in_w, float* d_in_b,
                      int frames, int gh1, int gw1, int C1, int C0, int Kp, float* ws, int64_t ws_floats, bf_stream_t stream);
int bf_lploss_finalize(const float* lossbuf, int frames, int Co, float* loss, float* coef, bf_stream_t stream);
int bf_nchw2pm(int dtype, const float* dpred, const float* pred, const float* y, const float* coef, const float* gscale,
               void* dpm, int frames, int Co, int h, int w, int Np, bf_stream_t stream);
int bf_wprep(int dtype, int mode, const float* src, void* dst, int R, int K, int Kp, bf_stream_t stream);
int bf_wgrad_unprep(int mode, const float* gsrc, float* gdst, int R, int K, int Kp, int transposed, bf_stream_t stream);
int bf_film_net_fwd(const float* cond, const float* lnw, const float* lnb, const float* W, const float* bias, float* gb,
                    float* chat, float* crstd, int B, int P, int E2, bf_stream_t stream);
int bf_film_net_bwd(const float* dgb, const float* chat, const float* lnw, const float* lnb, const float* W, float* dW,
                    float* dbias, float* dlnw, float* dlnb, int B, int P, int E2, bf_stream_t stream);
int bf_adamw(float* p, const float* g, float* m, float* v, int64_t n, int step, float lr, float beta1, float beta2, float eps,
             float wd, float gscale, bf_stream_t stream);
int bf_adam(float* p, const float* g, float* m, float* v, int64_t n, int step, float lr, float beta1, float beta2, float eps,
            float wd, float gscale, bf_stream_t stream);
int bf_clip_gather(const float* src, int64_t field_stride, const int32_t* field, const int64_t* first, int t0, const float* diff,
                   const float* div, float* out, int B, int T, int C, int H, int W, int Ho, int Wo, bf_stream_t stream);
int bf_clip_gather_batch(const float* src, int64_t field_stride, const int64_t* idx, int64_t nsamples, const int64_t* first_tab, const int32_t* in_field,
                         const float* in_diff, const float* in_div, int Cin, int Tin, float* in_out, const int32_t* out_field,
                         const float* out_diff, const float* out_div, int Cout, int Tout, float* out_out, const float* fluid_tab,
                         const int64_t* file_tab, int P, float* fluid_out, int B, int H, int W, int Ho, int Wo, bf_stream_t stream);
int64_t bf_field_stats_ws_doubles(int nseg);
int bf_field_stats(const float* src, const int64_t* seg_begin, const int64_t* seg_len, int nseg, double* out, double* ws, bf_stream_t stream);
int bf_eikonal_sum(const float* phi, int64_t frames, int H, int W, float dx, double* out, bf_stream_t stream);
int bf_eikonal_l1_frames(const float* phi, int64_t frames, int H, int W, float dx, float* out, bf_stream_t stream);
int bf_heatflux_rows(const float* dfun, const float* temp, int64_t frames, int64_t frame_stride, int W, float x_min, float dx,
                     float heater_temp, float lc, float* flux, bf_stream_t stream);
int64_t bf_rollout_score_ws_doubles(int B, int T, int C, int Ho, int Wo);
int bf_rollout_score(const float* pred, const float* frames, int64_t field_stride, int64_t total_frames, int nfields, const int64_t* first,
                     int32_t* step, const int32_t* field, const float* diff, const float* div, int sdf_channel, float dx, float* rel_l2,
                     float* criterion, float* eik_pred, float* eik_tgt, float* next_in, float* archive, double* ws, int64_t ws_doubles,
                     int B, int T, int C, int H, int W, int Ho, int Wo, int steps, bf_stream_t stream);
int bf_rollout_heatflux(const float* pred, const float* frames, int64_t field_stride, int64_t total_frames, int nfields, const int64_t* first,
                        const int32_t* step, const int32_t* field, const float* diff, const float* div, int dfun_channel, int temp_channel,
                        const float* heater_temp, float x_min, float dx, float lc, float conductivity, float* flux_pred, float* flux_tgt,
                        int B, int T, int C, int H, int W, int Ho, int Wo, int steps, bf_stream_t stream);
int64_t bf_kde_kl_ws_doubles(int R, int64_t n, int64_t m, int points);
int bf_kde_kl(const double* p, const double* q, int R, int64_t n, int64_t m, int points, double eps, double* kl, double* x, double* pdf_p,
              double* pdf_q, double* ws, int64_t ws_doubles, bf_stream_t stream);
int64_t bf_bubble_census_lds_cells(void);
int64_t bf_bubble_census_ws_bytes(int64_t frames, int H, int W, int max_bubbles);
int bf_bubble_census(const float* phi, int64_t frames, int H, int W, int connectivity, int max_bubbles, int32_t* count, int32_t* vapour_cells,
                     int32_t* attached, int32_t* area, float* centroid, unsigned char* on_heater, int32_t* labels, void* ws, int64_t ws_bytes,
                     bf_stream_t stream);
int bf_rollout_bubbles(const float* pred, const float* frames, int64_t field_stride, int64_t total_frames, int nfields, const int64_t* first,
                       const int32_t* step, const int32_t* field, const float* diff, const float* div, int sdf_channel, int connectivity,
                       int max_bubbles, int32_t* count_pred, int32_t* count_tgt, int32_t* cells_pred, int32_t* cells_tgt, int32_t* attached_pred,
                       int32_t* attached_tgt, int32_t* area_pred, int32_t* area_tgt, void* ws, int64_t ws_bytes, int B, int T, int C, int H, int W,
                       int Ho, int Wo, int steps, bf_stream_t stream);
int64_t bf_lp_rows_ws_doubles(int64_t rows, int64_t n);
int bf_lp_rows_fwd(const float* pred, const float* y, int64_t rows, int64_t n, double p, float* ratio, double* sums, double* ws, int64_t ws_doubles,
                   bf_stream_t stream);
// ... 136 lines not shown
```

Baseline: 815.5 samples/s.

## Group weight-gradient GEMMs into one launch and deepen side-stream overlap in backward

Adds a grouped token-reduction kernel that computes up to four weight-gradient GEMMs in one launch. It accumulates slices in registers and writes the outputs directly, so the slab workspace and the separate reduce pass go away. The backward side stream grows from two to four scratch sets and several streams, deferred stage-done reporting lets more wgrad work overlap the main chain, and the grid size of the dgelu stream GEMM and the attention backward can be capped while side work runs. The cost is more scratch memory and more complex synchronisation, with a risk of contention between the main and side streams.

```diff
diff --git a/bubbleformer_amd/_lib.py b/bubbleformer_amd/_lib.py
--- a/bubbleformer_amd/_lib.py
+++ b/bubbleformer_amd/_lib.py
@@ -80,6 +80,9 @@
     "bf_prof_enable": (None, [C.c_int]),
     "bf_debug_force_generic_attn": (None, [C.c_int]),
     "bf_debug_tokred_fold": (None, [C.c_int]),
+    "bf_debug_tokred_group": (None, [C.c_int]),
+    "bf_debug_tokred_group_run": (C.c_int, [C.c_int, C.c_int, C.POINTER(C.c_int32), C.POINTER(C.c_int32), i64, C.POINTER(vp), C.POINTER(i64), C.POINTER(vp),
+                                            C.POINTER(i64), C.POINTER(vp), C.POINTER(C.c_int32), C.POINTER(vp), vp]),
     "bf_side_defer": (None, [C.c_int]),
     "bf_prep_stages": (C.c_int, [C.POINTER(Dims), C.c_int, C.POINTER(C.c_int32), C.POINTER(vp), C.POINTER(vp), C.POINTER(vp), vp]),
     "bf_stage_prepared": (None, [C.c_int]),
diff --git a/bubbleformer_amd/csrc/attn_mfma.hip b/bubbleformer_amd/csrc/attn_mfma.hip
--- a/bubbleformer_amd/csrc/attn_mfma.hip
+++ b/bubbleformer_amd/csrc/attn_mfma.hip
@@ -918,7 +918,8 @@
         if (bpc > 0) per_cu = bpc;
         resident = cus * per_cu;
     }
-    long grid = std::min<long>((nprob + wpb - 1) / wpb, (long)resident);
+    const int want = bf_bwd_grid().attn_bwd;
+    long grid = std::min<long>((nprob + wpb - 1) / wpb, want > 0 ? std::min<long>(want, resident) : (long)resident);
     {
         long a = wpb, b = heads;
         while (b) { const long t = a % b; a = b; b = t; }
diff --git a/bubbleformer_amd/csrc/bf_common.h b/bubbleformer_amd/csrc/bf_common.h
--- a/bubbleformer_amd/csrc/bf_common.h
+++ b/bubbleformer_amd/csrc/bf_common.h
@@ -49,6 +49,11 @@
 
 int bf_gemm_slabs(int dtype, int M, int N, int K, const bf_operand* A, const bf_operand* B, float* out, long ldc, int accumulate, int splitk,
                   float* ws, long ws_floats, hipStream_t st);
+struct BfBwdGrid { int stream_dgelu = 0, attn_bwd = 0; };
+BfBwdGrid& bf_bwd_grid();
+struct BfTokredJob { int Nout, Kin; int64_t M; const void* dy; int64_t ldy; const void* x; int64_t ldx; float* out; int accumulate; float* colsum; };
+bool bf_gemm_tokred_group_covers(int dtype, int Nout, int Kin, int64_t M);
+int bf_gemm_tokred_group(int dtype, int n, const BfTokredJob* jobs, hipStream_t stream);
 int bf_tokred_narrow(int dtype, int C, int64_t P, const void* wide, const void* narrow, float* out, int ldo, int accumulate, int transposed,
                      const float* sc, const float* sh, int64_t rows_per_frame, float* ws, int64_t ws_floats, hipStream_t st);
 int bf_gemm_pair_scaled(int M, int N, int K, const bf_operand* A, const bf_operand* B, const bf_epilogue* E, void* out2, const float* rowfac,
diff --git a/bubbleformer_amd/csrc/gemm_stream.hip b/bubbleformer_amd/csrc/gemm_stream.hip
--- a/bubbleformer_amd/csrc/gemm_stream.hip
+++ b/bubbleformer_amd/csrc/gemm_stream.hip
@@ -515,6 +515,8 @@
 }
 
 }
+
+BfBwdGrid& bf_bwd_grid() { static thread_local BfBwdGrid g; return g; }
 
 int bf_gemm_stream_try(int M, int N, int K, const bf_operand* A, const bf_operand* B, const bf_epilogue* E, hipStream_t st) {
     static const int enabled = bf_knob("BF_GEMM_STREAM", 1);
@@ -538,7 +540,8 @@
     a.KS = K / BK; a.mt = M / BM; a.mh = M / (BM / 2);
     static const int half_on = bf_knob("BF_STREAM_HALF", 1);
     a.hunit = half_on ? 1 : 2;
-    const int grid = (num_cus() / 8) * 8;
+    const int want = E->aux_mode == BF_AUX_DGELU ? bf_bwd_grid().stream_dgelu : 0;
+    const int grid = ((want >= 8 ? std::min(want, num_cus()) : num_cus()) / 8) * 8;
     if (!team_split(N / BNB, (use_pp || !half_on) ? a.mt : a.mh, grid / 8, &a.nb, &a.ng)) return 1;
     static const int dbg = bf_knob("BF_STREAM_DEBUG", 0);
     a.dbg = dbg;
diff --git a/bubbleformer_amd/csrc/gemm_tokred.hip b/bubbleformer_amd/csrc/gemm_tokred.hip
--- a/bubbleformer_amd/csrc/gemm_tokred.hip
+++ b/bubbleformer_amd/csrc/gemm_tokred.hip
@@ -31,10 +31,12 @@
     return __builtin_bit_cast(bf16x8, r);
 }
 
-template <int NI, int GRP>
+struct ResTile { float* out; float* colsum; int Kin, halves_per, accumulate; };
+
+template <int NI, int GRP, bool RES = false>
 __device__ __forceinline__ void tokred_pp_body(const bf16* __restrict__ A, long lda, const bf16* __restrict__ B, long ldb,
                                                float* __restrict__ slab_tile, float* __restrict__ cslab_row, int nh, bool do_cs,
-                                               unsigned ring_lds, int lane, int w4) {
+                                               unsigned ring_lds, int lane, int w4, const ResTile rt = ResTile{}) {
     using Gm = PPGeom<NI>;
     constexpr int HALFB = Gm::HALFB;
     constexpr int PG = NI == 6 ? (GRP == 0 ? 5 : 4) : 3;
@@ -83,6 +85,39 @@
 #pragma unroll
     for (int c = 0; c < 8; ++c) ones[c] = (bf16)1.0f;
 
+    f32x4 run[RES ? NI : 1][RES ? 6 : 1];
+    float runcs[NCS];
+    float* const otile = RES ? rt.out + (size_t)(16 * wm + (lane & 15)) * rt.Kin + 16 * wn + 4 * (lane >> 4) : nullptr;
+    const bool res_cs = RES && do_cs && (NI == 6 || GRP == 0) && lane < 16;
+    int left = RES ? rt.halves_per : 0;
+    if constexpr (RES) {
+#pragma unroll
+        for (int i = 0; i < NI; ++i)
+#pragma unroll
+            for (int j = 0; j < 6; ++j) run[i][j] = f32x4{0.f, 0.f, 0.f, 0.f};
+#pragma unroll
+        for (int c = 0; c < NCS; ++c) runcs[c] = 0.f;
+        if (rt.accumulate) {
+#pragma unroll
+            for (int i = 0; i < NI; ++i)
+#pragma unroll
+                for (int j = 0; j < 6; ++j) {
+                    const float4 o = *reinterpret_cast<const float4*>(otile + (size_t)(64 * i) * rt.Kin + 32 * j);
+                    run[i][j] = f32x4{o.x, o.y, o.z, o.w};
+                }
+            if (res_cs) {
+#pragma unroll
+                for (int c = 0; c < NCS; ++c) runcs[c] = rt.colsum[16 * (wm + 4 * (NI == 6 ? NCS * GRP + c : c)) + lane];
+            }
+#pragma unroll
+            for (int i = 0; i < NI; ++i)
+#pragma unroll
+                for (int j = 0; j < 6; ++j) asm volatile("s_waitcnt vmcnt(0)" : "+v"(run[i][j]) :: "memory");
+#pragma unroll
+            for (int c = 0; c < NCS; ++c) asm volatile("s_waitcnt vmcnt(0)" : "+v"(runcs[c]) :: "memory");
+        }
+    }
+
     issue(0);
     if (nh > 1) issue(1);
     if (nh > 2) issue(2);
@@ -115,11 +150,39 @@
                 else if constexpr (GRP == 0) cs[c] = __builtin_amdgcn_mfma_f32_16x16x32_bf16(ones, fa[c], cs[c], 0, 0, 0);
             }
         }
+        if constexpr (RES) {
+            if (--left == 0 || h + 1 == nh) {
+                left = rt.halves_per;
+#pragma unroll
+                for (int i = 0; i < NI; ++i)
+#pragma unroll
+                    for (int j = 0; j < 6; ++j) {
+#pragma unroll
+                        for (int e = 0; e < 4; ++e) run[i][j][e] += acc[i][j][e];
+                        acc[i][j] = f32x4{0.f, 0.f, 0.f, 0.f};
+                    }
+#pragma unroll
+                for (int c = 0; c < NCS; ++c) { runcs[c] += cs[c][0]; cs[c] = f32x4{0.f, 0.f, 0.f, 0.f}; }
+            }
+        }
         __builtin_amdgcn_sched_barrier(0);
         __builtin_amdgcn_s_barrier();
         buf = (buf + 1) & 3;
     }
     if constexpr (GRP == 0) __builtin_amdgcn_s_barrier();
+
+    if constexpr (RES) {
+#pragma unroll
+        for (int i = 0; i < NI; ++i)
+#pragma unroll
+            for (int j = 0; j < 6; ++j)
+                *reinterpret_cast<float4*>(otile + (size_t)(64 * i) * rt.Kin + 32 * j) = make_float4(run[i][j][0], run[i][j][1], run[i][j][2], run[i][j][3]);
+        if (res_cs) {
+#pragma unroll
+            for (int c = 0; c < NCS; ++c) rt.colsum[16 * (wm + 4 * (NI == 6 ? NCS * GRP + c : c)) + lane] = runcs[c];
+        }
+        return;
+    }
 
     const int wave = GRP * 4 + w4;
     float* so = slab_tile + ((size_t)wave * Gm::TILES * 64 + lane) * 4;
@@ -196,6 +259,27 @@
     else tokred_pp_body<NI, 1>(a0, lda, b0, ldb, slab_tile, cslab_row, nh, do_cs, ring_lds, lane, wave - 4);
 }
 
+constexpr int GROUP_MAX = 4;
+struct GroupGemm { const bf16* A; const bf16* B; float* out; float* colsum; long lda, ldb; int Kin, tiles_k, tile_end, halves, halves_per, accumulate; };
+struct TokredGroup { GroupGemm g[GROUP_MAX]; };
+__global__ void __launch_bounds__(512) tokred_group_kernel(const TokredGroup G, int ngemm, int total) {
+    extern __shared__ __attribute__((aligned(16))) char smem[];
+    const int tid = threadIdx.x, lane = tid & 63, wave = __builtin_amdgcn_readfirstlane(tid >> 6);
+    const int seq = xcd_remap(blockIdx.x, total);
+    GroupGemm g = G.g[0];
+    int beg = 0;
+#pragma unroll
+    for (int k = 1; k < GROUP_MAX; ++k)
+        if (k < ngemm && seq >= G.g[k - 1].tile_end) { g = G.g[k]; beg = G.g[k - 1].tile_end; }
+    const int tile = seq - beg;
+    const int n0 = (tile / g.tiles_k) * 192, c0 = (tile % g.tiles_k) * PTN;
+    const bool do_cs = g.colsum != nullptr && c0 == 0;
+    const ResTile rt{g.out + (size_t)n0 * g.Kin + c0, do_cs ? g.colsum + n0 : nullptr, g.Kin, g.halves_per, g.accumulate};
+    const unsigned ring_lds = lds_addr(smem);
+    if (wave < 4) tokred_pp_body<3, 0, true>(g.A + n0, g.lda, g.B + c0, g.ldb, nullptr, nullptr, g.halves, do_cs, ring_lds, lane, wave, rt);
+    else tokred_pp_body<3, 1, true>(g.A + n0, g.lda, g.B + c0, g.ldb, nullptr, nullptr, g.halves, do_cs, ring_lds, lane, wave - 4, rt);
+}
+
 template <int NI, int MAXS>
 __global__ void __launch_bounds__(256) tokred_pp_reduce_kernel(const float* __restrict__ slab, const float* __restrict__ cslab, int nslice,
                                                                int ntiles, int tiles_k, int Nout, int Kin, float* __restrict__ out,
@@ -507,6 +591,19 @@
 extern "C" int bf_gemm_tokred(int dtype, int Nout, int Kin, int64_t M, const void* dy, int64_t ldy, const void* x, int64_t ldx, float* out,
                               int accumulate, float* colsum, float* ws, int64_t ws_floats, bf_stream_t stream) {
     return tokred_impl(dtype, Nout, Kin, M, dy, ldy, x, ldx, out, accumulate, colsum, ws, ws_floats, false, stream);
+}
+namespace {
+struct SliceLayout { int halves_per, ns; };
+SliceLayout pp_slice_layout(int Nout, int Kin, int64_t M, int tm, int slices_env, int wgs_env) {
+    const long halves = M / HR;
+    int nslice = slices_env > 0 ? slices_env : std::max(1, wgs_env / ((Nout / tm) * (Kin / PTN)));
+    nslice = (int)std::max<long>(1, std::min<long>({(long)nslice, (long)MAX_SLICES, halves / 4}));
+    const int halves_per = bf_cdiv(halves, nslice);
+    return SliceLayout{halves_per, (int)bf_cdiv(halves, halves_per)};
+}
+bool pp_covers(int dtype, int Nout, int Kin, int64_t M, int64_t ldy, int64_t ldx) {
+    return dtype == BF_DTYPE_BF16 && Nout > 0 && Kin > 0 && Nout % 192 == 0 && Kin % PTN == 0 && M % HR == 0 && M >= 4 * HR && ldy % 8 == 0 && ldx % 8 == 0;
+}
 }
 static int tokred_impl(int dtype, int Nout, int Kin, int64_t M, const void* dy, int64_t ldy, const void* x, int64_t ldx, float* out,
                        int accumulate, float* colsum, float* ws, int64_t ws_floats, bool defer, bf_stream_t stream) {
@@ -527,13 +624,10 @@
     static const int wgs_env = bf_knob("BF_TOKRED_WGS", 128);
     if (pp) {
         const long halves = M / HR;
-        const int tiles_k0 = Kin / PTN;
         const bool big = Nout % 384 == 0 && tile_env == 384;
         const int tm = big ? 384 : 192;
-        int nslice = slices_env > 0 ? slices_env : std::max(1, wgs_env / ((Nout / tm) * tiles_k0));
-        nslice = (int)std::max<long>(1, std::min<long>({(long)nslice, (long)MAX_SLICES, halves / 4}));
-        const int halves_per = bf_cdiv(halves, nslice);
-        const int ns = bf_cdiv(halves, halves_per);
+        const SliceLayout sl = pp_slice_layout(Nout, Kin, M, tm, slices_env, wgs_env);
+        const int halves_per = sl.halves_per, ns = sl.ns;
         BF_REQUIRE(ws_floats >= (int64_t)ns * (n + Nout), "bf_gemm_tokred: workspace too small (bf_gemm_tokred_ws_floats)");
         const int tiles_k = Kin / PTN, ntiles = (Nout / tm) * tiles_k;
         static const bool fold_on = bf_knob("BF_TOKRED_FOLD", 1) != 0;
@@ -612,6 +706,52 @@
     return 0;
 }
 
+bool bf_gemm_tokred_group_covers(int dtype, int Nout, int Kin, int64_t M) { return pp_covers(dtype, Nout, Kin, M, 8, 8); }
+int bf_gemm_tokred_group(int dtype, int n, const BfTokredJob* jobs, hipStream_t st) {
+    BF_REQUIRE(n >= 1 && n <= GROUP_MAX && jobs, "bf_gemm_tokred_group: 1 .. 4 GEMMs per launch");
+    static const int slices_env = bf_knob("BF_TOKRED_SLICES", 0);
+    static const int tile_env = bf_knob("BF_TOKRED_TILE", 0);
+    static const int wgs_env = bf_knob("BF_TOKRED_WGS", 128);
+    static const int skip_env = bf_knob("BF_TOKRED_SKIP", 0);
+    if (skip_env) return 0;
+    if (tile_env == 384) return 1;
+    TokredGroup G{};
+    int total = 0;
+    double flops = 0.0, bytes = 0.0;
+    for (int k = 0; k < n; ++k) {
+        const BfTokredJob& j = jobs[k];
+        if (!pp_covers(dtype, j.Nout, j.Kin, j.M, j.ldy, j.ldx)) return 1;
+        BF_REQUIRE(j.dy && j.x && j.out, "bf_gemm_tokred_group: null pointer");
+        BF_REQUIRE(((uintptr_t)j.dy & 15) == 0 && ((uintptr_t)j.x & 15) == 0 && ((uintptr_t)j.out & 15) == 0, "bf_gemm_tokred_group: operands must be 16-byte aligned");
+        BF_REQUIRE(j.ldy >= j.Nout && j.ldx >= j.Kin, "bf_gemm_tokred_group: leading dimensions smaller than the row length");
+        const SliceLayout sl = pp_slice_layout(j.Nout, j.Kin, j.M, 192, slices_env, wgs_env);
+        const int tiles_k = j.Kin / PTN;
+        total += (j.Nout / 192) * tiles_k;
+        G.g[k] = GroupGemm{(const bf16*)j.dy, (const bf16*)j.x, j.out, j.colsum, (long)j.ldy, (long)j.ldx, j.Kin, tiles_k, total, (int)(j.M / HR), sl.halves_per, j.accumulate ? 1 : 0};
+        flops += 2.0 * j.Nout * j.Kin * (double)j.M;
+        bytes += (double)j.M * (j.Nout + j.Kin) * 2.0 + (double)j.Nout * j.Kin * 4.0;
+    }
+    BfProfScope prof(st, "tokred_group_kernel<192x192,h32,ring4>", flops, bytes);
+    static BfPerDeviceOnce attr_once; bool& attr_done = attr_once.flag();
+    constexpr int lds_bytes = NBUF * PPGeom<3>::HALFB;
+    if (!attr_done) {
+        hipError_t e_ = hipFuncSetAttribute((const void*)tokred_group_kernel, hipFuncAttributeMaxDynamicSharedMemorySize, lds_bytes);
+        if (e_ != hipSuccess) return bf_fail(e_, __FILE__, __LINE__);
+        attr_done = true;
+    }
+    hipLaunchKernelGGL(tokred_group_kernel, dim3((unsigned)total), dim3(512), lds_bytes, st, G, n, total);
+    BF_CHECK_LAUNCH();
+    return 0;
+}
+extern "C" int bf_debug_tokred_group_run(int dtype, int n, const int32_t* nout, const int32_t* kin, int64_t M, const void* const* dy, const int64_t* ldy,
+                                         const void* const* x, const int64_t* ldx, float* const* out, const int32_t* accumulate, float* const* colsum,
+                                         bf_stream_t stream) {
+    BF_REQUIRE(n >= 1 && n <= GROUP_MAX && nout && kin && dy && ldy && x && ldx && out && accumulate && colsum, "bf_debug_tokred_group_run: bad arguments");
+    BfTokredJob jobs[GROUP_MAX];
+    for (int k = 0; k < n; ++k) jobs[k] = BfTokredJob{nout[k], kin[k], M, dy[k], ldy[k], x[k], ldx[k], out[k], accumulate[k], colsum[k]};
+    return bf_gemm_tokred_group(dtype, n, jobs, (hipStream_t)stream);
+}
+
 int bf_tokred_narrow(int dtype, int C, int64_t P, const void* wide, const void* narrow, float* out, int ldo, int accumulate, int transposed,
                      const float* sc, const float* sh, int64_t rows_per_frame, float* ws, int64_t ws_floats, hipStream_t st) {
     static const bool off = bf_knob("BF_TOKRED_NARROW", 1) == 0;
diff --git a/bubbleformer_amd/csrc/model.hip b/bubbleformer_amd/csrc/model.hip
--- a/bubbleformer_amd/csrc/model.hip
+++ b/bubbleformer_amd/csrc/model.hip
@@ -79,13 +79,17 @@
 #define ZERO_ON(stream, ptr, bytes) do { hipError_t e__ = hipMemsetAsync((ptr), 0, (bytes), (stream)); if (e__ != hipSuccess) return bf_fail(e__, __FILE__, __LINE__); } while (0)
 #define HIP_TRY(x) do { hipError_t e__ = (x); if (e__ != hipSuccess) return bf_fail(e__, __FILE__, __LINE__); } while (0)
 
-struct SideStream { hipStream_t st = nullptr; hipEvent_t fork = nullptr, join = nullptr, tail[2] = {nullptr, nullptr}; bool failed = false; bool pending[2] = {false, false}; };
+constexpr int SIDE_SETS = 4, SIDE_STREAMS = 2, SIDE_STREAMS_MAX = 4, DBR_BUFS = 4;
+struct SideStream {
+    hipStream_t st = nullptr, sts[SIDE_STREAMS_MAX] = {}; hipEvent_t fork = nullptr, join = nullptr, tail[SIDE_SETS] = {}; bool failed = false;
+    bool pending[SIDE_SETS] = {}, reads_dout[SIDE_SETS] = {}; long seq[SIDE_SETS] = {}, issued = 0; int rr = 0, nst = SIDE_STREAMS;
+};
 bool g_side_defer = false;
 
 struct NextHead { bool armed = false; const float *w = nullptr, *b = nullptr; float *mean = nullptr, *rstd = nullptr, *sc = nullptr, *sh = nullptr; void* xn = nullptr; const void* saved = nullptr; };
 struct NextTail { bool armed = false; const bf_spatial_params* p = nullptr; const void* saved = nullptr; bool drop = false; };
 struct NextScale { const float* f = nullptr; int fdiv = 1; };
-struct StageHints { bool prepared = false; NextHead head; NextTail tail; NextScale scale; };
+struct StageHints { bool prepared = false; NextHead head; NextTail tail; NextScale scale; bool sliced_wgrad = false; };
 
 struct ReduceJobs {
     static constexpr int IN_CAP = 6, ATTN_CAP = 4;
@@ -102,7 +106,8 @@
     struct HeadDone { const void* saved = nullptr; hipStream_t st = nullptr; } head_done;
     struct TailDone { const void* saved = nullptr; const void* dx = nullptr; float* ws = nullptr; hipStream_t st = nullptr; } tail_done;
     struct DbrReady { const void* dx = nullptr; const float* f = nullptr; void* buf = nullptr; hipStream_t st = nullptr; } dbr_ready;
-    int scratch_parity = 0; bool tail_ws_flip = false, dbr_flip = false;
+    int scratch_parity = 0; bool tail_ws_flip = false; int dbr_flip = 0;
+    int side_lag = 2;
     bool take_head_done(const void* saved, hipStream_t st) { const bool hit = head_done.saved == saved && head_done.st == st; head_done = HeadDone{}; return hit; }
     struct { ReduceJobs jobs; bool on = false; hipStream_t st = nullptr; } reduce;
     hipEvent_t handoff = nullptr;
@@ -117,9 +122,14 @@
             int lo = 0, hi = 0;
             (void)hipDeviceGetStreamPriorityRange(&lo, &hi);
             const unsigned ef = hipEventDisableTiming | hipEventDisableSystemFence;
-            if (hipStreamCreateWithPriority(&s.st, hipStreamNonBlocking, lo) != hipSuccess || hipEventCreateWithFlags(&s.fork, ef) != hipSuccess ||
-                hipEventCreateWithFlags(&s.join, ef) != hipSuccess || hipEventCreateWithFlags(&s.tail[0], ef) != hipSuccess ||
-                hipEventCreateWithFlags(&s.tail[1], ef) != hipSuccess) { s.failed = true; s.st = nullptr; }
+            bool ok = hipEventCreateWithFlags(&s.fork, ef) == hipSuccess && hipEventCreateWithFlags(&s.join, ef) == hipSuccess;
+            static const int nst_env = bf_knob("BF_SIDE_STREAMS", SIDE_STREAMS);
+            s.nst = std::min(std::max(nst_env, 1), SIDE_STREAMS_MAX);
+            for (int i = 0; ok && i < s.nst; ++i) ok = hipStreamCreateWithPriority(&s.sts[i], hipStreamNonBlocking, lo) == hipSuccess;
+            ok = ok && hipStreamCreateWithPriority(&s.st, hipStreamNonBlocking, lo) == hipSuccess;
+            for (int i = 0; ok && i < SIDE_SETS; ++i) ok = hipEventCreateWithFlags(&s.tail[i], ef) == hipSuccess;
+            if (!ok) s.st = nullptr;
+            s.failed = !ok;
         }
         return s.st ? &s : nullptr;
     }
@@ -169,28 +179,63 @@
         if (s) { HIP_TRY(hipEventRecord(s->join, s->st)); HIP_TRY(hipStreamWaitEvent(main, s->join, 0)); }
     }
     if (!s) return 0;
-    for (int i = 0; i < 2; ++i)
+    for (int i = 0; i < SIDE_SETS; ++i)
         if ((set < 0 || set == i) && s->pending[i]) {
             HIP_TRY(hipStreamWaitEvent(main, s->tail[i], 0));
             s->pending[i] = false;
         }
     return 0;
 }
+int side_join_old(TrunkLinks& L, hipStream_t main) {
+    SideStream* s = L.side_stream();
+    if (!s) return 0;
+    const long next = s->issued + 1;
+    for (int i = 0; i < SIDE_SETS; ++i)
+        if (s->pending[i] && (s->seq[i] <= next - L.side_lag || (s->reads_dout[i] && s->seq[i] <= next - 2))) {
+            HIP_TRY(hipStreamWaitEvent(main, s->tail[i], 0));
+            s->pending[i] = false;
+        }
+    return 0;
+}
+bool g_group_off = false;
+bool group_covers(const D& d) {
+    static const bool on = bf_knob("BF_TOKRED_GROUP", 1) != 0;
+    if (!on || g_group_off || d.E % 192) return false;
+    const int bt = 16 * (d.E / 192) * (d.E / 192);
+    return bt >= 32 && bt <= 64 && bf_gemm_tokred_group_covers(d.dtype, d.E, d.E, d.N);
+}
+struct BwdGridScope {
+    BfBwdGrid was;
+    explicit BwdGridScope(bool group) : was(bf_bwd_grid()) {
+        static const int sg = bf_knob("BF_BWD_STREAM_WGS", 0), ag = bf_knob("BF_BWD_ATTN_WGS", 0);
+        if (group) bf_bwd_grid() = BfBwdGrid{sg, ag};
+    }
+    ~BwdGridScope() { bf_bwd_grid() = was; }
+};
 struct Fork {
     hipStream_t main; SideStream* s; bool used = false; bool deferred; int set;
-    std::vector<std::function<int(hipStream_t)>> jobs;
+    bool group = false; int dtype = 0, n_gemm = 0; BfTokredJob gemms[4]; bool reads_dout = false;
     std::vector<std::function<int(hipStream_t)>> late;
     hipStream_t last_side = nullptr;
-    explicit Fork(TrunkLinks& L, hipStream_t m, bool may_defer = false, int scratch_set = 0) : main(m), s(L.side_stream()), set(scratch_set) {
+    explicit Fork(TrunkLinks& L, hipStream_t m, bool may_defer = false, int scratch_set = 0, const D* d = nullptr, bool may_group = true)
+        : main(m), s(L.side_stream()), set(scratch_set) {
         deferred = may_defer && g_side_defer && s != nullptr;
-    }
-    int begin(hipStream_t* out) {
+        group = deferred && d && may_group && group_covers(*d);
+        if (d) dtype = d->dtype;
+    }
+    int begin(hipStream_t* out, hipStream_t side = nullptr) {
         *out = main;
         if (!s) return 0;
+        if (!side) side = s->st;
         HIP_TRY(hipEventRecord(s->fork, main));
-        HIP_TRY(hipStreamWaitEvent(s->st, s->fork, 0));
+        HIP_TRY(hipStreamWaitEvent(side, s->fork, 0));
         used = true;
-        *out = s->st;
+        *out = side;
+        return 0;
+    }
+    int add(const BfTokredJob& j) {
+        BF_REQUIRE(group && n_gemm < 4, "Fork: more weight-gradient GEMMs than one grouped launch holds");
+        gemms[n_gemm++] = j;
         return 0;
     }
     template <class F> int run(F&& job) {
@@ -208,18 +253,25 @@
         return 0;
     }
     int flush() {
-        if (!deferred || jobs.empty()) return 0;
+        if (!group || n_gemm == 0) return 0;
         hipStream_t ss;
-        TRY(begin(&ss));
-        for (auto& j : jobs) TRY(j(ss));
-        jobs.clear();
-        return 0;
+        TRY(begin(&ss, s->sts[s->rr]));
+        s->rr = (s->rr + 1) % s->nst;
+        last_side = ss;
+        const int rc = bf_gemm_tokred_group(dtype, n_gemm, gemms, ss);
+        n_gemm = 0;
+        BF_REQUIRE(rc <= 0, "Fork: a stage's weight gradients left the grouped launch's tiling");
+        return rc;
     }
     int join() {
         if (deferred) {
             TRY(flush());
             TRY(drain_late());
-            if (used) { HIP_TRY(hipEventRecord(s->tail[set], s->st)); s->pending[set] = true; used = false; }
+            ++s->issued;
+            if (used) {
+                HIP_TRY(hipEventRecord(s->tail[set], last_side ? last_side : s->st));
+                s->pending[set] = true; s->seq[set] = s->issued; s->reads_dout[set] = reads_dout; used = false;
+            }
             return 0;
         }
         TRY(drain_late());
@@ -600,7 +652,7 @@
 }
 void* bwd_scratch(TrunkLinks& L, const D& d, void* scratch) {
     if (!g_side_defer || !L.side_stream()) return scratch;
-    L.scratch_parity ^= 1;
+    L.scratch_parity = (L.scratch_parity + 1) % SIDE_SETS;
     return (char*)scratch + (size_t)L.scratch_parity * Scratch(d, nullptr).bytes;
 }
 struct TailNorm { const void* z; void* dz; const float *mean, *rstd, *w, *g; int gdiv; float* ws; bool* done; };
@@ -636,7 +688,8 @@
                 const float* W, const float* bias, const float* nb, const float* gamma, const float* lo, const float* hi,
                 const float* alpha, const float* mc, float* dW, float* dbias, float* dnb, float* dgamma, float* dlo, float* dhi,
                 void* don, hipStream_t st, Fork& fk, const InFuse* fu = nullptr) {
-    TRY(fk.run([=](hipStream_t ss) -> int {
+    if (fk.group) TRY(fk.add(BfTokredJob{d.E, d.E, d.N, dout, d.E, on, d.E, sc.G, 0, sc.csum}));
+    else TRY(fk.run([=](hipStream_t ss) -> int {
         const void* dsrc = dout;
         const int trc = bf_gemm_tokred_deferred(d.dtype, d.E, d.E, d.N, dsrc, d.E, on, d.E, sc.G, 0, sc.csum, sc.tokred_ws, sc.tokred_floats, ss);
         if (trc < 0) return trc;
@@ -670,7 +723,8 @@
                const void* w_c, float* dW, float* db, void* dxn, const bf_epilogue* dx_epi, hipStream_t st, Fork& fk, const InFuse* fu = nullptr,
                bool last = false, const void* w_t = nullptr, void* scaled_out = nullptr, const float* rowfac = nullptr, int rpg = 1,
                bool* scaled_done = nullptr) {
-    TRY(fk.run([=](hipStream_t ss) -> int {
+    if (fk.group && xpro == BF_PRO_NONE) TRY(fk.add(BfTokredJob{Nout, Kin, d.N, dy, Nout, x, Kin, dW, 1, db}));
+    else TRY(fk.run([=](hipStream_t ss) -> int {
         const void* xo = x;
         int pro = xpro;
         bf_operand A = op_plain(dy, Nout, BF_LAY_XC);
@@ -711,9 +765,10 @@
 extern "C" int64_t bf_temporal_saved_bytes(const bf_dims* s) { D d; if (get_dims(s, &d)) return -1; return (int64_t)TemporalSaved(d, nullptr).bytes; }
 extern "C" int64_t bf_spatial_saved_bytes(const bf_dims* s) { D d; if (get_dims(s, &d)) return -1; return (int64_t)SpatialSaved(d, nullptr).bytes; }
 size_t dbr_bytes(const D& d) { return (((size_t)d.N * d.E * d.es) + 255) & ~(size_t)255; }
-extern "C" int64_t bf_scratch_bytes(const bf_dims* s) { D d; if (get_dims(s, &d)) return -1; return 2 * (int64_t)Scratch(d, nullptr).bytes + 2 * (int64_t)dbr_bytes(d); }
+extern "C" int64_t bf_scratch_bytes(const bf_dims* s) { D d; if (get_dims(s, &d)) return -1; return SIDE_SETS * (int64_t)Scratch(d, nullptr).bytes + DBR_BUFS * (int64_t)dbr_bytes(d); }
 
 extern "C" void bf_side_defer(int on) { g_side_defer = on != 0; }
+extern "C" void bf_debug_tokred_group(int on) { g_group_off = on == 0; }
 extern "C" int bf_side_join(bf_stream_t s) { return side_join_pending(g_links.get(), (hipStream_t)s); }
 
 extern "C" void bf_stage_prepared(int on) { g_links.get().hints.prepared = on != 0; }
@@ -790,8 +845,9 @@
     TemporalSaved sv(d, saved);
     Scratch sc(d, bwd_scratch(L, d, scratch));
     const void* win_c = d.dtype == BF_DTYPE_F32 ? (const void*)p->input_head_w : sv.win_c;
-    Fork fk(L, st, true, L.scratch_parity);
-    if (fk.deferred) TRY(side_join_pending(L, st, fk.set));
+    Fork fk(L, st, true, L.scratch_parity, &d, !H.sliced_wgrad);
+    const BwdGridScope grid_scope(fk.group);
+    if (fk.deferred) { TRY(side_join_old(L, st)); TRY(side_join_pending(L, st, fk.set)); }
     void* don = sc.t1;
     void* dO = sc.t1b;
     void* dqkv = sc.t3;
@@ -805,6 +861,7 @@
         }
     }
     L.dbr_ready = TrunkLinks::DbrReady{};
+    fk.reads_dout = dbr == dout;
     const InFuse fu2{sv.o, nullptr, dO, sv.mean2, sv.rstd2, p->norm2_w, p->norm2_b, sc.in_ws2};
     TRY(outproj_bwd(d, sc, dbr, sv.on, sv.wout_s, p->output_head_w, p->output_head_b, p->norm2_b, p->gamma, nullptr, nullptr,
                     sv.alpha, sv.mc, g->output_head_w, g->output_head_b, nullptr, g->gamma, nullptr, nullptr, don, st, fk, &fu2));
@@ -826,7 +883,7 @@
     static const bool chain_on = bf_knob("BF_BWD_CHAIN", 1) != 0;
     if (H.tail.armed && chain_on && fk.deferred && d.dtype == BF_DTYPE_BF16 && d.S == 144 && d.F % 2 == 0) {
         const NextTail& h = H.tail;
-        const int oset = L.scratch_parity ^ 1;
+        const int oset = (L.scratch_parity + 1) % SIDE_SETS;
         TRY(side_join_pending(L, st, oset));
         Scratch so(d, (char*)scratch + (size_t)oset * Scratch(d, nullptr).bytes);
         SpatialSaved ps(d, const_cast<void*>(h.saved));
@@ -1005,8 +1062,9 @@
     const void* w1_c = f32 ? (const void*)p->fc1_w : sv.w1_c;
     const void* w2_c = f32 ? (const void*)p->fc2_w : sv.w2_c;
     TRY(flush_pending_reduce(L, st));
-    Fork fk(L, st, true, L.scratch_parity);
-    if (fk.deferred) TRY(side_join_pending(L, st, fk.set));
+    Fork fk(L, st, true, L.scratch_parity, &d, !H.sliced_wgrad);
+    const BwdGridScope grid_scope(fk.group);
+    if (fk.deferred) { TRY(side_join_old(L, st)); TRY(side_join_pending(L, st, fk.set)); }
     void* dz = sc.t1;
     ReduceJobs jobs;
     const TrunkLinks::TailDone td = L.tail_done;
@@ -1073,11 +1131,11 @@
     L.dbr_ready = TrunkLinks::DbrReady{};
     static const bool scaled_on = bf_knob("BF_BWD_SCALED_COPY", 1) != 0;
     if (ns.f && scaled_on && fk.deferred && d.dtype == BF_DTYPE_BF16) {
-        fu1.scaled_out = (char*)scratch + 2 * Scratch(d, nullptr).bytes + (L.dbr_flip ? dbr_bytes(d) : 0);
+        fu1.scaled_out = (char*)scratch + SIDE_SETS * Scratch(d, nullptr).bytes + (size_t)L.dbr_flip * dbr_bytes(d);
         fu1.scaled_f = ns.f; fu1.scaled_fdiv = ns.fdiv; fu1.scaled_done = &scaled_done;
     }
     TRY(linear_bwd(d, sc, dqkv, 3 * d.E, sv.xn, d.E, BF_PRO_NONE, nullptr, nullptr, win_c, g->input_head_w, g->input_head_b, dxn, nullptr, st, fk, &fu1, true));
-    if (scaled_done) { L.dbr_ready = {dx, ns.f, fu1.scaled_out, st}; L.dbr_flip = !L.dbr_flip; }
+    if (scaled_done) { L.dbr_ready = {dx, ns.f, fu1.scaled_out, st}; L.dbr_flip = (L.dbr_flip + 1) % DBR_BUFS; }
     TRY(jobs.push(InReduceJob{sc.in_ws, (int)d.F, d.E, p->norm1_w, p->norm1_b, nullptr, 1, g->norm1_w, g->norm1_b, nullptr, nullptr, nullptr, nullptr}));
     static const bool merge_on = bf_knob("BF_REDUCE_MERGE", 1) != 0;
     if (fk.deferred && merge_on) { L.reduce.jobs = jobs; L.reduce.on = true; L.reduce.st = st; }
@@ -1133,12 +1191,28 @@
     (void)L.take_hints();
     const void* cur = dout;
     int rot = 0;
+    struct LagScope { TrunkLinks& L; int was; ~LagScope() { L.side_lag = was; } } lag_scope{L, L.side_lag};
+    L.side_lag = SIDE_SETS;
+    SideStream* side = g_side_defer ? L.side_stream() : nullptr;
+    std::vector<std::pair<int, long>> unreported;
+    auto report = [&]() {
+        size_t k = 0;
+        for (; k < unreported.size(); ++k) {
+            bool in_flight = false;
+            for (int q = 0; side && q < SIDE_SETS; ++q) in_flight |= side->pending[q] && side->seq[q] == unreported[k].second;
+            if (in_flight) break;
+            stage_done(unreported[k].first, user);
+        }
+        unreported.erase(unreported.begin(), unreported.begin() + k);
+    };
     for (int i = n - 1; i >= 0; --i) {
         BF_REQUIRE(params[i] && grads[i] && saved[i] && (kinds[i] == 0 || kinds[i] == 1), "bf_trunk_train_bwd: bad stage entry");
         const void* in = i ? acts[i - 1] : x;
         void* gout = i ? gbuf3[rot] : dx;
         rot = (rot + 1) % 3;
         StageHints H;
+        static const int tail_stages = bf_knob("BF_GROUP_TAIL", 2);
+        H.sliced_wgrad = i < tail_stages;
         if (kinds[i] == 0) {
             if (i > 0 && kinds[i - 1] == 1) H.tail = NextTail{true, (const bf_spatial_params*)params[i - 1], saved[i - 1], drop_b && drop_b[i - 1]};
             TRY(temporal_bwd(L, H, dims, (const bf_temporal_params*)params[i], (const bf_temporal_params*)grads[i], in, cur, gout, saved[i], scratch,
@@ -1148,8 +1222,12 @@
             TRY(spatial_bwd(L, H, dims, (const bf_spatial_params*)params[i], (const bf_spatial_params*)grads[i], in, cur, gout, saved[i], scratch,
                             drop_a ? drop_a[i] : nullptr, drop_b ? drop_b[i] : nullptr, s));
         }
-        if (stage_done) stage_done(i, user);
+        if (stage_done) { unreported.push_back({i, side ? side->issued : 0}); report(); }
         cur = gout;
+    }
+    if (stage_done && !unreported.empty()) {
+        TRY(side_join_pending(L, (hipStream_t)s));
+        report();
     }
     return 0;
 }
diff --git a/bubbleformer_amd/kernels.py b/bubbleformer_amd/kernels.py
--- a/bubbleformer_amd/kernels.py
+++ b/bubbleformer_amd/kernels.py
@@ -30,6 +30,22 @@
     if rc == 1:
         return False
     L.check(rc, "bf_gemm_tokred")
+    return True
+
+
+def gemm_tokred_group(gemms):
+    n = len(gemms)
+    M = gemms[0][0].shape[0]
+    assert all(dy.shape[0] == M and x.shape[0] == M for dy, x, *_ in gemms)
+    i32a, i64a, vpa = C.c_int32 * n, C.c_int64 * n, C.c_void_p * n
+    rc = L.lib().bf_debug_tokred_group_run(
+        _dt(gemms[0][1].dtype), n, i32a(*[g[0].shape[1] for g in gemms]), i32a(*[g[1].shape[1] for g in gemms]), M,
+        vpa(*[_p(g[0]) for g in gemms]), i64a(*[g[0].stride(0) for g in gemms]), vpa(*[_p(g[1]) for g in gemms]),
+        i64a(*[g[1].stride(0) for g in gemms]), vpa(*[_p(g[2]) for g in gemms]), i32a(*[int(bool(g[3])) for g in gemms]),
+        vpa(*[_p(g[4]) for g in gemms]), _stream())
+    if rc == 1:
+        return False
+    L.check(rc, "bf_debug_tokred_group_run")
     return True
 
 
diff --git a/include/bubbleformer_hip.h b/include/bubbleformer_hip.h
--- a/include/bubbleformer_hip.h
+++ b/include/bubbleformer_hip.h
@@ -120,6 +120,10 @@
 int bf_side_join(bf_stream_t stream);
 void bf_debug_force_generic_attn(int on);
 void bf_debug_tokred_fold(int on);
+void bf_debug_tokred_group(int on);
+int bf_debug_tokred_group_run(int dtype, int n, const int32_t* nout, const int32_t* kin, int64_t M, const void* const* dy, const int64_t* ldy,
+                              const void* const* x, const int64_t* ldx, float* const* out, const int32_t* accumulate, float* const* colsum,
+                              bf_stream_t stream);
 
 int bf_im2col_nchw(int dtype, const float* x, void* out, int frames, int C, int H, int W, int Kp, bf_stream_t stream);
 int bf_col2im_nchw(int dtype, const void* g, float* dx, int frames, int C, int H, int W, int Kp, bf_stream_t stream);
```

After: 795.0 samples/s. -2.5%, worse.
